# cg-saarland/hagrid

Measured on AMD Instinct MI355X. Metric: Mrays/s (primary traversal) + grid build ms, 1M-tri scene @1/2/4/8 MI355X, higher is better.
Workload: dtype f32

## Files before the change

hagrid_amd/csrc/build.hip:

```cpp
#include "ctx.h"
#include "wave_prims.h"

#include "hagrid/grid.h"
#include "hagrid/prims.h"

#include <cstring>
#include <vector>

using namespace hagrid;
using namespace hagrid_impl;

namespace {

struct BuildK {
    ivec3 dims;
    int shift;
    vec3 bmin, bmax;
    vec3 cell_size;
};

__device__ __forceinline__ Tri load_tri(const float4* __restrict__ tris, int i) {
    const float4* p = tris + 3 * size_t(i);
    const float4 a = p[0], b = p[1], c = p[2];
    return Tri(vec3(a.x, a.y, a.z), a.w, vec3(b.x, b.y, b.z), b.w, vec3(c.x, c.y, c.z), c.w);
}
__device__ __forceinline__ void store_cell(Cell* cells, int i, ivec3 lo, int begin, ivec3 hi, int end) {
    int4* p = reinterpret_cast<int4*>(cells) + 2 * size_t(i);
    p[0] = make_int4(lo.x, lo.y, lo.z, begin);
    p[1] = make_int4(hi.x, hi.y, hi.z, end);
}
__device__ __forceinline__ ivec3 load_cell_min(const Cell* cells, int i) {
    const int4 a = reinterpret_cast<const int4*>(cells)[2 * size_t(i)];
    return ivec3(a.x, a.y, a.z);
}
__device__ __forceinline__ BBox cell_world_box(const BuildK& k, ivec3 lo, ivec3 hi) {
    return BBox(k.bmin + vec3(lo) * k.cell_size, k.bmin + vec3(hi) * k.cell_size);
}

constexpr int kBoxWords = 8;
constexpr int kNoBadTri = 0x7fffffff;
__device__ __forceinline__ int wave_min_i(int v) { return -wave_max(-v); }
__global__ void __launch_bounds__(kBlock) bbox_partials(const float4* __restrict__ tris, int n, float* __restrict__ partials) {
    __shared__ float lds[kWaves][6];
    __shared__ int lds_bad[kWaves];
    float lo[3] = { FLT_MAX, FLT_MAX, FLT_MAX }, hi[3] = { -FLT_MAX, -FLT_MAX, -FLT_MAX };
    int bad = kNoBadTri;
    for (int i = blockIdx.x * kBlock + threadIdx.x; i < n; i += gridDim.x * kBlock) {
        const Tri t = load_tri(tris, i);
        const BBox b = t.bbox();
        if (!tri_admissible(t)) bad = min(bad, i);
        lo[0] = min(lo[0], b.min.x); lo[1] = min(lo[1], b.min.y); lo[2] = min(lo[2], b.min.z);
        hi[0] = max(hi[0], b.max.x); hi[1] = max(hi[1], b.max.y); hi[2] = max(hi[2], b.max.z);
    }
#pragma unroll
    for (int c = 0; c < 3; c++) { lo[c] = wave_min_f(lo[c]); hi[c] = wave_max_f(hi[c]); }
    bad = wave_min_i(bad);
    if (lane_id() == 0) { for (int c = 0; c < 3; c++) { lds[wave_id()][c] = lo[c]; lds[wave_id()][3 + c] = hi[c]; } lds_bad[wave_id()] = bad; }
    __syncthreads();
    if (threadIdx.x < 6) {
        float v = lds[0][threadIdx.x];
        for (int w = 1; w < kWaves; w++) v = threadIdx.x < 3 ? min(v, lds[w][threadIdx.x]) : max(v, lds[w][threadIdx.x]);
        partials[blockIdx.x * kBoxWords + threadIdx.x] = v;
    } else if (threadIdx.x == 6) {
        int v = lds_bad[0];
        for (int w = 1; w < kWaves; w++) v = min(v, lds_bad[w]);
        reinterpret_cast<int*>(partials)[blockIdx.x * kBoxWords + 6] = v;
    }
}
__global__ void __launch_bounds__(kBlock) bbox_final(const float* __restrict__ partials, int num, float* __restrict__ out) {
    __shared__ float lds[kWaves][6];
    __shared__ int lds_bad[kWaves];
    float v[6] = { FLT_MAX, FLT_MAX, FLT_MAX, -FLT_MAX, -FLT_MAX, -FLT_MAX };
    int bad = kNoBadTri;
    for (int i = threadIdx.x; i < num; i += kBlock) {
        for (int c = 0; c < 6; c++) v[c] = c < 3 ? min(v[c], partials[i * kBoxWords + c]) : max(v[c], partials[i * kBoxWords + c]);
        bad = min(bad, reinterpret_cast<const int*>(partials)[i * kBoxWords + 6]);
    }
#pragma unroll
    for (int c = 0; c < 6; c++) v[c] = c < 3 ? wave_min_f(v[c]) : wave_max_f(v[c]);
    bad = wave_min_i(bad);
    if (lane_id() == 0) { for (int c = 0; c < 6; c++) lds[wave_id()][c] = v[c]; lds_bad[wave_id()] = bad; }
    __syncthreads();
    if (threadIdx.x < 6) {
        float r = lds[0][threadIdx.x];
        for (int w = 1; w < kWaves; w++) r = threadIdx.x < 3 ? min(r, lds[w][threadIdx.x]) : max(r, lds[w][threadIdx.x]);
        out[threadIdx.x] = r;
    } else if (threadIdx.x == 6) {
        int r = lds_bad[0];
        for (int w = 1; w < kWaves; w++) r = min(r, lds_bad[w]);
        reinterpret_cast<int*>(out)[6] = r;
    }
}

constexpr int kCoopCells = 64;


__global__ void __launch_bounds__(kBlock) top_log_dims(const int* __restrict__ refs_per_cell, int num_top, BuildK k, float snd_density,
                                                       int* __restrict__ log_dims, int* __restrict__ max_out) {
    __shared__ int lds[kWaves];
    const int i = blockIdx.x * kBlock + threadIdx.x;
    int ld = 0;
    if (i < num_top) {
        const vec3 ext = BBox(k.bmin, k.bmax).extents() / vec3(k.dims);
        const ivec3 d = compute_grid_dims(BBox(vec3(0, 0, 0), ext), refs_per_cell[i], snd_density);
        const int max_dim = max(d.x, max(d.y, d.z));
        ld = 31 - __clz(max_dim);
        ld = (1 << ld) < max_dim ? ld + 1 : ld;
        log_dims[i] = ld;
    }
    ld = wave_max(ld);
    if (lane_id() == 0) lds[wave_id()] = ld;
    __syncthreads();
    if (threadIdx.x == 0) {
        int m = lds[0];
        for (int w = 1; w < kWaves; w++) m = max(m, lds[w]);
        if (m > 0) atomicMax(max_out, m);
    }
}


__device__ __forceinline__ BuildK with_device_shift(BuildK k, const int* __restrict__ shift_dev, vec3 extents) {
    k.shift = *shift_dev;
    k.cell_size = extents / vec3(k.dims << k.shift);
    return k;
}

__device__ __forceinline__ bool prefix_too_large(int s) { return unsigned(s) >= 0x40000000u; }
struct ChildCountIn {
    const uint32_t* entries;
    __device__ int operator()(int i) const { return (entries[i] & 3u) ? 8 : 0; }
    __device__ void load4(int i, int n, int* v) const {
        if (i + 4 <= n && lb_aligned16(entries + i)) {
            const uint4 e = *reinterpret_cast<const uint4*>(entries + i);
            v[0] = (e.x & 3u) ? 8 : 0; v[1] = (e.y & 3u) ? 8 : 0; v[2] = (e.z & 3u) ? 8 : 0; v[3] = (e.w & 3u) ? 8 : 0;
        } else {
            for (int c = 0; c < 4; c++) v[c] = i + c < n ? (*this)(i + c) : 0;
        }
    }
};
struct UpdateEntriesOut {
    uint32_t* entries; int* too_large;
    __device__ static uint32_t word(uint32_t e, int i, int start) { const uint32_t ld = e & 3u; return ld | (uint32_t(ld ? start : i) << 2); }
    __device__ void operator()(int i, int start) const { entries[i] = word(entries[i], i, start); if (prefix_too_large(start)) *too_large = 1; }
    __device__ void store4(int i, int n, const int* v) const {
        if (i + 4 <= n && lb_aligned16(entries + i)) {
            uint4* p = reinterpret_cast<uint4*>(entries + i);
            const uint4 e = *p;
            if (prefix_too_large(v[3])) *too_large = 1;
            *p = make_uint4(word(e.x, i, v[0]), word(e.y, i + 1, v[1]), word(e.z, i + 2, v[2]), word(e.w, i + 3, v[3]));
        } else {
            for (int c = 0; c < 4; c++) if (i + c < n) (*this)(i + c, v[c]);
        }
    }
};

__device__ __forceinline__ int split_mask(const BuildK& k, ivec3 lo, ivec3 hi, const Tri& tri) {
    const vec3 cmin = k.bmin + k.cell_size * vec3(lo);
    const vec3 cmax = k.bmin + k.cell_size * vec3(hi);
    const vec3 mid = (cmin + cmax) * 0.5f;
    int mask = 0xFF;
    const BBox rb = tri.bbox();
    if (rb.min.x > cmax.x || rb.max.x < cmin.x) mask = 0;
    if (rb.min.x > mid.x) mask &= 0xAA;
    if (rb.max.x < mid.x) mask &= 0x55;
    if (rb.min.y > cmax.y || rb.max.y < cmin.y) mask = 0;
    if (rb.min.y > mid.y) mask &= 0xCC;
    if (rb.max.y < mid.y) mask &= 0x33;
    if (rb.min.z > cmax.z || rb.max.z < cmin.z) mask = 0;
    if (rb.min.z > mid.z) mask &= 0xF0;
    if (rb.max.z < mid.z) mask &= 0x0F;
    int todo = mask;
    while (todo) {
        const int i = __ffs(todo) - 1;
        todo &= todo - 1;
        const BBox b(vec3(i & 1 ? mid.x : cmin.x, i & 2 ? mid.y : cmin.y, i & 4 ? mid.z : cmin.z),
                     vec3(i & 1 ? cmax.x : mid.x, i & 2 ? cmax.y : mid.y, i & 4 ? cmax.z : mid.z));
        if (!intersect_prim_cell(tri, b)) mask &= ~(1 << i);
    }
    return mask;
}


struct LeafIn {
    const uint32_t* entries; const int* cell_counts;
    __device__ static Int2 item(uint32_t e, int count) { const bool leaf = (e & 3u) == 0; return Int2{ leaf ? 1 : 0, leaf ? count : 0 }; }
    __device__ Int2 operator()(int i) const { return item(entries[i], cell_counts[i]); }
    __device__ void load4(int i, int n, Int2* v) const {
        if (i + 4 <= n && lb_aligned16(entries + i) && lb_aligned16(cell_counts + i)) {
            const uint4 e = *reinterpret_cast<const uint4*>(entries + i);
            const int4 c = *reinterpret_cast<const int4*>(cell_counts + i);
            v[0] = item(e.x, c.x); v[1] = item(e.y, c.y); v[2] = item(e.z, c.z); v[3] = item(e.w, c.w);
        } else {
            for (int k = 0; k < 4; k++) v[k] = i + k < n ? (*this)(i + k) : Int2{0, 0};
        }
    }
};
struct LeafOut {
    int* start_cell; int* ref_begin;
    __device__ void operator()(int i, Int2 v) const { start_cell[i] = v.a; ref_begin[i] = v.b; }
    __device__ void store4(int i, int n, const Int2* v) const {
        if (i + 4 <= n && lb_aligned16(start_cell + i) && lb_aligned16(ref_begin + i)) {
            *reinterpret_cast<int4*>(start_cell + i) = make_int4(v[0].a, v[1].a, v[2].a, v[3].a);
            *reinterpret_cast<int4*>(ref_begin + i) = make_int4(v[0].b, v[1].b, v[2].b, v[3].b);
        } else {
            for (int k = 0; k < 4; k++) if (i + k < n) (*this)(i + k, v[k]);
        }
    }
};


#ifndef HG_TILE_REFS
#define HG_TILE_REFS 1024
#endif
#ifndef HG_CHUNK_CELLS
#define HG_CHUNK_CELLS 256
#endif
#ifndef HG_EMIT_CHUNK
#define HG_EMIT_CHUNK 256
#endif
#ifndef HG_STAGE
#define HG_STAGE 1024
#endif
constexpr int kTileRefs = HG_TILE_REFS;
constexpr int kChunkCells = HG_CHUNK_CELLS;
constexpr int kEmitChunk = HG_EMIT_CHUNK;
constexpr int kStage = HG_STAGE;

__device__ __forceinline__ void mark_tiles(int* __restrict__ tile_first, int i, int start, int count) {
    for (int t = start / kTileRefs + 1; t <= (start + count) / kTileRefs; t++) tile_first[t] = i + 1;
}
struct SegIn {
    const int* counts;
    __device__ int operator()(int i) const { return counts[i]; }
};
struct SegOut {
    const int* counts; int* seg_begin; int* tile_first;
    Cell* cells; uint32_t* entries; int* cell_counts; const int* log_dims; const int* shift_dev; ivec3 dims;
    __device__ void operator()(int i, int start) const {
        seg_begin[i] = start; mark_tiles(tile_first, i, start, counts[i]);
        const int shift = *shift_dev;
        entries[i] = 0u; cell_counts[i] = 0;
        const int x = i % dims.x, y = (i / dims.x) % dims.y, z = i / (dims.x * dims.y);
        const ivec3 lo(x << shift, y << shift, z << shift);
// ... 425 lines not shown
struct GLevel {
    int2* refs = nullptr; int num_refs = 0;
    Cell* cells = nullptr; uint32_t* entries = nullptr; int num_cells = 0;
    int* cell_counts = nullptr;
    int* seg_begin = nullptr;
    int* tile_first = nullptr; int num_tiles = 0;
    int* start_cell = nullptr; int* ref_begin = nullptr;
};

struct Arena {
    hagrid_ctx* ctx; Temps& tmp; char* base = nullptr; size_t size = 0, used = 0, wanted = 0; int num_tris;
    Arena(hagrid_ctx* c, Temps& t, int n_tris) : ctx(c), tmp(t), num_tris(n_tris) {
        size_t want = c->build_arena_hint;
        if (want && c->build_arena_tris > 0 && 2ll * n_tris < c->build_arena_tris)
            want = size_t(double(want) * 1.25 * double(std::max(n_tris, 1)) / double(c->build_arena_tris)) + 4096;
        if (want) {
            base = pool_try_alloc<char>(c, want);
            if (base) { t.ptrs.push_back(base); size = want; }
        }
    }
    ~Arena() { ctx->build_arena_hint = wanted; ctx->build_arena_tris = num_tris; }
    template <typename T> T* get(size_t n) {
        const size_t bytes = (std::max(n, size_t(1)) * sizeof(T) + 255) & ~size_t(255);
        wanted += bytes;
        if (base && used + bytes <= size) { T* p = reinterpret_cast<T*>(base + used); used += bytes; return p; }
        return tmp.get<T>(n);
    }
    void drop(void* p) { if (!base || p < base || p >= base + size) tmp.drop(p); }
};

int build_levels(hagrid_ctx* ctx, const float4* tris, int num_tris, hagrid_grid* grid, BuildK k, const BBox& gb, float snd_density, Temps& tmp) {
    hipStream_t st = ctx->stream;
    int* dsc = ctx->dscratch;
    Arena ar(ctx, tmp, num_tris);
    const ivec3 dims = k.dims;
    const int num_top = dims.x * dims.y * dims.z;

    int* counts = ar.get<int>(size_t(num_tris));
    int* start_emit = ar.get<int>(size_t(num_tris));
    int* refs_per_cell = ar.get<int>(size_t(num_top));
    int* log_dims = ar.get<int>(size_t(num_top));
    int* const partials = nullptr;
    if (!counts || !start_emit || !refs_per_cell || !log_dims) return HAGRID_ENOMEM;
    HG_HIP(ctx, hipMemsetAsync(refs_per_cell, 0, size_t(num_top) * sizeof(int), st));
    int* big_list = ar.get<int>(size_t(num_tris));
    if (!big_list) return HAGRID_ENOMEM;
    top_range_sizes<<<grid_blocks(num_tris, kBlock), kBlock, 0, st>>>(tris, num_tris, k, counts, big_list, dsc + 2); HG_DBG(ctx);
    if (!ctx_scan<int>(ctx, PlainIn{counts}, PlainOut{start_emit, dsc + 3}, num_tris, partials, (const int*)nullptr, dsc + 0)) return HAGRID_ENOMEM;
    int R0 = 0, num_big = 0;
    {
        int h[4];
        HG_TRY(read_back(ctx, dsc, h, sizeof(h)));
        R0 = h[0]; num_big = h[2];
        if (h[3]) R0 = -1;
    }
    if (R0 < 0 || R0 > 0x3fffffff) HG_FAIL(ctx, HAGRID_ERANGE, "build_grid: too many top-level references");
    ar.drop(counts);
    int* pair_rank = ar.get<int>(size_t(R0) + 1);
    if (!pair_rank) return HAGRID_ENOMEM;
    const int prim_blocks = grid_blocks(num_tris, kBlock), big_blocks = std::min(num_big, 2048);
    count_top_refs<<<prim_blocks + big_blocks, kBlock, 0, st>>>(tris, num_tris, k, start_emit, refs_per_cell, pair_rank, big_list, dsc + 2, prim_blocks); HG_DBG(ctx);
    top_log_dims<<<grid_blocks(num_top, kBlock), kBlock, 0, st>>>(refs_per_cell, num_top, k, snd_density, log_dims, dsc + 1); HG_DBG(ctx);

    std::vector<GLevel> levels;
    GLevel L;
    L.num_refs = R0; L.num_cells = num_top;
    L.num_tiles = grid_blocks(R0, kTileRefs);
    L.refs = ar.get<int2>(size_t(R0) + 1);
    L.cells = ar.get<Cell>(size_t(num_top)); L.entries = ar.get<uint32_t>(size_t(num_top) + 1);
    L.cell_counts = ar.get<int>(size_t(num_top)); L.seg_begin = ar.get<int>(size_t(num_top) + 1);
    L.tile_first = ar.get<int>(size_t(L.num_tiles) + 2);
    L.start_cell = ar.get<int>(size_t(num_top)); L.ref_begin = ar.get<int>(size_t(num_top));
    if (!L.refs || !L.cells || !L.entries || !L.cell_counts || !L.seg_begin || !L.tile_first || !L.start_cell || !L.ref_begin) return HAGRID_ENOMEM;
    if (!ctx_scan<int>(ctx, SegIn{refs_per_cell}, SegOut{refs_per_cell, L.seg_begin, L.tile_first, L.cells, L.entries, L.cell_counts, log_dims, dsc + 1, dims}, num_top, partials,
                       (const int*)nullptr, (int*)nullptr)) return HAGRID_ENOMEM;
    hagrid_build_counts& bc = ctx->counts;
    memset(&bc, 0, sizeof(bc));
    bc.num_tris = num_tris; bc.top_cells = num_top; bc.top_refs = R0;
    emit_top_refs<<<prim_blocks + big_blocks, kBlock, 0, st>>>(tris, num_tris, k, dsc + 1, gb.extents(), start_emit, pair_rank, L.seg_begin, L.refs, log_dims, L.entries, big_list, dsc + 2, prim_blocks); HG_DBG(ctx);
    levels.push_back(L);

    {
        if (!ctx_scan<int>(ctx, ChildCountIn{L.entries}, UpdateEntriesOut{L.entries, dsc + 3}, num_top, (int*)nullptr, (const int*)nullptr, dsc + 8)) return HAGRID_ENOMEM;
    }
    int num_new_cells = 0, shift = 0;
    {
        int h[8];
        HG_TRY(read_back(ctx, dsc + 1, h, sizeof(h)));
        shift = h[0]; num_new_cells = h[7];
        if (h[2]) num_new_cells = -1;
    }
    if (shift >= 24) HG_FAIL(ctx, HAGRID_ERANGE, "build_grid: too many levels");
    k.shift = shift;
    k.cell_size = gb.extents() / vec3(dims << shift);
    ar.drop(start_emit); ar.drop(pair_rank); ar.drop(refs_per_cell);
    for (int level = 0;; level++) {
        GLevel& P = levels.back();
        int* tot = dsc + 8 + 4 * level;
        if (num_new_cells < 0 || num_new_cells > 0x3fffffff) HG_FAIL(ctx, HAGRID_ERANGE, "build_grid: level too large");
        if ((int)levels.size() >= 24) HG_FAIL(ctx, HAGRID_ERANGE, "build_grid: too many levels");
        const bool last = num_new_cells == 0;
        if (last && level > 0) {
            if (level < HAGRID_MAX_LEVELS) { bc.level_refs[level] = P.num_refs; bc.level_cells[level] = P.num_cells; bc.level_kept[level] = P.num_refs; bc.num_levels = level + 1; }
            break;
        }
        GLevel N;
        N.num_cells = num_new_cells;
        unsigned char* masks = ar.get<unsigned char>(size_t(P.num_refs) + 1);
        if (!masks) return HAGRID_ENOMEM;
        if (!last) {
            N.cells = ar.get<Cell>(size_t(num_new_cells)); N.entries = ar.get<uint32_t>(size_t(num_new_cells) + 1);
            N.cell_counts = ar.get<int>(size_t(num_new_cells)); N.seg_begin = ar.get<int>(size_t(num_new_cells) + 1);
            N.tile_first = ar.get<int>(size_t(grid_blocks(8ll * P.num_refs, kTileRefs)) + 2);
            N.start_cell = ar.get<int>(size_t(num_new_cells)); N.ref_begin = ar.get<int>(size_t(num_new_cells));
            if (!N.cells || !N.entries || !N.cell_counts || !N.seg_begin || !N.tile_first || !N.start_cell || !N.ref_begin) return HAGRID_ENOMEM;
        }
        if (P.num_refs > 0) {
            classify_refs<<<std::min(P.num_tiles, 4096), kBlock, 0, st>>>(P.refs, P.seg_begin, P.num_cells, P.num_refs, P.tile_first, P.num_tiles, level == 0 ? 1 : 0,
                                                                             tris, P.cells, P.entries, k, masks, P.cell_counts, N.cells, N.cell_counts, N.entries, tot + 1); HG_DBG(ctx);
        }
        Int2* next = reinterpret_cast<Int2*>(tot + 2);
        if (!last) {
            if (!ctx_scan<Int2>(ctx, ChildSegIn{N.cell_counts, N.entries}, ChildSegOut{N.cell_counts, N.entries, N.seg_begin, N.tile_first, tot + 1}, num_new_cells, (Int2*)nullptr,
                                (const Int2*)nullptr, next)) return HAGRID_ENOMEM;
        }
        int h3[3] = {0, 0, 0};
        HG_TRY(read_back(ctx, tot + 1, h3, sizeof(h3)));
        if (h3[0] < 0) HG_FAIL(ctx, HAGRID_ERANGE, "build_grid: level too large");
        if (level < HAGRID_MAX_LEVELS) { bc.level_refs[level] = P.num_refs; bc.level_cells[level] = P.num_cells; bc.level_kept[level] = h3[0]; bc.num_levels = level + 1; }
        if (last) { ar.drop(masks); break; }
        const int num_children = h3[1];
        if (num_children < 0 || num_children > 0x3fffffff) HG_FAIL(ctx, HAGRID_ERANGE, "build_grid: level too large");
        N.num_refs = num_children; N.num_tiles = grid_blocks(num_children, kTileRefs);
        N.refs = ar.get<int2>(size_t(num_children) + 1);
        if (!N.refs) return HAGRID_ENOMEM;
        if (P.num_refs > 0 && num_children > 0) {
            emit_child_refs<<<std::min(P.num_tiles, 4096), kBlock, 0, st>>>(P.refs, P.seg_begin, P.num_cells, P.num_refs, P.tile_first, P.num_tiles,
                                                                                   masks, P.entries, N.seg_begin, N.refs); HG_DBG(ctx);
        }
        ar.drop(masks);
        num_new_cells = h3[2];
        levels.push_back(N);
    }
    ar.drop(log_dims);

    const int num_levels = (int)levels.size();
    long long total_cells_ll = 0;
    int max_cells = 0;
    for (auto& V : levels) { total_cells_ll += V.num_cells; max_cells = std::max(max_cells, V.num_cells); }
    if (total_cells_ll > 0x3fffffff) HG_FAIL(ctx, HAGRID_ERANGE, "build_grid: too many voxel map entries");
    const int total_cells = int(total_cells_ll);
    Int2* const part2 = nullptr;
    Int2* carry = reinterpret_cast<Int2*>(dsc + 128);
    for (int l = 0; l < num_levels; l++) {
        GLevel& V = levels[l];
        if (!ctx_scan<Int2>(ctx, LeafIn{V.entries, V.cell_counts}, LeafOut{V.start_cell, V.ref_begin}, V.num_cells, part2,
                            l ? carry + (l - 1) : (const Int2*)nullptr, carry + l)) return HAGRID_ENOMEM;
    }
    int hf[2];
    HG_TRY(read_back(ctx, carry + (num_levels - 1), hf, sizeof(hf)));
    const int new_total_cells = hf[0], total_refs = hf[1];
    if (new_total_cells <= 0 || total_refs < 0) HG_FAIL(ctx, HAGRID_ERANGE, "build_grid: inconsistent totals");

    Cell* out_cells = pool_alloc<Cell>(ctx, size_t(new_total_cells));
    uint32_t* out_entries = pool_alloc<uint32_t>(ctx, size_t(total_cells));
    int* out_refs = pool_alloc<int>(ctx, size_t(total_refs));
    if (!out_cells || !out_entries || !out_refs) {
        hagrid_mem_free(ctx, out_cells); hagrid_mem_free(ctx, out_entries); hagrid_mem_free(ctx, out_refs);
        return HAGRID_ENOMEM;
    }
    for (int l = 0, off = 0; l < num_levels; off += levels[l].num_cells, l++) {
        GLevel& V = levels[l];
        concat_level<<<grid_blocks(V.num_cells, kBlock), kBlock, 0, st>>>(V.entries, V.cells, V.cell_counts, V.start_cell, V.ref_begin, V.num_cells, off,
                                                                                  V.refs, V.seg_begin, V.num_refs, l == 0 ? 1 : 0, out_cells, out_entries, out_refs); HG_DBG(ctx);
    }
    hipError_t e = hipGetLastError();
    if (e == hipSuccess) e = hipStreamSynchronize(st);
    if (e != hipSuccess) {
        hagrid_mem_free(ctx, out_cells); hagrid_mem_free(ctx, out_entries); hagrid_mem_free(ctx, out_refs);
        HG_FAIL(ctx, HAGRID_EHIP, hipGetErrorString(e));
    }
    memset(grid, 0, sizeof(*grid));
    grid->entries = out_entries; grid->ref_ids = out_refs; grid->cells = out_cells; grid->small_cells = nullptr;
    grid->bbox_min[0] = gb.min.x; grid->bbox_min[1] = gb.min.y; grid->bbox_min[2] = gb.min.z;
    grid->bbox_max[0] = gb.max.x; grid->bbox_max[1] = gb.max.y; grid->bbox_max[2] = gb.max.z;
    grid->dims[0] = dims.x; grid->dims[1] = dims.y; grid->dims[2] = dims.z;
    grid->num_cells = new_total_cells; grid->num_entries = total_cells; grid->num_refs = total_refs;
    bc.build_cells = new_total_cells; bc.build_entries = total_cells; bc.build_refs = total_refs;
    grid->shift = shift;
    grid->num_offsets = shift + 1;
    for (int i = 0, off = 0; i <= shift; i++) {
        if (i < num_levels) off += levels[i].num_cells;
        grid->offsets[i] = off;
    }
    return HAGRID_OK;
}

}

extern "C" int hagrid_build_grid(hagrid_ctx* ctx, const void* tris_v, int num_tris, hagrid_grid* grid,
                                 float top_density, float snd_density) {
    if (!ctx || !grid) return HAGRID_EINVAL;
    trav_image_drop(ctx);
    if (!tris_v || num_tris <= 0) HG_FAIL(ctx, HAGRID_EINVAL, "build_grid: no triangles");
    HG_HIP(ctx, hipSetDevice(ctx->device));
    const float4* tris = static_cast<const float4*>(tris_v);
    hipStream_t st = ctx->stream;
    Temps tmp(ctx);
    int* dsc = ctx->dscratch;
    HG_HIP(ctx, hipMemsetAsync(dsc, 0, 256 * sizeof(int), st));

    const int bb_blocks = std::min(grid_blocks(num_tris, kBlock), 1024);
    float* bb_part = tmp.get<float>(size_t(bb_blocks) * kBoxWords + 8);
    if (!bb_part) return HAGRID_ENOMEM;
    float* bb_out = bb_part + size_t(bb_blocks) * kBoxWords;
    bbox_partials<<<bb_blocks, kBlock, 0, st>>>(tris, num_tris, bb_part); HG_DBG(ctx);
    bbox_final<<<1, kBlock, 0, st>>>(bb_part, bb_blocks, bb_out); HG_DBG(ctx);
    float hb[8];
    HG_TRY(read_back(ctx, bb_out, hb, sizeof(hb)));
    int bad_tri; memcpy(&bad_tri, &hb[6], sizeof(int));
    if (bad_tri != kNoBadTri) {
        char msg[96];
        snprintf(msg, sizeof(msg), "build_grid: triangle %d is not finite", bad_tri);
        HG_FAIL(ctx, HAGRID_EINVAL, msg);
    }
    BBox gb(vec3(hb[0], hb[1], hb[2]), vec3(hb[3], hb[4], hb[5]));
    {
        const vec3 e = gb.extents();
        if (!(e.x <= FLT_MAX && e.y <= FLT_MAX && e.z <= FLT_MAX)) HG_FAIL(ctx, HAGRID_ERANGE, "build_grid: the extent of the scene box is not finite");
    }
    if (!grid_dims_defined(gb, num_tris, top_density)) gb = widen_scene_box(gb);
    ivec3 dims = compute_grid_dims(gb, num_tris, top_density);
    if (dims.x > 0x3fffffff || dims.y > 0x3fffffff || dims.z > 0x3fffffff) HG_FAIL(ctx, HAGRID_ERANGE, "build_grid: top-level grid too large");
    dims.x += dims.x & 1; dims.y += dims.y & 1; dims.z += dims.z & 1;
    const vec3 ext = gb.extents();
    gb.min -= ext * 0.001f;
    gb.max += ext * 0.001f;
    const long long num_top_ll = (long long)dims.x * dims.y * dims.z;
    if (num_top_ll > 0x3fffffff) HG_FAIL(ctx, HAGRID_ERANGE, "build_grid: top-level grid too large");
    {
        const vec3 e = gb.extents();
        if (!(e.x <= FLT_MAX && e.y <= FLT_MAX && e.z <= FLT_MAX)) HG_FAIL(ctx, HAGRID_ERANGE, "build_grid: the extent of the scene box is not finite");
    }

    BuildK k;
    k.dims = dims; k.shift = 0; k.bmin = gb.min; k.bmax = gb.max; k.cell_size = vec3(0.0f);

    return build_levels(ctx, tris, num_tris, grid, k, gb, snd_density, tmp);
}
```

hagrid_amd/csrc/compress.hip:

```cpp
#include "ctx.h"
#include "wave_prims.h"

#include "hagrid/grid.h"

using namespace hagrid;
using namespace hagrid_impl;

namespace {

struct SentinelIn {
    const Cell* cells;
    __device__ int operator()(int i) const {
        const int4* p = reinterpret_cast<const int4*>(cells) + 2 * size_t(i);
        const int n = p[1].w - p[0].w;
        return n > 0 ? n + 1 : 0;
    }
};

struct SmallCellOut {
    const Cell* cells; const int* refs; uint4* small_cells; int* out_refs;
    __device__ void operator()(int i, int first) const {
        const int4* p = reinterpret_cast<const int4*>(cells) + 2 * size_t(i);
        const int4 a = p[0], b = p[1];
        const int n = b.w - a.w;
        small_cells[i] = make_uint4((uint32_t(a.x) & 0xffffu) | (uint32_t(a.y) << 16),
                                    (uint32_t(a.z) & 0xffffu) | (uint32_t(b.x) << 16),
                                    (uint32_t(b.y) & 0xffffu) | (uint32_t(b.z) << 16),
                                    uint32_t(n > 0 ? first : -1));
        if (n > 0) {
            for (int j = 0; j < n; j++) out_refs[first + j] = refs[a.w + j];
            out_refs[first + n] = -1;
        }
    }
};
struct NullOut { __device__ void operator()(int, int) const {} };

}

extern "C" int hagrid_compress_grid(hagrid_ctx* ctx, hagrid_grid* grid) {
    if (!ctx || !grid) return HAGRID_EINVAL;
    if (!grid->cells || !grid->ref_ids) HG_FAIL(ctx, HAGRID_EINVAL, "compress_grid: incomplete (or already compressed) grid");
    trav_image_drop(ctx);
    for (int c = 0; c < 3; c++)
        if ((grid->dims[c] << grid->shift) >= (1 << 16)) return 0;
    HG_HIP(ctx, hipSetDevice(ctx->device));
    hipStream_t st = ctx->stream;
    const int n = grid->num_cells;
    const Cell* cells = static_cast<const Cell*>(grid->cells);
    int* partials = pool_alloc<int>(ctx, size_t(scan_num_tiles(n)) + 1);
    uint4* small = static_cast<uint4*>(hagrid_mem_alloc(ctx, size_t(n) * 16));
    if (!partials || !small) { hagrid_mem_free(ctx, partials); hagrid_mem_free(ctx, small); return HAGRID_ENOMEM; }
    int* total = ctx->dscratch;
    scan_partials<int, SentinelIn><<<std::max(scan_num_tiles(n), 1), kBlock, 0, st>>>(SentinelIn{cells}, n, partials); HG_DBG(ctx);
    scan_spine<int><<<1, kBlock, 0, st>>>(partials, scan_num_tiles(n), nullptr, total); HG_DBG(ctx);
    int h = 0;
    int rc = read_back(ctx, total, &h, sizeof(int));
    if (rc != HAGRID_OK || h < 0) { hagrid_mem_free(ctx, partials); hagrid_mem_free(ctx, small); return rc != HAGRID_OK ? rc : HAGRID_ERANGE; }
    int* srefs = pool_alloc<int>(ctx, size_t(h));
    if (!srefs) { hagrid_mem_free(ctx, partials); hagrid_mem_free(ctx, small); return HAGRID_ENOMEM; }
    scan_apply<int, SentinelIn, SmallCellOut><<<std::max(scan_num_tiles(n), 1), kBlock, 0, st>>>(
        SentinelIn{cells}, SmallCellOut{cells, static_cast<const int*>(grid->ref_ids), small, srefs}, n, partials); HG_DBG(ctx);
    hipError_t e = hipGetLastError();
    if (e == hipSuccess) e = hipStreamSynchronize(st);
    hagrid_mem_free(ctx, partials);
    ctx->counts.compressed = 1; ctx->counts.compress_cells = n; ctx->counts.compress_refs_out = h;
    if (e != hipSuccess) { hagrid_mem_free(ctx, small); hagrid_mem_free(ctx, srefs); HG_FAIL(ctx, HAGRID_EHIP, hipGetErrorString(e)); }
    hagrid_mem_free(ctx, grid->cells);
    hagrid_mem_free(ctx, grid->ref_ids);
    grid->cells = nullptr;
    grid->small_cells = small;
    grid->ref_ids = srefs;
    grid->num_refs = h;
    return 1;
}
```

hagrid_amd/csrc/ctx.h:

```cpp
#pragma once

#include <hip/hip_runtime.h>

#include <atomic>
#include <cstdio>
#include <memory>
#include <string>
#include <unordered_map>
#include <vector>

#include "hagrid_amd.h"

namespace hagrid_impl {

struct Slot {
    void* ptr = nullptr;
    size_t size = 0;
    bool in_use = false;
    int refs = 0;
};

}

namespace hagrid_impl {

struct TravImageCache {
    void* table = nullptr;
    size_t table_bytes = 0;
    int wide_records = 0;
    void* blocks = nullptr;
    size_t block_bytes = 0;
    bool valid = false;
    bool uniform = false;
    bool general = false;
    int slim = 0;
    int vtop_k = 0;
    uint32_t vtop_base = 0;
    bool detached = false;
    bool borrowed = false;
    std::shared_ptr<std::atomic<bool>> alive;
    const void* entries = nullptr; const void* cells = nullptr; const void* refs = nullptr;
    int num_cells = 0, num_entries = 0, num_refs = 0, shift = 0, dims[3] = {0, 0, 0}, cell_bytes = 32;
    int max_ref = -1;
    void* alt_blocks = nullptr; void* alt_table = nullptr; size_t alt_block_bytes = 0, alt_table_bytes = 0; int alt_wide_records = 0, alt_slim = 0;
};

}

namespace hagrid_impl {
enum MailboxWord : int {
    kMbxRowLen = 300,
    kMbxOrderStale = 304,
    kMbxReadBackEpoch = 310,
    kMbxHeadSuggest = 312,
    kMbxPriorStats = 316,
};
enum ScratchWord : int {
    kScrRowLenBinned = 232,
    kScrRowLen = 236,
    kScrMaxRef = 240,
    kScrBlobFlag = 250,
};
}

struct hagrid_ctx {
    int device = 0;
    hipStream_t stream = nullptr;
    bool keep = false;
    int num_cus = 0;

    std::vector<hagrid_impl::Slot> slots;
    std::unordered_map<void*, int> tracker;
    size_t usage = 0, max_usage = 0;

    hipEvent_t ev_begin = nullptr, ev_end = nullptr;

    int* mailbox = nullptr;
    int* dscratch = nullptr;
    unsigned long long* lb_state = nullptr;
    size_t lb_words = 0;
    unsigned lb_epoch = 0;
    int* row_scores = nullptr;
    int* bin_diff = nullptr;

    int ray_binning = 0;
    int opt_variant = 0;
    int opt_lookback = 1;
    int opt_merge_inplace = 1;
    int opt_merge_inplace_iters = 0;
    int opt_merge_inplace_div = 0;
    int opt_merge_inplace_room = 0;
    int opt_merge_narrow = 1;
    int opt_expand_voxel_map = 1;
    int opt_expand_subset_only = 1;
    int opt_image_width = 0;
    int opt_band_rows = 0;
    int opt_super_log2 = 3;
    int opt_xcd_chunk_log2 = -2;
    int opt_narrow = 1;
    int opt_image_max_mb = 0;
    int opt_quad_head = 20;
    int opt_image_vtop = 1;
    int opt_image_uniform = 1;
    int opt_row_cache = 1;
    struct RayHints {
        const void* key_rays = nullptr; int key_n = 0;
        const void* rowlen_rays = nullptr; int rowlen_n = 0, rowlen_age = 0, rowlen_known = -1, rowlen_seen = 0; bool rows_from_origins = false ;
        hipEvent_t rowlen_evt = nullptr; bool rowlen_pending = false;
        int* lpt_buf = nullptr; int lpt_cap = 0; const void* lpt_rays = nullptr; int lpt_n = 0, lpt_blocks = 0, lpt_age = 0, lpt_period = 32, lpt_rot = 0 ; bool rot_adopted = false ;
        hipEvent_t trial_evt[2] = {nullptr, nullptr}; bool trial_pending = false, trial_with_head = false, head_disabled = false;
        float t_base = 0.0f, t_head = 0.0f; int n_base = 0, n_head = 0, trial_opt = -1 ; unsigned head_serial = 0 ; bool lpt_valid = false;
        int lpt_epoch = 1 , relearn_streak = 0, cooldown = 0, cooldown_len = 64; unsigned long long relearn_clock = 0;
        hipEvent_t share_evt[12][2] = {}; int share_issued = 0, share_done = 0, share_choice = -1 , share_ncand = 0 , share_shape_nc = 0 , share_cands[4] = {0, 0, 0, 0} ,
            share_last = -1 , share_launches = 0; float share_t[4] = {0.0f, 0.0f, 0.0f, 0.0f}; unsigned share_serial = 0 ;
        int trial_kind = 0 , n_all = 0, all_stage = 0 ; float t_all = 0.0f; bool learned_all = false;
        bool learned_once = false;
        unsigned order_serial = 0;
        bool cmp_pending = false, cmp_done = false; int n_conf = 0; float t_conf = 0.0f;
        bool order_loses = false;
        int last_report = -1;
        unsigned long long used = 0;
    };
    static constexpr int kRayHints = 4;
    RayHints hints[kRayHints];
    unsigned long long hint_clock = 0;
    int opt_mailbox = -1;
    int opt_tail = 1;
    int opt_lds_pad = 0;
    int opt_tail_dual = -1;
    int opt_share_trial = 1;
    int opt_order_gate = 1;
    int opt_tile_order = -1;
    int opt_quad_tail = -1;
    int opt_image_slim = 1;
    int opt_image_general = 1;
    int opt_image = 2;

    int opt_id_is_steps = 0;

    hagrid_impl::TravImageCache image;
    unsigned image_serial = 0;
    int readback_epoch = 0;
    int opt_fast_readback = 1;
    int build_arena_tris = 0;
    size_t build_arena_hint = 0;
    hagrid_build_counts counts = {};

    std::string err;
};

namespace hagrid_impl {

inline int fail(hagrid_ctx* ctx, int code, const char* file, int line, const char* msg) {
    if (ctx) {
        char buf[512];
        snprintf(buf, sizeof(buf), "%s(%d): %s", file, line, msg);
        ctx->err = buf;
    }
    return code;
}

#define HG_FAIL(ctx, code, msg) return ::hagrid_impl::fail((ctx), (code), __FILE__, __LINE__, (msg))
#define HG_HIP(ctx, call)                                                                         \
    do {                                                                                          \
        hipError_t e_ = (call);                                                                   \
        if (e_ != hipSuccess) return ::hagrid_impl::fail((ctx), HAGRID_EHIP, __FILE__, __LINE__, hipGetErrorString(e_)); \
    } while (0)
#define HG_TRY(expr)                                                                              \
    do {                                                                                          \
        int rc_ = (expr);                                                                         \
        if (rc_ < 0) return rc_;                                                                  \
    } while (0)

void debug_sync(hagrid_ctx* ctx, const char* file, int line);
#ifdef HAGRID_DEBUG_SYNC
#define HG_DBG(ctx) ::hagrid_impl::debug_sync((ctx), __FILE__, __LINE__)
#else
#define HG_DBG(ctx) do { } while (0)
#endif

template <typename T>
inline T* pool_alloc(hagrid_ctx* ctx, size_t n) {
    return static_cast<T*>(hagrid_mem_alloc(ctx, (n ? n : 1) * sizeof(T)));
}

template <typename T>
inline T* pool_try_alloc(hagrid_ctx* ctx, size_t n) {
    const std::string saved = ctx->err;
    T* p = pool_alloc<T>(ctx, n);
    if (!p) { (void)hipGetLastError(); ctx->err = saved; }
    return p;
}

struct PoolTemps {
    hagrid_ctx* ctx;
    std::vector<void*> ptrs;
    explicit PoolTemps(hagrid_ctx* c) : ctx(c) {}
    PoolTemps(const PoolTemps&) = delete;
    PoolTemps& operator=(const PoolTemps&) = delete;
    template <typename T> T* get(size_t n) { T* p = pool_alloc<T>(ctx, n); if (p) ptrs.push_back(p); return p; }
    void drop(void* p) { for (auto& q : ptrs) if (q == p && p) { hagrid_mem_free(ctx, p); q = nullptr; } }
    void* keep(void* p) { for (auto& q : ptrs) if (q == p) q = nullptr; return p; }
    ~PoolTemps() { for (void* p : ptrs) if (p) hagrid_mem_free(ctx, p); }
};

int pool_split(hagrid_ctx* ctx, void* base, void* const* parts, int n);

int read_back(hagrid_ctx* ctx, const void* dptr, void* hptr, size_t bytes);

inline int grid_blocks(long long n, int block) { return (int)((n + block - 1) / block); }

inline bool aligned(const void* p, size_t n) { return (reinterpret_cast<uintptr_t>(p) & (n - 1)) == 0; }

unsigned long long* lookback_state(hagrid_ctx* ctx, int tiles, int words_per_tile, unsigned* epoch);

int trav_image_build(hagrid_ctx* ctx, const hagrid_grid* grid);
void trav_image_drop(hagrid_ctx* ctx);
bool trav_image_matches(const hagrid_ctx* ctx, const hagrid_grid* grid);
bool trav_image_stale(const hagrid_ctx* ctx);
void trav_image_source_touched(hagrid_ctx* ctx, const void* ptr, size_t bytes);

}
```

hagrid_amd/csrc/ctx.hip:

```cpp
#include "ctx.h"

#include <chrono>

#include <algorithm>
#include <cstring>
#include <iostream>

using namespace hagrid_impl;

extern "C" int hagrid_abi_version(void) { return HAGRID_ABI_VERSION; }

extern "C" int hagrid_ctx_create(hagrid_ctx** out, int device, int keep) {
    if (!out) return HAGRID_EINVAL;
    *out = nullptr;
    int count = 0;
    if (hipGetDeviceCount(&count) != hipSuccess || count <= 0 || device < 0 || device >= count) return HAGRID_ENODEV;
    hagrid_ctx* ctx = new hagrid_ctx();
    ctx->device = device;
    ctx->keep = keep != 0;
    if (hipSetDevice(device) != hipSuccess) { delete ctx; return HAGRID_ENODEV; }
    hipDeviceProp_t prop;
    if (hipGetDeviceProperties(&prop, device) != hipSuccess) { delete ctx; return HAGRID_ENODEV; }
    ctx->num_cus = prop.multiProcessorCount;
    if (hipEventCreate(&ctx->ev_begin) != hipSuccess || hipEventCreate(&ctx->ev_end) != hipSuccess ||
        hipHostMalloc((void**)&ctx->mailbox, 320 * sizeof(int), hipHostMallocDefault) != hipSuccess ||
        hipMalloc((void**)&ctx->dscratch, 256 * sizeof(int)) != hipSuccess) {
        hagrid_ctx_destroy(ctx);
        return HAGRID_EHIP;
    }
    memset(ctx->mailbox, 0, 320 * sizeof(int));
    *out = ctx;
    return HAGRID_OK;
}

extern "C" void hagrid_ctx_destroy(hagrid_ctx* ctx) {
    if (!ctx) return;
    (void)hipSetDevice(ctx->device);
    (void)hipStreamSynchronize(ctx->stream);
    for (auto& h : ctx->hints) h.rowlen_pending = false;
    if (!ctx->image.borrowed && ctx->image.alive) ctx->image.alive->store(false);
    for (auto& s : ctx->slots)
        if (s.ptr) (void)hipFree(s.ptr);
    if (ctx->ev_begin) (void)hipEventDestroy(ctx->ev_begin);
    if (ctx->ev_end) (void)hipEventDestroy(ctx->ev_end);
    for (auto& h : ctx->hints) { if (h.rowlen_evt) (void)hipEventDestroy(h.rowlen_evt); if (h.lpt_buf) (void)hipFree(h.lpt_buf); for (auto& e : h.trial_evt) if (e) (void)hipEventDestroy(e); for (auto& pr : h.share_evt) for (auto& e : pr) if (e) (void)hipEventDestroy(e); }
    if (ctx->mailbox) (void)hipHostFree(ctx->mailbox);
    if (ctx->dscratch) (void)hipFree(ctx->dscratch);
    if (ctx->bin_diff) (void)hipFree(ctx->bin_diff);
    if (ctx->row_scores) (void)hipFree(ctx->row_scores);
    if (ctx->lb_state) (void)hipFree(ctx->lb_state);
    delete ctx;
}

extern "C" int hagrid_ctx_set_stream(hagrid_ctx* ctx, void* stream) {
    if (!ctx) return HAGRID_EINVAL;
    hipStream_t next = static_cast<hipStream_t>(stream);
    if (next == ctx->stream) return HAGRID_OK;
    HG_HIP(ctx, hipSetDevice(ctx->device));
    HG_HIP(ctx, hipStreamSynchronize(ctx->stream));
    ctx->stream = next;
    return HAGRID_OK;
}

extern "C" int hagrid_ctx_synchronize(hagrid_ctx* ctx) {
    if (!ctx) return HAGRID_EINVAL;
    HG_HIP(ctx, hipSetDevice(ctx->device));
    HG_HIP(ctx, hipStreamSynchronize(ctx->stream));
    return HAGRID_OK;
}

extern "C" int hagrid_get_build_counts(const hagrid_ctx* ctx, hagrid_build_counts* out) {
    if (!ctx || !out) return HAGRID_EINVAL;
    *out = ctx->counts;
    return HAGRID_OK;
}

extern "C" const char* hagrid_last_error(const hagrid_ctx* ctx) { return ctx ? ctx->err.c_str() : "no context"; }

extern "C" int hagrid_device_info(const hagrid_ctx* ctx, char* name, int name_len, int* compute_units, int64_t* total_mem) {
    if (!ctx) return HAGRID_EINVAL;
    hipDeviceProp_t prop;
    if (hipGetDeviceProperties(&prop, ctx->device) != hipSuccess) return HAGRID_EHIP;
    if (name && name_len > 0) { strncpy(name, prop.gcnArchName, (size_t)name_len - 1); name[name_len - 1] = 0; }
    if (compute_units) *compute_units = prop.multiProcessorCount;
    if (total_mem) *total_mem = (int64_t)prop.totalGlobalMem;
    return HAGRID_OK;
}


static void release_slot_memory(hagrid_ctx* ctx, Slot& s) {
    if (s.ptr) (void)hipFree(s.ptr);
    ctx->usage -= s.size;
    s.ptr = nullptr;
    s.size = 0;
}

extern "C" void* hagrid_mem_alloc(hagrid_ctx* ctx, size_t bytes) {
    if (!ctx) return nullptr;
    if (bytes == 0) bytes = 4;
    bytes = (bytes + 255) & ~size_t(255);
    int fit = -1, biggest = -1, empty = -1;
    for (int i = 0, n = (int)ctx->slots.size(); i < n; i++) {
        const Slot& s = ctx->slots[i];
        if (s.in_use) continue;
        if (!s.ptr) { if (empty < 0) empty = i; continue; }
        if (s.size >= bytes && (fit < 0 || s.size < ctx->slots[fit].size)) fit = i;
        if (biggest < 0 || s.size > ctx->slots[biggest].size) biggest = i;
    }
    int idx = fit;
    if (idx >= 0 && ctx->slots[idx].size > 4 * bytes && ctx->slots[idx].size > (size_t(64) << 20)) idx = -1;
    if (idx < 0) {
        idx = fit < 0 ? (biggest >= 0 && ctx->keep ? biggest : empty) : empty;
        if (idx < 0) { idx = (int)ctx->slots.size(); ctx->slots.emplace_back(); }
        Slot& s = ctx->slots[idx];
        if (s.ptr) release_slot_memory(ctx, s);
        void* p = nullptr;
        (void)hipSetDevice(ctx->device);
        if (hipMalloc(&p, bytes) != hipSuccess) {
            for (auto& t : ctx->slots) if (!t.in_use && t.ptr) release_slot_memory(ctx, t);
            if (hipMalloc(&p, bytes) != hipSuccess) { fail(ctx, HAGRID_ENOMEM, __FILE__, __LINE__, "hipMalloc failed"); return nullptr; }
        }
        s.ptr = p; s.size = bytes;
        ctx->usage += bytes;
        ctx->max_usage = std::max(ctx->max_usage, ctx->usage);
    }
    Slot& s = ctx->slots[idx];
    s.in_use = true;
    s.refs = 1;
    ctx->tracker[s.ptr] = idx;
    return s.ptr;
}

int hagrid_impl::pool_split(hagrid_ctx* ctx, void* base, void* const* parts, int n) {
    auto it = ctx->tracker.find(base);
    if (it == ctx->tracker.end() || n <= 0) HG_FAIL(ctx, HAGRID_EINVAL, "pool_split: not a pool buffer");
    const int idx = it->second;
    Slot& s = ctx->slots[idx];
    if (s.refs != 1 || s.ptr != base) HG_FAIL(ctx, HAGRID_EINVAL, "pool_split: buffer is already split");
    for (int i = 0; i < n; i++) {
        const char* p = static_cast<const char*>(parts[i]);
        if (p < static_cast<const char*>(base) || p >= static_cast<const char*>(base) + s.size) HG_FAIL(ctx, HAGRID_EINVAL, "pool_split: part outside the buffer");
        for (int j = 0; j < i; j++) if (parts[j] == parts[i]) HG_FAIL(ctx, HAGRID_EINVAL, "pool_split: parts coincide");
    }
    ctx->tracker.erase(it);
    for (int i = 0; i < n; i++) ctx->tracker[parts[i]] = idx;
    s.refs = n;
    return HAGRID_OK;
}

extern "C" int hagrid_mem_free(hagrid_ctx* ctx, void* ptr) {
    if (!ctx) return HAGRID_EINVAL;
    if (!ptr) return HAGRID_OK;
    auto it = ctx->tracker.find(ptr);
    if (it == ctx->tracker.end()) HG_FAIL(ctx, HAGRID_EINVAL, "free of a pointer that does not come from this MemManager");
    trav_image_source_touched(ctx, ptr, 1);
    it = ctx->tracker.find(ptr);
    Slot& s = ctx->slots[it->second];
    ctx->tracker.erase(it);
    if (--s.refs > 0) return HAGRID_OK;
    s.in_use = false;
    if (!ctx->keep) {
        HG_HIP(ctx, hipStreamSynchronize(ctx->stream));
        release_slot_memory(ctx, s);
    }
    return HAGRID_OK;
}

extern "C" int hagrid_mem_copy_h2d(hagrid_ctx* ctx, void* dst, const void* src, size_t bytes) {
    if (!ctx) return HAGRID_EINVAL;
    if (!bytes) return HAGRID_OK;
    trav_image_source_touched(ctx, dst, bytes);
    HG_HIP(ctx, hipSetDevice(ctx->device));
    HG_HIP(ctx, hipMemcpyAsync(dst, src, bytes, hipMemcpyHostToDevice, ctx->stream));
    HG_HIP(ctx, hipStreamSynchronize(ctx->stream));
    return HAGRID_OK;
}
extern "C" int hagrid_mem_copy_d2h(hagrid_ctx* ctx, void* dst, const void* src, size_t bytes) {
    if (!ctx) return HAGRID_EINVAL;
    if (!bytes) return HAGRID_OK;
    HG_HIP(ctx, hipSetDevice(ctx->device));
    HG_HIP(ctx, hipMemcpyAsync(dst, src, bytes, hipMemcpyDeviceToHost, ctx->stream));
    HG_HIP(ctx, hipStreamSynchronize(ctx->stream));
    return HAGRID_OK;
}
extern "C" int hagrid_mem_copy_d2d(hagrid_ctx* ctx, void* dst, const void* src, size_t bytes) {
    if (!ctx) return HAGRID_EINVAL;
    if (!bytes) return HAGRID_OK;
    trav_image_source_touched(ctx, dst, bytes);
    HG_HIP(ctx, hipSetDevice(ctx->device));
    HG_HIP(ctx, hipMemcpyAsync(dst, src, bytes, hipMemcpyDeviceToDevice, ctx->stream));
    return HAGRID_OK;
}
extern "C" int hagrid_mem_zero(hagrid_ctx* ctx, void* ptr, size_t bytes) {
    if (!ctx) return HAGRID_EINVAL;
    if (!bytes) return HAGRID_OK;
    trav_image_source_touched(ctx, ptr, bytes);
    HG_HIP(ctx, hipSetDevice(ctx->device));
    HG_HIP(ctx, hipMemsetAsync(ptr, 0, bytes, ctx->stream));
    return HAGRID_OK;
}
extern "C" int hagrid_mem_one(hagrid_ctx* ctx, void* ptr, size_t bytes) {
    if (!ctx) return HAGRID_EINVAL;
    if (!bytes) return HAGRID_OK;
    trav_image_source_touched(ctx, ptr, bytes);
    HG_HIP(ctx, hipSetDevice(ctx->device));
    HG_HIP(ctx, hipMemsetAsync(ptr, 0xFF, bytes, ctx->stream));
    return HAGRID_OK;
}
extern "C" size_t hagrid_mem_usage(const hagrid_ctx* ctx) { return ctx ? ctx->usage : 0; }
extern "C" size_t hagrid_mem_max_usage(const hagrid_ctx* ctx) { return ctx ? ctx->max_usage : 0; }

extern "C" void hagrid_mem_debug_slots(const hagrid_ctx* ctx) {
    if (!ctx) return;
    size_t total = 0;
    std::cout << "SLOTS: " << std::endl;
    for (const auto& s : ctx->slots) {
        std::cout << "[" << (s.in_use ? 'X' : ' ') << "] " << (double)s.size / (1024.0 * 1024.0) << "MB" << std::endl;
        total += s.size;
    }
    std::cout << (double)total / (1024.0 * 1024.0) << "MB total" << std::endl;
}


extern "C" int hagrid_profile_begin(hagrid_ctx* ctx) {
    if (!ctx) return HAGRID_EINVAL;
    HG_HIP(ctx, hipSetDevice(ctx->device));
    HG_HIP(ctx, hipEventRecord(ctx->ev_begin, ctx->stream));
    return HAGRID_OK;
}
extern "C" float hagrid_profile_end(hagrid_ctx* ctx) {
    if (!ctx) return -1.0f;
    float ms = -1.0f;
    if (hipEventRecord(ctx->ev_end, ctx->stream) != hipSuccess) return -1.0f;
    if (hipEventSynchronize(ctx->ev_end) != hipSuccess) return -1.0f;
    if (hipEventElapsedTime(&ms, ctx->ev_begin, ctx->ev_end) != hipSuccess) return -1.0f;
    return ms;
}

namespace {
typedef float f32x4_t __attribute__((ext_vector_type(4)));
__global__ void __launch_bounds__(256) bw_stream_kernel(const f32x4_t* __restrict__ a, const f32x4_t* __restrict__ b, f32x4_t* __restrict__ c, size_t n) {
    const size_t base = size_t(blockIdx.x) * 1024 + threadIdx.x;
    if (!b) {
        f32x4_t v[4];
#pragma unroll
        for (int j = 0; j < 4; j++) if (base + j * 256 < n) v[j] = __builtin_nontemporal_load(a + base + j * 256);
#pragma unroll
        for (int j = 0; j < 4; j++) if (base + j * 256 < n) __builtin_nontemporal_store(v[j], c + base + j * 256);
    } else {
        f32x4_t v[4], w[4];
#pragma unroll
        for (int j = 0; j < 4; j++) if (base + j * 256 < n) { v[j] = __builtin_nontemporal_load(a + base + j * 256); w[j] = __builtin_nontemporal_load(b + base + j * 256); }
#pragma unroll
        for (int j = 0; j < 4; j++) if (base + j * 256 < n) __builtin_nontemporal_store(v[j] + 3.0f * w[j], c + base + j * 256);
    }
}
}

extern "C" int hagrid_bandwidth_probe(hagrid_ctx* ctx, size_t bytes, int iters, float* copy_gbps, float* triad_gbps) {
    if (!ctx || iters <= 0 || bytes < (size_t(1) << 20)) return HAGRID_EINVAL;
    HG_HIP(ctx, hipSetDevice(ctx->device));
    const size_t n = bytes / 16;
    f32x4_t* a = pool_alloc<f32x4_t>(ctx, n);
    f32x4_t* b = pool_alloc<f32x4_t>(ctx, n);
    f32x4_t* c = pool_alloc<f32x4_t>(ctx, n);
    int rc = HAGRID_OK;
    if (!a || !b || !c) rc = HAGRID_ENOMEM;
    if (rc == HAGRID_OK) {
        (void)hipMemsetAsync(a, 0, n * 16, ctx->stream); (void)hipMemsetAsync(b, 0, n * 16, ctx->stream);
        const int blocks = int((n + 1023) / 1024);
        float best_copy = 0.0f, best_triad = 0.0f;
        for (int it = 0; it < iters + 1 && rc == HAGRID_OK; it++) {
            float ms = -1.0f;
            if (hagrid_profile_begin(ctx) != HAGRID_OK) { rc = HAGRID_EHIP; break; }
            bw_stream_kernel<<<blocks, 256, 0, ctx->stream>>>(a, nullptr, c, n); HG_DBG(ctx);
            ms = hagrid_profile_end(ctx);
            if (ms > 0.0f && it) best_copy = std::max(best_copy, float(2.0 * double(n) * 16.0 / (double(ms) * 1e6)));
            if (hagrid_profile_begin(ctx) != HAGRID_OK) { rc = HAGRID_EHIP; break; }
            bw_stream_kernel<<<blocks, 256, 0, ctx->stream>>>(a, b, c, n); HG_DBG(ctx);
            ms = hagrid_profile_end(ctx);
            if (ms > 0.0f && it) best_triad = std::max(best_triad, float(3.0 * double(n) * 16.0 / (double(ms) * 1e6)));
        }
        if (copy_gbps) *copy_gbps = best_copy;
        if (triad_gbps) *triad_gbps = best_triad;
        if (hipGetLastError() != hipSuccess) rc = HAGRID_EHIP;
    }
    hagrid_mem_free(ctx, a); hagrid_mem_free(ctx, b); hagrid_mem_free(ctx, c);
    return rc;
}

unsigned long long* hagrid_impl::lookback_state(hagrid_ctx* ctx, int tiles, int words_per_tile, unsigned* epoch) {
    const size_t need = size_t(tiles > 0 ? tiles : 1) * size_t(words_per_tile);
    if (need > ctx->lb_words || ctx->lb_epoch >= (1u << 30) - 2u) {
        (void)hipStreamSynchronize(ctx->stream);
        if (need > ctx->lb_words) {
            if (ctx->lb_state) (void)hipFree(ctx->lb_state);
            ctx->lb_state = nullptr; ctx->lb_words = 0;
            const size_t words = need + need / 2 + 1024;
            if (hipMalloc((void**)&ctx->lb_state, words * sizeof(unsigned long long)) != hipSuccess) { (void)hipGetLastError(); return nullptr; }
            ctx->lb_words = words;
        }
        (void)hipMemsetAsync(ctx->lb_state, 0, ctx->lb_words * sizeof(unsigned long long), ctx->stream);
        ctx->lb_epoch = 0;
    }
    *epoch = ++ctx->lb_epoch;
    return ctx->lb_state;
}

void hagrid_impl::debug_sync(hagrid_ctx* ctx, const char* file, int line) {
    hipError_t e = hipStreamSynchronize(ctx->stream);
    if (e == hipSuccess) e = hipGetLastError();
    if (e != hipSuccess) {
        fprintf(stderr, "%s(%d): %s\n", file, line, hipGetErrorString(e));
        abort();
    }
}

extern "C" int hagrid_debug_sync_enabled(void) {
#ifdef HAGRID_DEBUG_SYNC
    return 1;
#else
    return 0;
#endif
}

namespace {
__global__ void __launch_bounds__(256) publish_words(const int* __restrict__ src, int n, int* dst, int* flag, int epoch) {
    if (int(threadIdx.x) < n) dst[threadIdx.x] = src[threadIdx.x];
    __threadfence_system();
    __syncthreads();
    if (threadIdx.x == 0) __hip_atomic_store(flag, epoch, __ATOMIC_RELEASE, __HIP_MEMORY_SCOPE_SYSTEM);
}
}

int hagrid_impl::read_back(hagrid_ctx* ctx, const void* dptr, void* hptr, size_t bytes) {
    if (ctx->opt_fast_readback && bytes > 0 && bytes <= 256 * sizeof(int) && (bytes & 3u) == 0 && (reinterpret_cast<uintptr_t>(dptr) & 3u) == 0) {
        int* flag = ctx->mailbox + kMbxReadBackEpoch;
        const int epoch = ++ctx->readback_epoch;
        publish_words<<<1, 256, 0, ctx->stream>>>(static_cast<const int*>(dptr), int(bytes / 4), ctx->mailbox, flag, epoch);
        HG_HIP(ctx, hipGetLastError());
        const auto t0 = std::chrono::steady_clock::now();
        for (unsigned spins = 0;; spins++) {
            if (__atomic_load_n(flag, __ATOMIC_ACQUIRE) == epoch) break;
            if ((spins & 1023u) == 1023u && std::chrono::steady_clock::now() - t0 > std::chrono::milliseconds(20)) {
                HG_HIP(ctx, hipStreamSynchronize(ctx->stream));
                if (__atomic_load_n(flag, __ATOMIC_ACQUIRE) != epoch) HG_FAIL(ctx, HAGRID_EHIP, "read_back: the words never arrived");
                break;
            }
        }
        memcpy(hptr, ctx->mailbox, bytes);
        return HAGRID_OK;
    }
    if (bytes <= 256 * sizeof(int)) {
        HG_HIP(ctx, hipMemcpyAsync(ctx->mailbox, dptr, bytes, hipMemcpyDeviceToHost, ctx->stream));
        HG_HIP(ctx, hipStreamSynchronize(ctx->stream));
        memcpy(hptr, ctx->mailbox, bytes);
    } else {
        HG_HIP(ctx, hipMemcpyAsync(hptr, dptr, bytes, hipMemcpyDeviceToHost, ctx->stream));
        HG_HIP(ctx, hipStreamSynchronize(ctx->stream));
    }
    return HAGRID_OK;
}
```

hagrid_amd/csrc/expand.hip:

```cpp
#include "ctx.h"
#include "wave_prims.h"

#include "hagrid/grid.h"
#include "hagrid/prims.h"

using namespace hagrid;
using namespace hagrid_impl;

namespace {

struct ExpandK { ivec3 dims; ivec3 top; int shift; vec3 gmin, cell_size, grid_inv; const int* voxel_cells; };
constexpr int kChanged = 1 << 3;
struct CellRec { ivec3 lo; int begin; ivec3 hi; int end; };

__device__ __forceinline__ CellRec load_cell(const Cell* cells, int i) {
    const int4* p = reinterpret_cast<const int4*>(cells) + 2 * size_t(i);
    const int4 a = p[0], b = p[1];
    CellRec c; c.lo = ivec3(a.x, a.y, a.z); c.begin = a.w; c.hi = ivec3(b.x, b.y, b.z); c.end = b.w;
    return c;
}
__device__ __forceinline__ int comp(const ivec3& v, int axis) { return axis == 0 ? v.x : (axis == 1 ? v.y : v.z); }


__device__ __forceinline__ int lower_bound_in(const int* __restrict__ a, int n, int x) {
// ... 113 lines not shown
        ov1 = face_growth<axis, SUBSET_ONLY>(k, entries, refs, tris, cells, cell, false, flag);
        ov2 = face_growth<axis, SUBSET_ONLY>(k, entries, refs, tris, cells, cell, true, flag);
    }
    if (axis == 0) { cell.lo.x += ov1; cell.hi.x += ov2; }
    if (axis == 1) { cell.lo.y += ov1; cell.hi.y += ov2; }
    if (axis == 2) { cell.lo.z += ov1; cell.hi.z += ov2; }
    cell_flags[id] = (unsigned char)((flag ? 1 << axis : 0) | (flags & ~((1 << axis) | kChanged)) | ((ov1 | ov2) ? kChanged : 0));
    int4* out = reinterpret_cast<int4*>(new_cells) + 2 * size_t(id);
    out[0] = make_int4(cell.lo.x, cell.lo.y, cell.lo.z, cell.begin);
    out[1] = make_int4(cell.hi.x, cell.hi.y, cell.hi.z, cell.end);
}

template <int axis, bool SUBSET_ONLY>
__global__ void __launch_bounds__(kBlock) overlap_step(ExpandK k, const Entry* __restrict__ entries, const int* __restrict__ refs,
                                                       const float4* __restrict__ tris, const Cell* __restrict__ cells, Cell* __restrict__ new_cells,
                                                       unsigned char* __restrict__ cell_flags, int num_cells) {
    const int id = xcd_block(blockIdx.x, gridDim.x) * kBlock + threadIdx.x;
    if (id >= num_cells) return;
    const int flags = cell_flags[id];
    if ((flags & (1 << axis)) == 0) {
        const int4* p = reinterpret_cast<const int4*>(cells) + 2 * size_t(id);
        int4* out = reinterpret_cast<int4*>(new_cells) + 2 * size_t(id);
        const int4 a = p[0], b = p[1];
        out[0] = a; out[1] = b;
        if (flags & kChanged) cell_flags[id] = (unsigned char)(flags & ~kChanged);
        return;
    }
    grow_cell<axis, SUBSET_ONLY, false>(k, entries, refs, tris, cells, new_cells, cell_flags, id, flags, false);
}

constexpr int kSelectItems = 16;
constexpr int kSelectTile = kBlock * kSelectItems;

template <int axis>
__global__ void __launch_bounds__(kBlock) expand_select(const Cell* __restrict__ cells, Cell* __restrict__ new_cells, unsigned char* __restrict__ cell_flags,
                                                        int num_cells, int* __restrict__ list, int* __restrict__ count) {
    __shared__ int tile_list[kSelectTile];
    __shared__ int tile_count, tile_base;
    if (threadIdx.x == 0) tile_count = 0;
    __syncthreads();
    const int base = blockIdx.x * kSelectTile;
    int fl[kSelectItems];
    #pragma unroll
    for (int j = 0; j < kSelectItems; j++) {
        const int id = base + j * kBlock + threadIdx.x;
        fl[j] = id < num_cells ? cell_flags[id] : 0;
    }
    #pragma unroll
    for (int j = 0; j < kSelectItems; j++) {
        const int id = base + j * kBlock + threadIdx.x;
        const int flags = fl[j];
        const bool listed = (flags & (1 << axis)) != 0;
        const unsigned long long m = __ballot(listed);
        int wbase = 0;
        if (lane_id() == 0 && m) wbase = atomicAdd(&tile_count, __popcll(m));
        wbase = __shfl(wbase, 0, 64);
        if (listed) {
            tile_list[wbase + __popcll(m & ((1ull << lane_id()) - 1ull))] = id;
        } else if (flags & kChanged) {
            const int4* p = reinterpret_cast<const int4*>(cells) + 2 * size_t(id);
            int4* out = reinterpret_cast<int4*>(new_cells) + 2 * size_t(id);
            const int4 a = p[0], b = p[1];
            out[0] = a; out[1] = b;
            cell_flags[id] = (unsigned char)(flags & ~kChanged);
        }
    }
    __syncthreads();
    if (threadIdx.x == 0) tile_base = tile_count ? atomicAdd(count, tile_count) : 0;
    __syncthreads();
    for (int i = threadIdx.x; i < tile_count; i += kBlock) list[tile_base + i] = tile_list[i];
}

template <int axis, bool SUBSET_ONLY>
__global__ void __launch_bounds__(kBlock) expand_listed(ExpandK k, const Entry* __restrict__ entries, const int* __restrict__ refs,
                                                        const float4* __restrict__ tris, const Cell* __restrict__ cells, Cell* __restrict__ new_cells,
                                                        unsigned char* __restrict__ cell_flags, const int* __restrict__ list, const int* __restrict__ count) {
    const int n = *count, active = (2 * n + kBlock - 1) / kBlock;
    if (int(blockIdx.x) >= active) return;
    const int t = xcd_block(blockIdx.x, active) * kBlock + threadIdx.x;
    const int i = t >> 1;
    if (i >= n) return;
    const int id = list[i];
    grow_cell<axis, SUBSET_ONLY, true>(k, entries, refs, tris, cells, new_cells, cell_flags, id, cell_flags[id], (t & 1) != 0);
}

template <int axis, bool SUBSET_ONLY>
void listed_step(hipStream_t st, const ExpandK& k, const Entry* entries, const int* refs, const float4* tris, const Cell* cells, Cell* other,
                 unsigned char* flags, int n, int* list, int* count) {
    expand_select<axis><<<grid_blocks(n, kSelectTile), kBlock, 0, st>>>(cells, other, flags, n, list, count);
    expand_listed<axis, SUBSET_ONLY><<<grid_blocks(2ll * n, kBlock), kBlock, 0, st>>>(k, entries, refs, tris, cells, other, flags, list, count);
}

}

extern "C" int hagrid_expand_grid(hagrid_ctx* ctx, hagrid_grid* grid, const void* tris_v, int iters) {
    if (!ctx || !grid) return HAGRID_EINVAL;
    const bool subset_only = ctx->opt_expand_subset_only != 0;
    if (!subset_only && !tris_v && iters > 0) HG_FAIL(ctx, HAGRID_EINVAL, "expand_grid: the precise mode needs the triangles");
    const float4* tris = static_cast<const float4*>(tris_v);
    if (iters <= 0) return HAGRID_OK;
    if (!grid->cells || !grid->entries || !grid->ref_ids) HG_FAIL(ctx, HAGRID_EINVAL, "expand_grid: incomplete (or compressed) grid");
    trav_image_drop(ctx);
    HG_HIP(ctx, hipSetDevice(ctx->device));
    hipStream_t st = ctx->stream;
    ExpandK k;
    k.top = ivec3(grid->dims[0], grid->dims[1], grid->dims[2]);
    k.dims = k.top << grid->shift;
    k.shift = grid->shift;
    {
        const vec3 lo(grid->bbox_min[0], grid->bbox_min[1], grid->bbox_min[2]), ext = vec3(grid->bbox_max[0], grid->bbox_max[1], grid->bbox_max[2]) - lo;
        k.gmin = lo; k.cell_size = ext / vec3(k.dims); k.grid_inv = vec3(k.dims) / ext;
    }
    const int n = grid->num_cells;
    Cell* cells = static_cast<Cell*>(grid->cells);
    Cell* other = pool_alloc<Cell>(ctx, size_t(n));
    unsigned char* flags = pool_alloc<unsigned char>(ctx, size_t(n));
    if (!other || !flags) { hagrid_mem_free(ctx, other); hagrid_mem_free(ctx, flags); return HAGRID_ENOMEM; }
    (void)hipMemsetAsync(flags, 0xFF, size_t(n), st);
    const Entry* entries = static_cast<const Entry*>(grid->entries);
    const int* refs = static_cast<const int*>(grid->ref_ids);
    const int blocks = grid_blocks(n, kBlock);
    int* list = iters > 1 ? pool_try_alloc<int>(ctx, size_t(n)) : nullptr;
    const long long voxels = (long long)k.dims.x * k.dims.y * k.dims.z;
    int* voxel_cells = (ctx->opt_expand_voxel_map && voxels <= (1ll << 28)) ? pool_try_alloc<int>(ctx, size_t(voxels)) : nullptr;
    k.voxel_cells = voxel_cells;
    if (voxel_cells) { ExpandK kf = k; kf.voxel_cells = nullptr; fill_voxel_cells<<<grid_blocks(voxels, kBlock), kBlock, 0, st>>>(kf, entries, voxel_cells, int(voxels)); HG_DBG(ctx); }
    int* counts = ctx->dscratch + 160;
    const int max_listed = 48;
    if (list) (void)hipMemsetAsync(counts, 0, max_listed * sizeof(int), st);
    int listed = 0;
    for (int it = 0; it < iters; it++) {
        if (it > 0 && list && listed + 3 <= max_listed) {
            if (subset_only) {
                listed_step<0, true>(st, k, entries, refs, tris, cells, other, flags, n, list, counts + listed++); std::swap(cells, other);
                listed_step<1, true>(st, k, entries, refs, tris, cells, other, flags, n, list, counts + listed++); std::swap(cells, other);
                listed_step<2, true>(st, k, entries, refs, tris, cells, other, flags, n, list, counts + listed++); std::swap(cells, other);
            } else {
                listed_step<0, false>(st, k, entries, refs, tris, cells, other, flags, n, list, counts + listed++); std::swap(cells, other);
                listed_step<1, false>(st, k, entries, refs, tris, cells, other, flags, n, list, counts + listed++); std::swap(cells, other);
                listed_step<2, false>(st, k, entries, refs, tris, cells, other, flags, n, list, counts + listed++); std::swap(cells, other);
            }
            continue;
        }
        if (subset_only) {
            overlap_step<0, true><<<blocks, kBlock, 0, st>>>(k, entries, refs, tris, cells, other, flags, n); HG_DBG(ctx); std::swap(cells, other);
            overlap_step<1, true><<<blocks, kBlock, 0, st>>>(k, entries, refs, tris, cells, other, flags, n); HG_DBG(ctx); std::swap(cells, other);
            overlap_step<2, true><<<blocks, kBlock, 0, st>>>(k, entries, refs, tris, cells, other, flags, n); HG_DBG(ctx); std::swap(cells, other);
        } else {
            overlap_step<0, false><<<blocks, kBlock, 0, st>>>(k, entries, refs, tris, cells, other, flags, n); HG_DBG(ctx); std::swap(cells, other);
            overlap_step<1, false><<<blocks, kBlock, 0, st>>>(k, entries, refs, tris, cells, other, flags, n); HG_DBG(ctx); std::swap(cells, other);
            overlap_step<2, false><<<blocks, kBlock, 0, st>>>(k, entries, refs, tris, cells, other, flags, n); HG_DBG(ctx); std::swap(cells, other);
        }
    }
    hipError_t e = hipGetLastError();
    if (e == hipSuccess) e = hipStreamSynchronize(st);
    ctx->counts.expand_passes = 3 * iters; ctx->counts.expand_cells = n;
    hagrid_mem_free(ctx, flags);
    hagrid_mem_free(ctx, other);
    hagrid_mem_free(ctx, list);
    hagrid_mem_free(ctx, voxel_cells);
    grid->cells = cells;
    if (e != hipSuccess) HG_FAIL(ctx, HAGRID_EHIP, hipGetErrorString(e));
    return HAGRID_OK;
}
```

hagrid_amd/csrc/flatten.hip:

```cpp
#include "ctx.h"
#include "wave_prims.h"

#include "hagrid/grid.h"

using namespace hagrid;
using namespace hagrid_impl;

namespace {

constexpr int kFlatLevels = 3;

__global__ void __launch_bounds__(kBlock) collapse_and_depth(uint32_t* __restrict__ entries, int* __restrict__ depths, int first, int num) {
    const int id = blockIdx.x * kBlock + threadIdx.x;
    if (id >= num) return;
    uint32_t e = entries[first + id];
    int d = 0;
    if (e & 3u) {
        const uint4* p = reinterpret_cast<const uint4*>(entries + (e >> 2));
        const uint4 a = p[0], b = p[1];
        if (a.x == a.y && a.x == a.z && a.x == a.w && a.x == b.x && b.x == b.y && b.x == b.z && b.x == b.w) {
            e = a.x;
            entries[first + id] = e;
        }
    }
    if (e & 3u) {
        const int4* q = reinterpret_cast<const int4*>(depths + (e >> 2));
        const int4 a = q[0], b = q[1];
        d = 1 + max(max(max(a.x, b.x), max(a.y, b.y)), max(max(a.z, b.z), max(a.w, b.w)));
    }
    depths[first + id] = d;
}

struct BlockSizeIn {
    const int* depths;
    __device__ int operator()(int i) const { const int d = depths[i]; return d > 0 ? 1 << (min(d, kFlatLevels) * 3) : 0; }
};
struct StartOut {
    int* start;
    __device__ void operator()(int i, int s) const { start[i] = s; }
};

__global__ void __launch_bounds__(kBlock) copy_top(const uint32_t* __restrict__ entries, const int* __restrict__ start, const int* __restrict__ depths,
                                                   uint32_t* __restrict__ out, int num) {
    const int id = blockIdx.x * kBlock + threadIdx.x;
    if (id >= num) return;
    uint32_t e = entries[id];
    if (e & 3u) e = uint32_t(min(depths[id], kFlatLevels)) | (uint32_t(start[id]) << 2);
    out[id] = e;
}

__global__ void __launch_bounds__(kBlock) flatten_level(const uint32_t* __restrict__ entries, const int* __restrict__ start, const int* __restrict__ depths,
                                                        uint32_t* __restrict__ out, int first, int num) {
    const int id = blockIdx.x * kWaves + wave_id();
    if (id >= num) return;
    const int d = min(depths[first + id], kFlatLevels);
    if (d == 0) return;
    const int nsub = 1 << (3 * d);
    const int base = start[first + id];
    const uint32_t root = entries[first + id];
    for (int m = lane_id(); m < nsub; m += 64) {
        int x = 0, y = 0, z = 0, next_id = first + id;
        uint32_t e = root;
        for (int cur = d - 1; cur >= 0; cur--) {
            const int pos = m >> (cur * 3);
            x += (pos & 1) << cur;
            y += ((pos >> 1) & 1) << cur;
            z += ((pos >> 2) & 1) << cur;
            if (e & 3u) { next_id = int(e >> 2) + (pos & 7); e = entries[next_id]; }
        }
        if (e & 3u) e = uint32_t(min(depths[next_id], kFlatLevels)) | (uint32_t(start[next_id]) << 2);
        out[base + x + ((y + (z << d)) << d)] = e;
    }
}

}

extern "C" int hagrid_flatten_grid(hagrid_ctx* ctx, hagrid_grid* grid) {
    if (!ctx || !grid) return HAGRID_EINVAL;
    if (!grid->entries || grid->num_offsets != grid->shift + 1) HG_FAIL(ctx, HAGRID_EINVAL, "flatten_grid: needs the un-flattened voxel map of build_grid/merge_grid");
    trav_image_drop(ctx);
    HG_HIP(ctx, hipSetDevice(ctx->device));
    hipStream_t st = ctx->stream;
    const int shift = grid->shift, num_entries = grid->num_entries;
    uint32_t* entries = static_cast<uint32_t*>(grid->entries);
    auto first_of = [&](int i) { return i > 0 ? grid->offsets[i - 1] : 0; };

    int* depths = pool_alloc<int>(ctx, size_t(num_entries) + 8);
    int* start = pool_alloc<int>(ctx, size_t(num_entries) + 8);
    int max_level = 0;
    for (int i = 0; i <= shift; i++) max_level = std::max(max_level, grid->offsets[i] - first_of(i));
    int* partials = pool_alloc<int>(ctx, size_t(scan_num_tiles(max_level)) + 1);
    auto release = [&]() { hagrid_mem_free(ctx, depths); hagrid_mem_free(ctx, start); hagrid_mem_free(ctx, partials); };
    if (!depths || !start || !partials) { release(); return HAGRID_ENOMEM; }

    for (int i = shift; i >= 0; i--) {
        const int first = first_of(i), num = grid->offsets[i] - first;
        if (num > 0) collapse_and_depth<<<grid_blocks(num, kBlock), kBlock, 0, st>>>(entries, depths, first, num);
    }
    int* carry = ctx->dscratch;
    const int top_entries = grid->offsets[0];
    HG_HIP(ctx, hipMemcpyAsync(carry, &top_entries, sizeof(int), hipMemcpyHostToDevice, st));
    int groups = 0;
    for (int i = 0; i < shift; i += kFlatLevels, groups++) {
        const int first = first_of(i), num = grid->offsets[i] - first;
        if (!ctx_scan<int>(ctx, BlockSizeIn{depths + first}, StartOut{start + first}, num, partials, carry + groups, carry + groups + 1)) { release(); return HAGRID_ENOMEM; }
    }
    int h[HAGRID_MAX_LEVELS + 2];
    int rc = read_back(ctx, carry, h, sizeof(int) * size_t(groups + 1));
    if (rc != HAGRID_OK) { release(); return rc; }
    const int total_entries = h[groups];
    if (total_entries < top_entries || total_entries > 0x3fffffff) { release(); HG_FAIL(ctx, HAGRID_ERANGE, "flatten_grid: voxel map too large"); }

    uint32_t* out = pool_alloc<uint32_t>(ctx, size_t(total_entries));
    if (!out) { release(); return HAGRID_ENOMEM; }
    copy_top<<<grid_blocks(top_entries, kBlock), kBlock, 0, st>>>(entries, start, depths, out, top_entries); HG_DBG(ctx);
    int new_offsets[HAGRID_MAX_LEVELS], num_new = 0;
    for (int i = 0, g = 0; i < shift; i += kFlatLevels, g++) {
        const int first = first_of(i), num = grid->offsets[i] - first;
        if (num > 0) flatten_level<<<grid_blocks(num, kWaves), kBlock, 0, st>>>(entries, start, depths, out, first, num);
        new_offsets[num_new++] = h[g];
    }
    new_offsets[num_new++] = total_entries;
    hipError_t e = hipGetLastError();
    if (e == hipSuccess) e = hipStreamSynchronize(st);
    if (e != hipSuccess) { release(); hagrid_mem_free(ctx, out); HG_FAIL(ctx, HAGRID_EHIP, hipGetErrorString(e)); }
    release();
    hagrid_mem_free(ctx, entries);
    ctx->counts.flatten_entries_in = num_entries; ctx->counts.flatten_entries_out = total_entries;
    grid->entries = out;
    grid->num_entries = total_entries;
    grid->num_offsets = num_new;
    for (int i = 0; i < num_new; i++) grid->offsets[i] = new_offsets[i];
    return HAGRID_OK;
}
```

hagrid_amd/csrc/kat/hagrid_amd_kat.h:

```cpp
#ifndef HAGRID_AMD_KAT_H
#define HAGRID_AMD_KAT_H

#include "hagrid_amd.h"

#ifdef __cplusplus
extern "C" {
#endif

int hagrid_kat_intersect_prim_ray(hagrid_ctx* ctx, const void* tris, const void* rays, const int32_t* tri_index,
                                  int n, int32_t* ret, int32_t* hit_id, float* hit_t);
int hagrid_kat_intersect_prim_ray_uvs(hagrid_ctx* ctx, const void* tris, const void* rays, const int32_t* tri_index,
                                      int n, int32_t* ret, int32_t* hit_id, float* hit_t, float* hit_u, float* hit_v);
int hagrid_kat_intersect_prim_cell(hagrid_ctx* ctx, const void* tris, const void* boxes, const int32_t* tri_index,
                                   int n, int32_t* ret);
int hagrid_kat_compute_range(hagrid_ctx* ctx, const int32_t* dims3, const void* grid_bb, const void* obj_bb, int n, int32_t* out6);
int hagrid_kat_compute_grid_dims(hagrid_ctx* ctx, const void* bb, const int32_t* num_prims, const float* density, int n, int32_t* out3);
int hagrid_kat_lookup_entry(hagrid_ctx* ctx, const uint32_t* entries, int num_entries, int shift, const int32_t* top_dims3,
                            const int32_t* voxels3, int n, uint32_t* out);
int hagrid_kat_scan(hagrid_ctx* ctx, const int32_t* values, int n, int words, const int32_t* carry_in, int lookback,
                    int32_t* out, int32_t* total);
int hagrid_kat_detect_ray_rows(hagrid_ctx* ctx, const void* rays_dev, int num_rays, float bbox_diag, int32_t* row_len);
int hagrid_kat_tile_slots(hagrid_ctx* ctx, int num_rays, int row_len, int super_log2, int xcd_chunk_log2, int32_t* slots);
int hagrid_kat_bin_rays(hagrid_ctx* ctx, const float* bbox_min3, const float* bbox_max3, const void* rays_dev, int num_rays, int mode,
                        int32_t* perm_out, uint16_t* keys_out, int32_t* decision_out);
int hagrid_kat_tile_order(hagrid_ctx* ctx, const int32_t* cost_in, int n, int rot, int head_tenths, const void* rays_dev, int num_rays,
                          int32_t* order_out, int32_t* cost_after_out, int32_t* suggest_out, float* sample_out8);
int hagrid_kat_traverse_timed(hagrid_ctx* ctx, const hagrid_grid* grid, const void* tris, const void* rays, void* hits, int num_rays,
                              int row_len, int tail, unsigned long long* times_dev, const int* tile_order_dev);
int hagrid_kat_image_records(hagrid_ctx* ctx, const hagrid_grid* grid, const int32_t* voxels3, int n, uint32_t* records8, int64_t* image_bytes);

int hagrid_kat_set_option(hagrid_ctx* ctx, const char* key, int value);

int hagrid_kat_forget_hints(hagrid_ctx* ctx);
int hagrid_kat_order_state(hagrid_ctx* ctx, const void* rays, int32_t* out12, float* ms4);

#ifdef __cplusplus
}
#endif
#endif
```

hagrid_amd/csrc/kat/kat.hip:

```cpp
#include "../trav_kernels.h"
#include "hagrid_amd_kat.h"

#include <cstring>

using namespace hagrid;
using namespace hagrid_impl;
using namespace hagrid_trav;


namespace {

__global__ void kat_prim_ray(const Tri* tris, const Ray* rays, const int* idx, int n, int* ret, int* hid, float* ht) {
    const int i = blockIdx.x * blockDim.x + threadIdx.x;
    if (i >= n) return;
    Hit h(-1, rays[i].tmax, 0, 0);
    ret[i] = intersect_prim_ray(tris[idx[i]], rays[i], idx[i], h) ? 1 : 0;
    hid[i] = h.id; ht[i] = h.t;
}
__global__ void kat_prim_ray_uvs(const Tri* tris, const Ray* rays, const int* idx, int n, int* ret, int* hid, float* ht, float* hu, float* hv) {
    const int i = blockIdx.x * blockDim.x + threadIdx.x;
    if (i >= n) return;
    Hit h(-1, rays[i].tmax, 0, 0);
    ret[i] = intersect_prim_ray_uvs(tris[idx[i]], rays[i], idx[i], h) ? 1 : 0;
    hid[i] = h.id; ht[i] = h.t; hu[i] = h.u; hv[i] = h.v;
// ... 144 lines not shown
    int max_idx = 0;
    for (int i = 0; i < n; i++) max_idx = std::max(max_idx, tri_index[i]);
    Staged t(ctx, tris, size_t(max_idx + 1) * 48), b(ctx, boxes, size_t(n) * 32), ix(ctx, tri_index, size_t(n) * 4), o(ctx, nullptr, size_t(n) * 4);
    kat_prim_cell<<<grid_blocks(n, 64), 64, 0, ctx->stream>>>((const Tri*)t.d, (const BBox*)b.d, (const int*)ix.d, n, (int*)o.d); HG_DBG(ctx);
    HG_HIP(ctx, hipGetLastError());
    return o.fetch(ret);
}

extern "C" int hagrid_kat_compute_range(hagrid_ctx* ctx, const int32_t* dims3, const void* grid_bb, const void* obj_bb, int n, int32_t* out6) {
    if (!ctx || n <= 0) return HAGRID_EINVAL;
    Staged d(ctx, dims3, size_t(n) * 12), g(ctx, grid_bb, size_t(n) * 32), ob(ctx, obj_bb, size_t(n) * 32), o(ctx, nullptr, size_t(n) * 24);
    kat_range<<<grid_blocks(n, 64), 64, 0, ctx->stream>>>((const int*)d.d, (const BBox*)g.d, (const BBox*)ob.d, n, (int*)o.d); HG_DBG(ctx);
    HG_HIP(ctx, hipGetLastError());
    return o.fetch(out6);
}

extern "C" int hagrid_kat_compute_grid_dims(hagrid_ctx* ctx, const void* bb, const int32_t* num_prims, const float* density, int n, int32_t* out3) {
    if (!ctx || n <= 0) return HAGRID_EINVAL;
    Staged b(ctx, bb, size_t(n) * 32), np(ctx, num_prims, size_t(n) * 4), de(ctx, density, size_t(n) * 4), o(ctx, nullptr, size_t(n) * 12);
    kat_grid_dims<<<grid_blocks(n, 64), 64, 0, ctx->stream>>>((const BBox*)b.d, (const int*)np.d, (const float*)de.d, n, (int*)o.d); HG_DBG(ctx);
    HG_HIP(ctx, hipGetLastError());
    return o.fetch(out3);
}

extern "C" int hagrid_kat_lookup_entry(hagrid_ctx* ctx, const uint32_t* entries, int num_entries, int shift, const int32_t* top_dims3,
                                       const int32_t* voxels3, int n, uint32_t* out) {
    if (!ctx || n <= 0 || num_entries <= 0) return HAGRID_EINVAL;
    Staged e(ctx, entries, size_t(num_entries) * 4), v(ctx, voxels3, size_t(n) * 12), o(ctx, nullptr, size_t(n) * 4);
    kat_lookup<<<grid_blocks(n, 64), 64, 0, ctx->stream>>>((const Entry*)e.d, shift, ivec3(top_dims3[0], top_dims3[1], top_dims3[2]), (const int*)v.d, n, (uint32_t*)o.d); HG_DBG(ctx);
    HG_HIP(ctx, hipGetLastError());
    return o.fetch(out);
}

extern "C" int hagrid_kat_detect_ray_rows(hagrid_ctx* ctx, const void* rays_dev, int num_rays, float bbox_diag, int32_t* row_len) {
    if (!ctx || !rays_dev || num_rays < 0 || !row_len) return HAGRID_EINVAL;
    int* d = ctx->dscratch + 232;
    TraverseArgs a;
    memset(&a, 0, sizeof(a));
    a.rays = static_cast<const float4*>(rays_dev);
    a.max_x = bbox_diag; a.min_x = 0.0f;
    launch_detect(ctx, a, num_rays, d, 65536);
    HG_HIP(ctx, hipGetLastError());
    HG_TRY(read_back(ctx, d, row_len, sizeof(int)));
    *row_len &= kRowLenMask;
    return HAGRID_OK;
}

extern "C" int hagrid_kat_bin_rays(hagrid_ctx* ctx, const float* bbox_min3, const float* bbox_max3, const void* rays_dev, int num_rays, int mode,
                                   int32_t* perm_out, uint16_t* keys_out, int32_t* decision_out) {
    if (!ctx || !bbox_min3 || !bbox_max3 || !rays_dev || num_rays <= 0 || (mode != 1 && mode != 2) || !perm_out || !keys_out) return HAGRID_EINVAL;
    TraverseArgs a;
    memset(&a, 0, sizeof(a));
    a.rays = static_cast<const float4*>(rays_dev); a.num_rays = num_rays;
    a.min_x = bbox_min3[0]; a.min_y = bbox_min3[1]; a.min_z = bbox_min3[2];
    a.max_x = bbox_max3[0]; a.max_y = bbox_max3[1]; a.max_z = bbox_max3[2];
    if (decision_out) *decision_out = -1;
    if (num_rays > 4096) {
        PoolTemps pre(ctx);
        int* p0 = pre.get<int>(size_t(num_rays)); unsigned short* p1 = pre.get<unsigned short>(size_t(num_rays));
        if (p0) HG_TRY(hagrid_mem_one(ctx, p0, size_t(num_rays) * sizeof(int)));
        if (p1) HG_TRY(hagrid_mem_one(ctx, p1, size_t(num_rays) * sizeof(unsigned short)));
    }
    PoolTemps tmp(ctx);
    const int saved = ctx->ray_binning;
    ctx->ray_binning = mode;
    const int rc = bin_rays(ctx, a, num_rays, tmp);
    ctx->ray_binning = saved;
    HG_TRY(rc);
    HG_HIP(ctx, hipGetLastError());
    if (!a.perm) return 0;
    if (tmp.ptrs.size() < 2 || tmp.ptrs[0] != a.perm || !tmp.ptrs[1]) HG_FAIL(ctx, HAGRID_EINVAL, "kat_bin_rays: bin_rays no longer takes perm and keys first from its pool temporaries");
    HG_TRY(hagrid_mem_copy_d2h(ctx, perm_out, a.perm, size_t(num_rays) * sizeof(int)));
    HG_TRY(hagrid_mem_copy_d2h(ctx, keys_out, tmp.ptrs[1], size_t(num_rays) * sizeof(uint16_t)));
    if (decision_out && a.perm_flag) HG_TRY(hagrid_mem_copy_d2h(ctx, decision_out, a.perm_flag, sizeof(int)));
    return 1;
}

extern "C" int hagrid_kat_tile_order(hagrid_ctx* ctx, const int32_t* cost_in, int n, int rot, int head_tenths, const void* rays_dev, int num_rays,
                                     int32_t* order_out, int32_t* cost_after_out, int32_t* suggest_out, float* sample_out8) {
    if (!ctx || !cost_in || n <= 0 || n > kMaxOrderTiles || head_tenths < 0 || head_tenths > 1000 || !rays_dev || num_rays <= 0 ||
        !order_out || !cost_after_out || !suggest_out || !sample_out8) return HAGRID_EINVAL;
    hagrid_ctx::RayHints h;
    if (!tile_order_buffers(ctx, h, n)) return HAGRID_ENOMEM;
    struct Release { hagrid_ctx* ctx; hagrid_ctx::RayHints& h; ~Release() { (void)hipStreamSynchronize(ctx->stream); (void)hipFree(h.lpt_buf); } } release{ctx, h};
    if (h.lpt_cap < n) HG_FAIL(ctx, HAGRID_EINVAL, "kat_tile_order: buffers smaller than the launch");
    const int32_t unset = -1;
    Staged sg(ctx, &unset, sizeof(int));
    if (!sg.d) return HAGRID_ENOMEM;
    HG_TRY(hagrid_mem_copy_h2d(ctx, h.lpt_buf, cost_in, size_t(n) * sizeof(int)));
    HG_HIP(ctx, hipMemsetAsync(h.lpt_buf + h.lpt_cap, 0xFF, size_t(h.lpt_cap) * sizeof(int) + 8 * sizeof(float4), ctx->stream));
    TraverseArgs a;
    memset(&a, 0, sizeof(a));
    a.rays = static_cast<const float4*>(rays_dev); a.num_rays = num_rays;
    const int saved = ctx->opt_quad_head;
    ctx->opt_quad_head = head_tenths;
    launch_tile_order(ctx, h, n, a, rot, static_cast<int*>(sg.d));
    ctx->opt_quad_head = saved;
    HG_HIP(ctx, hipGetLastError());
    HG_TRY(hagrid_mem_copy_d2h(ctx, order_out, h.lpt_buf + h.lpt_cap, size_t(n) * sizeof(int)));
    HG_TRY(hagrid_mem_copy_d2h(ctx, cost_after_out, h.lpt_buf, size_t(n) * sizeof(int)));
    HG_TRY(hagrid_mem_copy_d2h(ctx, sample_out8, tile_order_samples(h), 2 * sizeof(float4)));
    return sg.fetch(suggest_out);
}

extern "C" int hagrid_kat_tile_slots(hagrid_ctx* ctx, int num_rays, int row_len, int super_log2, int xcd_chunk_log2, int32_t* slots) {
    if (!ctx || num_rays <= 0 || !slots || super_log2 < 0 || (super_log2 & 0xff) > 8) return HAGRID_EINVAL;
    const int blocks = grid_blocks(num_rays, 64);
    TraverseArgs a;
    memset(&a, 0, sizeof(a));
    a.num_rays = num_rays; a.row_len_hint = row_len; a.super_log2 = super_log2 & 0xff; a.band_rows = super_log2 >> 8; a.xcd_chunk_log2 = xcd_chunk_log2;
    Staged o(ctx, nullptr, size_t(blocks) * 64 * 4);
    if (!o.d) return HAGRID_ENOMEM;
    kat_tile_slots<<<blocks, 64, 0, ctx->stream>>>(a, (int*)o.d); HG_DBG(ctx);
    HG_HIP(ctx, hipGetLastError());
    return o.fetch(slots);
}

extern "C" int hagrid_kat_image_records(hagrid_ctx* ctx, const hagrid_grid* grid, const int32_t* voxels3, int n, uint32_t* records8, int64_t* image_bytes) {
    if (!ctx || !grid || n < 0) return HAGRID_EINVAL;
    if (!trav_image_matches(ctx, grid)) HG_FAIL(ctx, HAGRID_EINVAL, "no traversal image for this grid");
    if (image_bytes) *image_bytes = (int64_t)ctx->image.block_bytes + (int64_t)ctx->image.table_bytes;
    if (n == 0) return HAGRID_OK;
    TraverseArgs a;
    HG_TRY(make_args(ctx, grid, nullptr, nullptr, nullptr, 0, a));
    image_args(ctx, a);
    Staged v(ctx, voxels3, size_t(n) * 12), o(ctx, nullptr, size_t(n) * 32);
    if (!v.d || !o.d) return HAGRID_ENOMEM;
    kat_image_records<<<grid_blocks(n, 64), 64, 0, ctx->stream>>>(a, (const int*)v.d, n, (uint32_t*)o.d, 1, ctx->image.slim, ctx->image.uniform ? 1 : 0, ctx->image.general ? 1 : 0); HG_DBG(ctx);
    HG_HIP(ctx, hipGetLastError());
    return o.fetch(records8);
}

extern "C" int hagrid_kat_traverse_timed(hagrid_ctx* ctx, const hagrid_grid* grid, const void* tris, const void* rays, void* hits, int num_rays,
                                         int row_len, int tail, unsigned long long* times_dev, const int* tile_order_dev) {
    if (!ctx || !grid || !times_dev || num_rays <= 0) return HAGRID_EINVAL;
    if (!trav_image_matches(ctx, grid) || !(ctx->image.uniform && ctx->image.slim == 20))
        HG_FAIL(ctx, HAGRID_EINVAL, "kat_traverse_timed: needs the table-free image with 20-bit slim records of this grid");
    TraverseArgs a;
    HG_TRY(make_args(ctx, grid, tris, rays, hits, num_rays, a));
    image_args(ctx, a);
    a.row_len_hint = row_len; a.wave_times = times_dev; a.tile_order = tile_order_dev;
    const int blocks = grid_blocks(num_rays, 64);
    if (tail) traverse_kernel_tail<20, true><<<blocks, 64, 0, ctx->stream>>>(a);
    else      traverse_kernel_img<0, 20, 0, true><<<blocks, 64, 0, ctx->stream>>>(a);
    HG_DBG(ctx);
    HG_HIP(ctx, hipGetLastError());
    return HAGRID_OK;
}

extern "C" int hagrid_kat_set_option(hagrid_ctx* ctx, const char* key, int value) {
    if (!ctx || !key) return HAGRID_EINVAL;
    struct { const char* name; int* dst; int lo, hi; } table[] = {
        {"traverse.variant", &ctx->opt_variant, 0, 4},              {"traverse.narrow", &ctx->opt_narrow, 0, 1},
        {"traverse.image_uniform", &ctx->opt_image_uniform, 0, 2},  {"traverse.image_slim", &ctx->opt_image_slim, 1, 2}, {"traverse.image_general", &ctx->opt_image_general, 0, 2}, {"traverse.image_vtop", &ctx->opt_image_vtop, 0, 1}, {"traverse.quad_head", &ctx->opt_quad_head, 0, 1000}, {"ctx.fast_readback", &ctx->opt_fast_readback, 0, 1},
        {"traverse.tail", &ctx->opt_tail, 0, 1},                    {"traverse.quad_tail", &ctx->opt_quad_tail, -1, 100},
        {"traverse.tail_dual", &ctx->opt_tail_dual, -1, 1},        
        {"traverse.super_tile", &ctx->opt_super_log2, 0, 8},        {"traverse.xcd_chunk", &ctx->opt_xcd_chunk_log2, -2, 16},
        {"traverse.row_cache", &ctx->opt_row_cache, 0, 1},          {"traverse.lds_pad", &ctx->opt_lds_pad, 0, 65536},
        {"merge.narrow_cells", &ctx->opt_merge_narrow, 0, 1},       {"scan.lookback", &ctx->opt_lookback, 1, 2},
        {"traverse.order_gate", &ctx->opt_order_gate, 0, 1}, {"traverse.share_trial", &ctx->opt_share_trial, 0, 1}, {"traverse.band_rows", &ctx->opt_band_rows, 0, 1 << 16}, {"traverse.mailbox", &ctx->opt_mailbox, -1, 1},
        {"merge.inplace", &ctx->opt_merge_inplace, 0, 1},           {"merge.inplace_iters", &ctx->opt_merge_inplace_iters, 0, 1 << 20}, {"merge.inplace_room", &ctx->opt_merge_inplace_room, 0, 0x7fffffff}, {"merge.inplace_div", &ctx->opt_merge_inplace_div, 0, 1 << 20},
        {"expand.voxel_map", &ctx->opt_expand_voxel_map, 0, 1},
    };
    for (auto& t : table)
        if (!strcmp(key, t.name)) {
            if (value < t.lo || value > t.hi || (t.dst == &ctx->opt_variant && value == 3)) HG_FAIL(ctx, HAGRID_EINVAL, "kat_set_option: value out of range");
            *t.dst = value;
            return HAGRID_OK;
        }
    return hagrid_set_option(ctx, key, value);
}

extern "C" int hagrid_kat_order_state(hagrid_ctx* ctx, const void* rays, int32_t* out12, float* ms2 ) {
    if (!ctx || !out12) return HAGRID_EINVAL;
    for (int i = 0; i < 12; i++) out12[i] = 0;
    out12[0] = -1;
    for (int i = 0; i < hagrid_ctx::kRayHints; i++) {
        const hagrid_ctx::RayHints& h = ctx->hints[i];
        if (h.key_rays != rays) continue;
        const int v[12] = {i, h.lpt_valid, h.cooldown > 0, h.lpt_rot, h.head_disabled, h.n_base, h.n_head, h.share_choice >= 0 ? h.share_cands[h.share_choice] : -1, h.share_done + 100 * h.share_issued + 10000 * int(h.order_loses), h.n_all + 10 * int(h.learned_all) + 100 * h.cooldown, __atomic_load_n(ctx->mailbox + kMbxHeadSuggest + i, __ATOMIC_RELAXED), h.share_launches};
        for (int k = 0; k < 12; k++) out12[k] = v[k];
        if (ms2) { ms2[0] = h.t_base; ms2[1] = h.t_head; ms2[2] = h.t_all; ms2[3] = h.share_choice >= 0 ? h.share_t[h.share_choice] : 0.0f; }
        return HAGRID_OK;
    }
    return HAGRID_OK;
}

extern "C" int hagrid_kat_forget_hints(hagrid_ctx* ctx) {
    if (!ctx) return HAGRID_EINVAL;
    for (auto& h : ctx->hints) { h.key_rays = nullptr; h.key_n = 0; h.used = 0; h.lpt_rays = nullptr; h.lpt_valid = false; h.rowlen_rays = nullptr; h.rowlen_seen = 0; h.share_ncand = 0; h.share_shape_nc = 0; h.share_choice = -1; }
    return HAGRID_OK;
}
```

hagrid_amd/csrc/merge.hip:

```cpp
#include "ctx.h"
#include "wave_prims.h"

#include "hagrid/grid.h"

using namespace hagrid;
using namespace hagrid_impl;

namespace {

struct MergeK {
    ivec3 dims;
    ivec3 top;
    vec3 cell_size;
    int shift;
};

struct CellRec { ivec3 lo; int begin; ivec3 hi; int end; };

template <bool NARROW> struct CellFmt;
template <> struct CellFmt<false> {
    static __device__ __forceinline__ CellRec load(const void* cells, int i) {
        const int4* p = reinterpret_cast<const int4*>(cells) + 2 * size_t(i);
        const int4 a = p[0], b = p[1];
        CellRec c; c.lo = ivec3(a.x, a.y, a.z); c.begin = a.w; c.hi = ivec3(b.x, b.y, b.z); c.end = b.w;
// ... 256 lines not shown
    return m;
}

__device__ __forceinline__ int ip_compact_tile(uint32_t mask4 , int id4, int* __restrict__ list, int* __restrict__ count) {
    if (threadIdx.x == 0) *count = 0;
    __syncthreads();
    const int n = int((mask4 & 1u) + ((mask4 >> 8) & 1u) + ((mask4 >> 16) & 1u) + ((mask4 >> 24) & 1u));
    const int incl = wave_inclusive_scan(n);
    const int total = __shfl(incl, 63, 64);
    int base = 0;
    if (lane_id() == 63 && total) base = atomicAdd(count, total);
    base = __shfl(base, 63, 64) + incl - n;
    for (int c = 0; c < 4; c++) if (mask4 & (1u << (8 * c))) list[base++] = id4 + c;
    __syncthreads();
    return *count;
}

__global__ void __launch_bounds__(kBlock) ip_begin(const void* __restrict__ cells, int slots, int* __restrict__ list_end, unsigned char* __restrict__ dirty,
                                                   const unsigned char* __restrict__ stamps, int since_x, int since_y, int since_z,
                                                   unsigned char* __restrict__ evaluated, unsigned char* __restrict__ absorbs, int* __restrict__ books, int num_refs, size_t dstride) {
    const int id = blockIdx.x * kBlock + threadIdx.x;
    if (id == 0) { books[0] = num_refs; books[1] = slots; books[2] = num_refs; books[3] = 0; }
    if (id >= slots) return;
    evaluated[id] = 0; absorbs[id] = 0;
    list_end[id] = int(reinterpret_cast<const uint4*>(cells)[size_t(id) + 1].w);
    const int st = stamps ? stamps[id] : 255;
    dirty[id] = st >= since_x; dirty[dstride + id] = st >= since_y; dirty[2 * dstride + id] = st >= since_z;
}
__global__ void __launch_bounds__(kBlock) ip_mark_entry(MergeK k, const Entry* __restrict__ entries, const void* __restrict__ cells, int slots,
                                                        unsigned char* __restrict__ dirty, const unsigned char* __restrict__ stamps, int since_x, int since_y, int since_z, size_t dstride) {
    __shared__ int list[kIpTile];
    __shared__ int count;
    const int id4 = (blockIdx.x * kBlock + threadIdx.x) * kIpPer;
    const int since_min = min(since_x, min(since_y, since_z));
    uint32_t recent = 0;
    if (id4 < slots) {
        const uint32_t f = ip_flags4(stamps, id4, slots);
        for (int c = 0; c < 4; c++) if (id4 + c < slots && int((f >> (8 * c)) & 0xffu) >= since_min) recent |= 1u << (8 * c);
    }
    const int n = ip_compact_tile(recent, id4, list, &count);
    for (int i = threadIdx.x; i < n; i += kBlock) {
        const int id = list[i], st = stamps[id];
        const CellRec cell = CellFmt<true>::load(cells, id);
        for (int axis = 0; axis < 3; axis++) {
            if (st < (axis == 0 ? since_x : (axis == 1 ? since_y : since_z))) continue;
            ivec3 p = cell.lo;
            if (axis == 0) p.x--; else if (axis == 1) p.y--; else p.z--;
            if (comp(p, axis) < 0) continue;
            dirty[size_t(axis) * dstride + int(lookup_entry(entries, k.shift, k.top, p))] = 1;
        }
    }
}

__device__ __forceinline__ void ip_count_one(int id, int axis, const MergeK& k, const Entry* __restrict__ entries, const void* __restrict__ cells, const int* __restrict__ list_end,
                                             const int* __restrict__ refs, Int2* __restrict__ minfo, int* __restrict__ nexts, unsigned char* __restrict__ evaluated,
                                             unsigned char* __restrict__ has_prev, int pass_tag, int empty_mask) {
    if (ip_is_tomb(reinterpret_cast<const uint4*>(cells)[id])) return;
    const CellRec c1 = ip_load(cells, list_end, id);
    const ivec3 np = next_cell_pos(axis, c1.lo, c1.hi);
    if (!merge_allowed(k, empty_mask, comp(c1.lo, axis)) || comp(np, axis) >= comp(k.dims, axis)) return;
    const int next_id = ip_live(cells, int(lookup_entry(entries, k.shift, k.top, np)));
    const CellRec c2 = ip_load(cells, list_end, next_id);
    if (!aligned(axis, c1, c2)) return;
    const int n = merged_size_if_cheaper(k, axis, c1, c2, refs);
    if (n < 0) return;
    minfo[id] = Int2{ n, (c1.end - c1.begin) + (c2.end - c2.begin) - n };
    nexts[id] = next_id;
    evaluated[id] = (unsigned char)pass_tag;
    has_prev[next_id] = (unsigned char)pass_tag;
}
__global__ void __launch_bounds__(kBlock) ip_counts(int axis, MergeK k, const Entry* __restrict__ entries, const void* __restrict__ cells, const int* __restrict__ list_end,
                                                    const int* __restrict__ refs, int slots, unsigned char* __restrict__ dirty_axis,
                                                    Int2* __restrict__ minfo, int* __restrict__ nexts, unsigned char* __restrict__ evaluated,
                                                    unsigned char* __restrict__ has_prev, int pass_tag, int empty_mask) {
    __shared__ int list[kIpTile];
    __shared__ int count;
    const int id4 = (xcd_block(blockIdx.x, gridDim.x) * kBlock + threadIdx.x) * kIpPer;
    uint32_t mask = 0;
    if (id4 < slots) {
        const uint32_t f = ip_flags4(dirty_axis, id4, slots);
        for (int c = 0; c < 4; c++) if ((f >> (8 * c)) & 0xffu) { mask |= 1u << (8 * c); dirty_axis[id4 + c] = 0; }
    }
    const int n = ip_compact_tile(mask, id4, list, &count);
    for (int i = threadIdx.x; i < n; i += kBlock)
        ip_count_one(list[i], axis, k, entries, cells, list_end, refs, minfo, nexts, evaluated, has_prev, pass_tag, empty_mask);
}

__global__ void __launch_bounds__(kBlock) ip_chains(int slots, const int* __restrict__ nexts, const unsigned char* __restrict__ evaluated,
                                                    const unsigned char* __restrict__ has_prev, unsigned char* __restrict__ absorbs, int pass_tag) {
    const int id4 = (blockIdx.x * kBlock + threadIdx.x) * kIpPer;
    if (id4 >= slots) return;
    const uint32_t heads = ip_match4(ip_flags4(evaluated, id4, slots), pass_tag) & ~ip_match4(ip_flags4(has_prev, id4, slots), pass_tag);
    if (!heads) return;
    for (int c = 0; c < 4; c++) {
        if (!(heads & (1u << (8 * c)))) continue;
        int cur = id4 + c, pos = 0;
        for (;;) {
            const int nxt = evaluated[cur] == pass_tag ? nexts[cur] : -1;
            if (nxt < 0) break;
            if (!(pos & 1)) absorbs[cur] = (unsigned char)pass_tag;
            cur = nxt; pos++;
        }
    }
}

__global__ void __launch_bounds__(kBlock) ip_tile_sums(const unsigned char* __restrict__ absorbs, int pass_tag, const Int2* __restrict__ minfo, int slots,
                                                       Int2* __restrict__ sums, int* __restrict__ removed) {
    __shared__ int lds[kWaves];
    const int id4 = (blockIdx.x * kBlock + threadIdx.x) * kIpPer;
    int need = 0, merges = 0, gone = 0;
    if (id4 < slots) {
        const uint32_t m = ip_match4(ip_flags4(absorbs, id4, slots), pass_tag);
        for (int c = 0; c < 4; c++) if (m & (1u << (8 * c))) { const Int2 v = minfo[id4 + c]; need += v.a; merges++; gone += v.b; }
    }
    need = block_sum(need, lds); merges = block_sum(merges, lds); gone = block_sum(gone, lds);
    if (threadIdx.x == 0) { sums[blockIdx.x] = Int2{need, merges}; removed[blockIdx.x] = gone; }
}

__global__ void __launch_bounds__(kBlock) ip_apply(void* cells, int* list_end, int* refs, const unsigned char* __restrict__ absorbs, int pass_tag,
                                                   const Int2* __restrict__ minfo, const int* __restrict__ nexts, const Int2* __restrict__ tile_prefix,
                                                   int slots, int* __restrict__ books, const Int2* __restrict__ pass_total, int capacity, int axis) {
    __shared__ int lds[kWaves];
    const int id4 = (blockIdx.x * kBlock + threadIdx.x) * kIpPer;
    const int* cursor = books;
    const int overflow = __hip_atomic_load(books + 3, __ATOMIC_RELAXED, __HIP_MEMORY_SCOPE_AGENT);
    if (overflow > 0 || (long long)*cursor + pass_total->a > (long long)capacity) {
        if (id4 == 0 && overflow <= 0) __hip_atomic_store(books + 3, -(1 + axis), __ATOMIC_RELAXED, __HIP_MEMORY_SCOPE_AGENT);
        return;
    }
    const uint32_t mine = id4 < slots ? ip_match4(ip_flags4(absorbs, id4, slots), pass_tag) : 0u;
    int m[4], total = 0;
    for (int c = 0; c < 4; c++) { m[c] = (mine & (1u << (8 * c))) ? minfo[id4 + c].a : 0; total += m[c]; }
    const int incl = wave_inclusive_scan(total);
    if (lane_id() == 63) lds[wave_id()] = incl;
    __syncthreads();
    if (!mine) return;
    int at = *cursor + tile_prefix[blockIdx.x].a + incl - total;
    for (int w = 0; w < wave_id(); w++) at += lds[w];
    for (int c = 0; c < 4; c++) {
        if (!(mine & (1u << (8 * c)))) continue;
        const int id = id4 + c, other = nexts[id];
        const CellRec a = ip_load(cells, list_end, id), n = ip_load(cells, list_end, other);
        write_union(refs + a.begin, a.end - a.begin, refs + n.begin, n.end - n.begin, refs + at, m[c]);
        CellFmt<true>::store(cells, id, min(n.lo, a.lo), at, max(n.hi, a.hi), 0);
        list_end[id] = at + m[c];
        reinterpret_cast<uint4*>(cells)[other] = make_uint4(kTombLo, 0u, 0u, uint32_t(id));
        at += m[c];
    }
}

__global__ void __launch_bounds__(kBlock) ip_mark(MergeK k, const Entry* __restrict__ entries, const void* __restrict__ cells, const unsigned char* __restrict__ absorbs,
                                                  int pass_tag, int slots, unsigned char* __restrict__ dirty, const Int2* __restrict__ pass_total,
                                                  const int* __restrict__ removed, int num_tiles, int* __restrict__ books ,
                                                  int* __restrict__ snap, size_t dstride) {
    __shared__ int lds[kWaves];
    const int id4 = (blockIdx.x * kBlock + threadIdx.x) * kIpPer;
    const int overflow = books[3];
    if (blockIdx.x == 0) {
        int gone = 0;
        for (int i = threadIdx.x; i < num_tiles; i += kBlock) gone += removed[i];
        gone = block_sum(gone, lds);
        if (threadIdx.x == 0) {
            if (overflow == 0) { books[0] += pass_total->a; books[1] -= pass_total->b; books[2] -= gone; }
            else if (overflow < 0) books[3] = -overflow;
            snap[0] = books[1]; snap[1] = books[2];
        }
    }
    __shared__ int list[kIpTile];
    __shared__ int count;
    const uint32_t mine = (overflow == 0 && id4 < slots) ? ip_match4(ip_flags4(absorbs, id4, slots), pass_tag) : 0u;
    const int n = ip_compact_tile(mine, id4, list, &count);
    for (int i = threadIdx.x; i < n; i += kBlock) {
        const int id = list[i];
        const CellRec cell = CellFmt<true>::load(cells, id);
        for (int axis = 0; axis < 3; axis++) {
            dirty[size_t(axis) * dstride + id] = 1;
            ivec3 p = cell.lo;
            if (axis == 0) p.x--; else if (axis == 1) p.y--; else p.z--;
            if (comp(p, axis) < 0) continue;
            dirty[size_t(axis) * dstride + ip_live(cells, int(lookup_entry(entries, k.shift, k.top, p)))] = 1;
        }
    }
}

__global__ void __launch_bounds__(kBlock) ip_live_sums(const void* __restrict__ cells, const int* __restrict__ list_end, int slots, Int2* __restrict__ sums, int num_tiles) {
    const int tile = blockIdx.x * kWaves + wave_id();
    if (tile >= num_tiles) return;
    Int2 s{0, 0};
    for (int c = 0; c < 4; c++) {
        const int i = tile * kMergeTile + c * 64 + lane_id();
        if (i < slots) {
            const uint4 v = reinterpret_cast<const uint4*>(cells)[i];
            if (!ip_is_tomb(v)) s = s + Int2{1, list_end[i] - int(v.w)};
        }
    }
    s = Int2{wave_sum(s.a), wave_sum(s.b)};
    if (lane_id() == 0) sums[tile] = s;
}
__global__ void __launch_bounds__(kBlock) ip_compact(const void* __restrict__ cells, const int* __restrict__ list_end, const int* __restrict__ refs, int slots,
                                                     const Int2* __restrict__ tile_prefix, Cell* __restrict__ out_cells, int* __restrict__ out_refs, int* __restrict__ new_ids) {
    __shared__ Int2 lds[kWaves];
    const int id = blockIdx.x * kBlock + threadIdx.x;
    uint4 v = make_uint4(kTombLo, 0u, 0u, 0u);
    if (id < slots) v = reinterpret_cast<const uint4*>(cells)[id];
    const bool live = id < slots && !ip_is_tomb(v);
    const int end = live ? list_end[id] : 0;
    const Int2 item = live ? Int2{1, end - int(v.w)} : Int2{0, 0};
    const Int2 incl = wave_inclusive_scan(item);
    if (lane_id() == 63) lds[wave_id()] = incl;
    __syncthreads();
    if (id >= slots) return;
    if (!live) { new_ids[id] = -1 - int(v.w); return; }
    Int2 at = tile_prefix[blockIdx.x];
    for (int w = 0; w < wave_id(); w++) at = at + lds[w];
    const int new_id = at.a + incl.a - 1, nb = at.b + incl.b - item.b;
    const CellRec c = CellFmt<true>::load(cells, id);
    CellFmt<false>::store(out_cells, new_id, c.lo, nb, c.hi, nb + item.b);
    for (int i = 0; i < item.b; i++) out_refs[nb + i] = refs[c.begin + i];
    new_ids[id] = new_id;
}
__global__ void __launch_bounds__(kBlock) ip_resolve_tombs(int* __restrict__ new_ids, int slots) {
    const int id = blockIdx.x * kBlock + threadIdx.x;
    if (id >= slots) return;
    int v = new_ids[id];
    if (v >= 0) return;
    int cur = -1 - v;
    for (;;) {
        const int w = __hip_atomic_load(new_ids + cur, __ATOMIC_RELAXED, __HIP_MEMORY_SCOPE_AGENT);
        if (w >= 0) { v = w; break; }
        cur = -1 - w;
    }
    new_ids[id] = v;
}

__global__ void __launch_bounds__(kBlock) widen_cells_kernel(const void* __restrict__ narrow, Cell* __restrict__ cells, const Int2* __restrict__ totals) {
    const int id = blockIdx.x * kBlock + threadIdx.x;
    if (id >= totals->a) return;
    CellRec c = CellFmt<true>::load(narrow, id);
    CellFmt<true>::finish(narrow, id, c);
    CellFmt<false>::store(cells, id, c.lo, c.begin, c.hi, c.end);
}

__global__ void __launch_bounds__(kBlock) remap_entries_kernel(uint32_t* __restrict__ entries, const int* __restrict__ new_cell_ids, int num_entries) {
    const int id = (blockIdx.x * kBlock + threadIdx.x) * 4;
    if (id >= num_entries) return;
    auto remap = [&](uint32_t e) { return (e & 3u) == 0 ? uint32_t(new_cell_ids[e >> 2]) << 2 : e; };
    if (id + 4 <= num_entries && lb_aligned16(entries + id)) {
        uint4* p = reinterpret_cast<uint4*>(entries + id);
        const uint4 e = *p;
        *p = make_uint4(remap(e.x), remap(e.y), remap(e.z), remap(e.w));
    } else {
        for (int i = id; i < min(id + 4, num_entries); i++) entries[i] = remap(entries[i]);
    }
}

}

extern "C" int hagrid_merge_grid(hagrid_ctx* ctx, hagrid_grid* grid, float alpha) {
    if (!ctx || !grid) return HAGRID_EINVAL;
    if (!grid->cells || !grid->entries || !grid->ref_ids) HG_FAIL(ctx, HAGRID_EINVAL, "merge_grid: incomplete (or compressed) grid");
    trav_image_drop(ctx);
    ctx->counts.merge_passes = 0;
    ctx->counts.merged_cells = grid->num_cells; ctx->counts.merged_refs = grid->num_refs;
    if (!(alpha > 0)) return HAGRID_OK;
    HG_HIP(ctx, hipSetDevice(ctx->device));
    hipStream_t st = ctx->stream;

    MergeK k;
    k.top = ivec3(grid->dims[0], grid->dims[1], grid->dims[2]);
    k.dims = k.top << grid->shift;
    k.shift = grid->shift;
    k.cell_size = (vec3(grid->bbox_max[0], grid->bbox_max[1], grid->bbox_max[2]) - vec3(grid->bbox_min[0], grid->bbox_min[1], grid->bbox_min[2])) / vec3(k.dims);

    const size_t nc0 = size_t(grid->num_cells), nr0 = size_t(grid->num_refs);
    Cell* cells_b = pool_alloc<Cell>(ctx, nc0);
    int* refs_b = pool_alloc<int>(ctx, nr0);
    int* merge_counts = pool_alloc<int>(ctx, nc0 + 1);
    int* nexts = pool_alloc<int>(ctx, nc0 + 1);
    unsigned char* prevs = pool_alloc<unsigned char>(ctx, nc0 + 4);
    unsigned char* cell_flags = pool_alloc<unsigned char>(ctx, nc0 + 4);
    const size_t stamp_stride = (nc0 + 4 + 255) & ~size_t(255);
    unsigned char* stamps = pool_alloc<unsigned char>(ctx, 2 * stamp_stride);
    unsigned char* stamps_other = stamps ? stamps + stamp_stride : nullptr;
    unsigned char* const stamps_base = stamps;
    const int max_tiles = grid_blocks(grid->num_cells, kMergeTile);
    Int2* tile_sums = pool_alloc<Int2>(ctx, size_t(max_tiles) + 1);
    Int2* partials = pool_alloc<Int2>(ctx, size_t(scan_num_tiles(max_tiles)) + 1);
    Int2* total = reinterpret_cast<Int2*>(ctx->dscratch);
    auto release = [&]() {
        hagrid_mem_free(ctx, merge_counts); hagrid_mem_free(ctx, nexts); hagrid_mem_free(ctx, prevs); hagrid_mem_free(ctx, cell_flags);
        hagrid_mem_free(ctx, tile_sums); hagrid_mem_free(ctx, partials); hagrid_mem_free(ctx, stamps_base);
    };
    if (!cells_b || !refs_b || !merge_counts || !nexts || !prevs || !cell_flags || !tile_sums || !partials || !stamps) {
        release(); hagrid_mem_free(ctx, cells_b); hagrid_mem_free(ctx, refs_b);
        return HAGRID_ENOMEM;
    }

    void* cells = grid->cells;
    void* cells_other = cells_b;
    int* refs = static_cast<int*>(grid->ref_ids);
    uint32_t* entries = static_cast<uint32_t*>(grid->entries);
    int num_cells = grid->num_cells, num_refs = grid->num_refs;
    const int num_entries = grid->num_entries;
    const bool narrow = ctx->opt_merge_narrow && std::max(k.dims.x, std::max(k.dims.y, k.dims.z)) < 65536;

    int rc = HAGRID_OK;
    int prev_num_cells = 0, iter = 0, pass_tag = 0;
    bool in_narrow = false;
    (void)hipMemsetAsync(prevs, 0, nc0, st);
    hagrid_build_counts& bc = ctx->counts;
    auto record = [&](int c, int r) {
        if (bc.merge_passes < HAGRID_MAX_MERGE_PASSES) { bc.merge_cells[bc.merge_passes] = c; bc.merge_refs[bc.merge_passes] = r; bc.merge_passes++; }
    };

    int global_pass = 0;
    bool have_stamps = false;
    int since[3] = {0, 0, 0};
    bool in_place = false;
    int ip_slots = 0, ip_iters = 0, prev_mask = 0;
    int* list_end = merge_counts;
    Int2* minfo = nullptr; unsigned char* dirty = nullptr; unsigned char* evaluated = nullptr;
    int* books = ctx->dscratch + 16;
    int* snap = ctx->dscratch + 20;
    Int2* ip_total = reinterpret_cast<Int2*>(ctx->dscratch + 26);
    int* tile_removed = nullptr;
    const int ip_capacity = int(std::min<size_t>(nr0, 0x7fffffff));
    size_t ip_dstride = 0;
    auto ip_enter = [&]() -> bool {
        const auto r256 = [](size_t n) { return (n + 255) & ~size_t(255); };
        const size_t slots = size_t(num_cells), dstride = r256(slots);
        const size_t off_dirty = r256(slots * 8), off_eval = off_dirty + 3 * dstride, off_removed = off_eval + r256(slots);
        if (off_removed + r256(size_t(grid_blocks(num_cells, kIpTile)) * sizeof(int)) > nc0 * sizeof(Cell)) return false;
        ip_slots = num_cells; ip_dstride = dstride;
        char* scratch = static_cast<char*>(cells_other);
        minfo = reinterpret_cast<Int2*>(scratch);
        dirty = reinterpret_cast<unsigned char*>(scratch + off_dirty);
        evaluated = reinterpret_cast<unsigned char*>(scratch + off_eval);
        tile_removed = reinterpret_cast<int*>(scratch + off_removed);
        const unsigned char* stp = have_stamps ? stamps : nullptr;
        ip_begin<<<grid_blocks(ip_slots, kBlock), kBlock, 0, st>>>(cells, ip_slots, list_end, dirty, stp, since[0], since[1], since[2],
                                                                   evaluated, cell_flags , books, num_refs, ip_dstride); HG_DBG(ctx);
        if (stp) ip_mark_entry<<<grid_blocks(ip_slots, kIpTile), kBlock, 0, st>>>(k, reinterpret_cast<const Entry*>(entries), cells, ip_slots, dirty, stp, since[0], since[1], since[2], ip_dstride); HG_DBG(ctx);
        in_place = true;
        return true;
    };
    auto ip_leave = [&]() -> int {
        const int tiles = grid_blocks(ip_slots, kMergeTile);
        ip_live_sums<<<grid_blocks(tiles, kWaves), kBlock, 0, st>>>(cells, list_end, ip_slots, tile_sums, tiles); HG_DBG(ctx);
        if (!ctx_scan<Int2>(ctx, SumsIn{tile_sums}, SumsOut{tile_sums}, tiles, partials, (const Int2*)nullptr, ip_total)) return HAGRID_ENOMEM;
        ip_compact<<<tiles, kBlock, 0, st>>>(cells, list_end, refs, ip_slots, tile_sums, static_cast<Cell*>(cells_other), refs_b, nexts); HG_DBG(ctx);
        ip_resolve_tombs<<<grid_blocks(ip_slots, kBlock), kBlock, 0, st>>>(nexts, ip_slots); HG_DBG(ctx);
        remap_entries_kernel<<<grid_blocks((num_entries + 3) / 4, kBlock), kBlock, 0, st>>>(entries, nexts, num_entries); HG_DBG(ctx);
        std::swap(cells, cells_other);
        std::swap(refs, refs_b);
        int h[2];
        HG_TRY(read_back(ctx, ip_total, h, sizeof(h)));
        if (h[0] != num_cells) return fail(ctx, HAGRID_EHIP, __FILE__, __LINE__, "merge_grid: the books of the in-place iterations do not add up");
        num_refs = h[1];
        in_place = false; in_narrow = false; ip_iters = 0;
        have_stamps = false;
        return HAGRID_OK;
    };
    int last_pass_in = 0, last_pass_out = 0;
    auto compacting_passes = [&](int first_axis, int mask) -> int {
        for (int axis = first_axis; axis < 3; axis++) {
            const int blocks = grid_blocks(num_cells, kBlock);
            Int2* tot = total + axis;
            const int* n_dev = axis > first_axis ? &total[axis - 1].a : nullptr;
            const Entry* ent = reinterpret_cast<const Entry*>(entries);
            if (++pass_tag == 256) { pass_tag = 1; (void)hipMemsetAsync(prevs, 0, nc0, st); }
            if (in_narrow) merge_counts_kernel<true><<<blocks, kBlock, 0, st>>>(axis, k, ent, cells, refs, merge_counts, nexts, prevs, pass_tag, mask, num_cells, n_dev);
            else           merge_counts_kernel<false><<<blocks, kBlock, 0, st>>>(axis, k, ent, cells, refs, merge_counts, nexts, prevs, pass_tag, mask, num_cells, n_dev);
            HG_DBG(ctx);
            cell_flags_kernel<<<grid_blocks((num_cells + 3) / 4, kBlock), kBlock, 0, st>>>(nexts, prevs, pass_tag, cell_flags, num_cells, n_dev); HG_DBG(ctx);
            const int tiles = grid_blocks(num_cells, kMergeTile);
            merge_tile_sums<<<grid_blocks(tiles, kWaves), kBlock, 0, st>>>(cell_flags, merge_counts, num_cells, n_dev, tile_sums, tiles); HG_DBG(ctx);
            if (!ctx_scan<Int2>(ctx, SumsIn{tile_sums}, SumsOut{tile_sums}, tiles, partials, (const Int2*)nullptr, tot)) return HAGRID_ENOMEM;
            global_pass++;
            const bool stamping = global_pass < 250 && (have_stamps || global_pass == 1);
            const unsigned char* st_in = stamping && have_stamps ? stamps : nullptr;
            unsigned char* st_out = stamping ? stamps_other : nullptr;
            if (in_narrow)   merge_kernel<true, true><<<tiles, kBlock, 0, st>>>(axis, k, ent, cells, refs, cell_flags, tile_sums, merge_counts, nexts, cells_other, refs_b, num_cells, n_dev, tot, st_in, st_out, global_pass);
            else if (narrow) merge_kernel<false, true><<<tiles, kBlock, 0, st>>>(axis, k, ent, cells, refs, cell_flags, tile_sums, merge_counts, nexts, cells_other, refs_b, num_cells, n_dev, tot, st_in, st_out, global_pass);
            else             merge_kernel<false, false><<<tiles, kBlock, 0, st>>>(axis, k, ent, cells, refs, cell_flags, tile_sums, merge_counts, nexts, cells_other, refs_b, num_cells, n_dev, tot, st_in, st_out, global_pass);
            HG_DBG(ctx);
            have_stamps = stamping; since[axis] = global_pass;
            std::swap(stamps, stamps_other);
            in_narrow = narrow;
            remap_entries_kernel<<<grid_blocks((num_entries + 3) / 4, kBlock), kBlock, 0, st>>>(entries, nexts, num_entries); HG_DBG(ctx);
            std::swap(cells, cells_other);
            std::swap(refs, refs_b);
        }
        int h[6];
        HG_TRY(read_back(ctx, total, h, sizeof(int) * 6));
        for (int axis = first_axis; axis < 3; axis++) {
            record(num_cells, num_refs);
            if (axis == 2) { last_pass_in = num_cells; last_pass_out = h[4]; }
            num_cells = h[2 * axis]; num_refs = h[2 * axis + 1];
        }
        return HAGRID_OK;
    };

    do {
        prev_num_cells = num_cells;
        const int mask = iter > 3 ? 0 : (1 << (iter + 1)) - 1;
        if (in_place && ctx->opt_merge_inplace_iters > 0 && ip_iters >= ctx->opt_merge_inplace_iters) {
            rc = ip_leave();
            if (rc != HAGRID_OK) break;
        }
        int first_compacting_axis = 0;
        if (in_place) {
            if (prev_mask & ~mask) (void)hipMemsetAsync(dirty, 1, 3 * ip_dstride, st);
            const int blocks = grid_blocks(ip_slots, kIpTile), tiles = blocks;
            const Entry* ent = reinterpret_cast<const Entry*>(entries);
            for (int axis = 0; axis < 3 && rc == HAGRID_OK; axis++) {
                global_pass++;
                if (++pass_tag == 256) {
                    pass_tag = 1;
                    (void)hipMemsetAsync(prevs, 0, nc0, st); (void)hipMemsetAsync(evaluated, 0, size_t(ip_slots), st); (void)hipMemsetAsync(cell_flags, 0, size_t(ip_slots), st);
                }
                ip_counts<<<blocks, kBlock, 0, st>>>(axis, k, ent, cells, list_end, refs, ip_slots, dirty + size_t(axis) * ip_dstride, minfo, nexts, evaluated, prevs, pass_tag, mask); HG_DBG(ctx);
                ip_chains<<<blocks, kBlock, 0, st>>>(ip_slots, nexts, evaluated, prevs, cell_flags, pass_tag); HG_DBG(ctx);
                ip_tile_sums<<<tiles, kBlock, 0, st>>>(cell_flags, pass_tag, minfo, ip_slots, tile_sums, tile_removed); HG_DBG(ctx);
                if (!ctx_scan<Int2>(ctx, SumsIn{tile_sums}, SumsOut{tile_sums}, tiles, partials, (const Int2*)nullptr, ip_total)) { rc = HAGRID_ENOMEM; break; }
                ip_apply<<<tiles, kBlock, 0, st>>>(cells, list_end, refs, cell_flags, pass_tag, minfo, nexts, tile_sums, ip_slots, books, ip_total,
                                                    ctx->opt_merge_inplace_room > 0 ? std::min(ip_capacity, ctx->opt_merge_inplace_room) : ip_capacity, axis); HG_DBG(ctx);
                ip_mark<<<blocks, kBlock, 0, st>>>(k, ent, cells, cell_flags, pass_tag, ip_slots, dirty, ip_total, tile_removed, tiles, books, snap + 2 * axis, ip_dstride); HG_DBG(ctx);
            }
            if (rc != HAGRID_OK) break;
            int h[10];
            rc = read_back(ctx, books, h, sizeof(h));
            if (rc != HAGRID_OK) break;
            const int applied = h[3] > 0 ? h[3] - 1 : 3;
            for (int axis = 0; axis < applied; axis++) { record(num_cells, num_refs); num_cells = h[4 + 2 * axis]; num_refs = h[5 + 2 * axis]; }
            ip_iters++;
            if (applied < 3) {
                rc = ip_leave();
                if (rc != HAGRID_OK) break;
                first_compacting_axis = applied;
            }
        }
        if (!in_place) {
            if (first_compacting_axis < 3) rc = compacting_passes(first_compacting_axis, mask);
            if (rc != HAGRID_OK) break;
            const int div = ctx->opt_merge_inplace_div > 0 ? ctx->opt_merge_inplace_div : 2;
            if (in_narrow && ctx->opt_merge_inplace && (long long)div * (prev_num_cells - num_cells) < prev_num_cells && num_cells < alpha * prev_num_cells) (void)ip_enter();
        }
        prev_mask = mask;
        iter++;
    } while (rc == HAGRID_OK && num_cells < alpha * prev_num_cells);
    if (rc == HAGRID_OK && in_place) rc = ip_leave();
    else if (rc == HAGRID_OK && in_narrow) {
        widen_cells_kernel<<<grid_blocks(num_cells, kBlock), kBlock, 0, st>>>(cells, static_cast<Cell*>(cells_other), total + 2); HG_DBG(ctx);
        std::swap(cells, cells_other);
    }

    if (rc == HAGRID_OK) {
        hipError_t e = hipGetLastError();
        if (e != hipSuccess) rc = fail(ctx, HAGRID_EHIP, __FILE__, __LINE__, hipGetErrorString(e));
    }
    release();
    hagrid_mem_free(ctx, cells_other);
    hagrid_mem_free(ctx, refs_b);
    if (rc != HAGRID_OK) {
        (void)hipStreamSynchronize(st);
        hagrid_mem_free(ctx, cells); hagrid_mem_free(ctx, refs);
        grid->cells = nullptr; grid->ref_ids = nullptr; grid->num_cells = 0; grid->num_refs = 0;
        return rc;
    }
    grid->cells = cells; grid->ref_ids = refs;
    grid->num_cells = num_cells; grid->num_refs = num_refs;
    ctx->counts.merged_cells = num_cells; ctx->counts.merged_refs = num_refs;
    return rc;
}
```

hagrid_amd/csrc/wave_prims.h:

```cpp
#pragma once
#include "ctx.h"

#include <hip/hip_runtime.h>
#include <stdint.h>

#include <algorithm>

namespace hagrid_impl {

constexpr int kBlock = 256;
constexpr int kWaves = kBlock / 64;
constexpr int kScanItems = 8;
constexpr int kScanTile = kBlock * kScanItems;

__device__ __forceinline__ int lane_id() { return threadIdx.x & 63; }
__device__ __forceinline__ int wave_id() { return threadIdx.x >> 6; }

#ifndef HG_XCD_CHUNK_LOG2
#define HG_XCD_CHUNK_LOG2 6
#endif
constexpr int kXcdChunkLog2 = HG_XCD_CHUNK_LOG2;
__device__ __forceinline__ int xcd_block(int b, int nb) {
    if (kXcdChunkLog2 < 0) return b;
    const int full = (nb >> (kXcdChunkLog2 + 3)) << (kXcdChunkLog2 + 3);
// ... 56 lines not shown
}
__device__ __forceinline__ float wave_max_f(float v) {
#pragma unroll
    for (int d = 32; d > 0; d >>= 1) { float o = __shfl_xor(v, d, 64); v = o > v ? o : v; }
    return v;
}

__device__ __forceinline__ int block_sum(int v, int* lds) {
    v = wave_sum(v);
    __syncthreads();
    if (lane_id() == 0) lds[wave_id()] = v;
    __syncthreads();
    int r = 0;
#pragma unroll
    for (int w = 0; w < kWaves; w++) r += lds[w];
    return r;
}

__device__ __forceinline__ int wave_append(int n, int* counter) {
    const int incl = wave_inclusive_scan(n);
    const int total = __shfl(incl, 63, 64);
    int base = 0;
    if (lane_id() == 63 && total > 0) base = atomicAdd(counter, total);
    base = __shfl(base, 63, 64);
    return base + incl - n;
}


template <typename V, typename In>
__global__ void __launch_bounds__(kBlock) scan_partials(In in, int n, V* partials) {
    __shared__ V lds[kWaves];
    const int base = blockIdx.x * kScanTile;
    V s = zero_of(V());
#pragma unroll
    for (int j = 0; j < kScanItems; j++) {
        const int i = base + j * kBlock + threadIdx.x;
        if (i < n) s = s + in(i);
    }
    s = wave_inclusive_scan(s);
    if (lane_id() == 63) lds[wave_id()] = s;
    __syncthreads();
    if (threadIdx.x == 0) {
        V t = lds[0];
        for (int w = 1; w < kWaves; w++) t = t + lds[w];
        partials[blockIdx.x] = t;
    }
}

template <typename V>
__global__ void __launch_bounds__(kBlock) scan_spine(V* partials, int num_partials, const V* carry_in, V* total_out) {
    __shared__ V lds[kWaves];
    __shared__ V running;
    if (threadIdx.x == 0) running = carry_in ? *carry_in : zero_of(V());
    __syncthreads();
    for (int base = 0; base < num_partials; base += kBlock) {
        const int i = base + threadIdx.x;
        const V v = i < num_partials ? partials[i] : zero_of(V());
        const V incl = wave_inclusive_scan(v);
        if (lane_id() == 63) lds[wave_id()] = incl;
        __syncthreads();
        V excl = running;
        for (int w = 0; w < wave_id(); w++) excl = excl + lds[w];
        const V prev = shfl_up_v(incl, 1);
        if (lane_id() > 0) excl = excl + prev;
        if (i < num_partials) partials[i] = excl;
        __syncthreads();
        if (threadIdx.x == 0) {
            V t = running;
            for (int w = 0; w < kWaves; w++) t = t + lds[w];
            running = t;
        }
        __syncthreads();
    }
    if (threadIdx.x == 0 && total_out) *total_out = running;
}

template <typename V, typename In, typename Out>
__global__ void __launch_bounds__(kBlock) scan_apply(In in, Out out, int n, const V* partials) {
    __shared__ V lds[kWaves];
    __shared__ V running;
    if (threadIdx.x == 0) running = partials[blockIdx.x];
    __syncthreads();
    const int base = blockIdx.x * kScanTile;
#pragma unroll 1
    for (int j = 0; j < kScanItems; j++) {
        const int i = base + j * kBlock + threadIdx.x;
        if (base + j * kBlock >= n) break;
        const V v = i < n ? in(i) : zero_of(V());
        const V incl = wave_inclusive_scan(v);
        if (lane_id() == 63) lds[wave_id()] = incl;
        __syncthreads();
        V excl = running;
        for (int w = 0; w < wave_id(); w++) excl = excl + lds[w];
        const V prev = shfl_up_v(incl, 1);
        if (lane_id() > 0) excl = excl + prev;
        if (i < n) out(i, excl);
        __syncthreads();
        if (threadIdx.x == 0) {
            V t = running;
            for (int w = 0; w < kWaves; w++) t = t + lds[w];
            running = t;
        }
        __syncthreads();
    }
}

constexpr int kLbVec = 4;
constexpr int kLbItems = 8;
constexpr int kLbWindows = 4;
constexpr int kLbTile = kBlock * kLbItems;
constexpr unsigned kLbAggregate = 1u, kLbPrefix = 2u;

__device__ __forceinline__ unsigned long long lb_pack(unsigned epoch, unsigned flag, int value) {
    return ((unsigned long long)epoch << 34) | ((unsigned long long)flag << 32) | (unsigned)value;
}
__device__ __forceinline__ void lb_store(unsigned long long* p, unsigned long long w) {
    __hip_atomic_store(p, w, __ATOMIC_RELAXED, __HIP_MEMORY_SCOPE_AGENT);
}
__device__ __forceinline__ unsigned long long lb_load(const unsigned long long* p) {
    return __hip_atomic_load(p, __ATOMIC_RELAXED, __HIP_MEMORY_SCOPE_AGENT);
}
__device__ __forceinline__ void lb_publish(unsigned long long* state, int tile, unsigned epoch, unsigned flag, int v) { lb_store(state + tile, lb_pack(epoch, flag, v)); }
__device__ __forceinline__ void lb_publish(unsigned long long* state, int tile, unsigned epoch, unsigned flag, Int2 v) {
    lb_store(state + 2 * size_t(tile), lb_pack(epoch, flag, v.a));
    lb_store(state + 2 * size_t(tile) + 1, lb_pack(epoch, flag, v.b));
}
__device__ __forceinline__ unsigned lb_wait(const unsigned long long* state, int t, unsigned epoch, int& v) {
    unsigned long long w;
    do { w = lb_load(state + t); } while ((unsigned)(w >> 34) != epoch || ((w >> 32) & 3u) == 0u);
    v = int(unsigned(w));
    return unsigned(w >> 32) & 3u;
}
__device__ __forceinline__ unsigned lb_wait(const unsigned long long* state, int t, unsigned epoch, Int2& v) {
    int a, b;
    unsigned fa, fb;
    do {
        fa = lb_wait(state, 2 * t, epoch, a);
        fb = lb_wait(state, 2 * t + 1, epoch, b);
    } while (fa != fb);
    v = Int2{a, b};
    return fa;
}
__device__ __forceinline__ bool lb_try(const unsigned long long* state, int t, unsigned epoch, int& v, unsigned& flag) {
    const unsigned long long w = lb_load(state + t);
    v = int(unsigned(w)); flag = unsigned(w >> 32) & 3u;
    return (unsigned)(w >> 34) == epoch && flag != 0u;
}
__device__ __forceinline__ bool lb_try(const unsigned long long* state, int t, unsigned epoch, Int2& v, unsigned& flag) {
    const unsigned long long a = lb_load(state + 2 * size_t(t)), b = lb_load(state + 2 * size_t(t) + 1);
    v = Int2{int(unsigned(a)), int(unsigned(b))}; flag = unsigned(a >> 32) & 3u;
    return (unsigned)(a >> 34) == epoch && (unsigned)(b >> 34) == epoch && flag != 0u && flag == (unsigned(b >> 32) & 3u);
}
template <typename V> constexpr int lb_words() { return int(sizeof(V) / sizeof(int)); }

__device__ __forceinline__ bool lb_aligned16(const void* p) { return (reinterpret_cast<uintptr_t>(p) & 15u) == 0; }
template <typename V, typename In> __device__ __forceinline__ auto lb_load_row(const In& in, int i, int n, V* v, int) -> decltype(in.load4(i, n, v), void()) { in.load4(i, n, v); }
template <typename V, typename In> __device__ __forceinline__ void lb_load_row(const In& in, int i, int n, V* v, long) {
#pragma unroll
    for (int c = 0; c < kLbVec; c++) v[c] = i + c < n ? in(i + c) : zero_of(V());
}
template <typename V, typename Out> __device__ __forceinline__ auto lb_store_row(const Out& out, int i, int n, const V* v, int) -> decltype(out.store4(i, n, v), void()) { out.store4(i, n, v); }
template <typename V, typename Out> __device__ __forceinline__ void lb_store_row(const Out& out, int i, int n, const V* v, long) {
#pragma unroll
    for (int c = 0; c < kLbVec; c++) if (i + c < n) out(i + c, v[c]);
}

template <typename V, typename In, typename Out>
__global__ void __launch_bounds__(kBlock) scan_lookback(In in, Out out, int n, int tiles, unsigned long long* state, unsigned epoch, unsigned help_after, const V* carry_in, V* total_out) {
    __shared__ V lds[kWaves];
    __shared__ V tile_prefix;
    constexpr int kWaveItems = kLbItems * 64, kRows = kLbItems / kLbVec;
    for (int tile = blockIdx.x; tile < tiles; tile += gridDim.x) {
        const int base = tile * kLbTile + wave_id() * kWaveItems + lane_id() * kLbVec;
        V v[kLbItems];
#pragma unroll
        for (int r = 0; r < kRows; r++) lb_load_row<V>(in, base + r * 64 * kLbVec, n, v + r * kLbVec, 0);
        V run = zero_of(V());
#pragma unroll
        for (int r = 0; r < kRows; r++) {
            V mine = zero_of(V());
#pragma unroll
            for (int c = 0; c < kLbVec; c++) { const V x = v[r * kLbVec + c]; v[r * kLbVec + c] = mine; mine = mine + x; }
            const V incl = wave_inclusive_scan(mine);
            const V before = shfl_up_v(incl, 1);
            const V lane_off = lane_id() > 0 ? run + before : run;
#pragma unroll
            for (int c = 0; c < kLbVec; c++) v[r * kLbVec + c] = v[r * kLbVec + c] + lane_off;
            run = run + V(shfl_v(incl, 63));
        }
        __syncthreads();
        if (lane_id() == 0) lds[wave_id()] = run;
        __syncthreads();
        if (wave_id() == 0) {
            V agg = lds[0];
            for (int w = 1; w < kWaves; w++) agg = agg + lds[w];
            V excl = zero_of(V());
            if (tile == 0) {
                if (carry_in) excl = *carry_in;
            } else {
                if (lane_id() == 0) lb_publish(state, tile, epoch, kLbAggregate, agg);
                int p = tile - 1;
                for (;;) {
                    V pv[kLbWindows];
                    unsigned flag[kLbWindows];
                    bool ok[kLbWindows];
#pragma unroll
                    for (int w = 0; w < kLbWindows; w++) {
                        pv[w] = zero_of(V()); flag[w] = kLbPrefix;
                        ok[w] = p - w * 64 - lane_id() < 0;
                    }
                    for (unsigned polls = 0;; polls++) {
                        bool all = true;
#pragma unroll
                        for (int w = 0; w < kLbWindows; w++) {
                            if (!ok[w]) {
                                ok[w] = lb_try(state, p - w * 64 - lane_id(), epoch, pv[w], flag[w]);
                                if (!ok[w] && polls >= help_after) {
                                    const int t = p - w * 64 - lane_id();
                                    const int first = t * kLbTile, last = min(n, first + kLbTile);
                                    V sum = zero_of(V());
                                    for (int i = first; i < last; i++) sum = sum + in(i);
                                    if (t == 0 && carry_in) sum = sum + *carry_in;
                                    pv[w] = sum; flag[w] = t == 0 ? kLbPrefix : kLbAggregate; ok[w] = true;
                                    __builtin_amdgcn_fence(__ATOMIC_ACQUIRE, "agent");
                                    V pub = zero_of(V()); unsigned pflag = 0u;
                                    if (lb_try(state, t, epoch, pub, pflag)) { pv[w] = pub; flag[w] = pflag; }
                                }
                            }
                            all = all && ok[w];
                        }
                        if (all) break;
                    }
                    unsigned long long is_prefix[kLbWindows];
#pragma unroll
                    for (int w = 0; w < kLbWindows; w++) is_prefix[w] = __ballot(flag[w] == kLbPrefix);
                    bool found = false;
#pragma unroll
                    for (int w = 0; w < kLbWindows; w++) {
                        if (found) break;
                        const int first = __ffsll((long long)is_prefix[w]) - 1;
                        if (first < 0 || lane_id() <= first) excl = excl + pv[w];
                        found = first >= 0;
                    }
                    if (found) break;
                    p -= 64 * kLbWindows;
                }
#pragma unroll
                for (int d = 32; d > 0; d >>= 1) excl = excl + V(shfl_xor_v(excl, d));
            }
            if (lane_id() == 0) {
                lb_publish(state, tile, epoch, kLbPrefix, excl + agg);
#if !defined(__gfx950__) && !defined(__gfx942__) && !defined(__gfx90a__) && defined(__HIP_DEVICE_COMPILE__)
#error "scan_lookback: the in-place ordering relies on gfx9's vmcnt counting stores; use a release fence on this target"
#endif
                asm volatile("s_waitcnt vmcnt(0)" ::: "memory");
                tile_prefix = excl;
                if (total_out && tile == tiles - 1) *total_out = excl + agg;
            }
        }
        __syncthreads();
        V offset = tile_prefix;
        for (int w = 0; w < wave_id(); w++) offset = offset + lds[w];
#pragma unroll
        for (int r = 0; r < kRows; r++) {
#pragma unroll
            for (int c = 0; c < kLbVec; c++) v[r * kLbVec + c] = offset + v[r * kLbVec + c];
            lb_store_row<V>(out, base + r * 64 * kLbVec, n, v + r * kLbVec, 0);
        }
    }
    if (tiles == 0 && blockIdx.x == 0 && threadIdx.x == 0 && total_out) *total_out = carry_in ? *carry_in : zero_of(V());
}

inline int scan_num_tiles(int n) { return (n + kScanTile - 1) / kScanTile; }

template <typename V, typename In, typename Out>
inline void device_scan_lookback(hipStream_t stream, int num_cus, In in, Out out, int n, unsigned long long* state, unsigned epoch, unsigned help_after, const V* carry_in, V* total_out) {
    static const int per_cu = [] {
        int n = 0;
        if (hipOccupancyMaxActiveBlocksPerMultiprocessor(&n, scan_lookback<V, In, Out>, kBlock, 0) != hipSuccess) { (void)hipGetLastError(); n = 2; }
        return std::max(1, std::min(n - 1, 8));
    }();
    const int tiles = (n + kLbTile - 1) / kLbTile;
    const int blocks = std::max(1, std::min(tiles, std::max(num_cus, 1) * per_cu));
    scan_lookback<V, In, Out><<<blocks, kBlock, 0, stream>>>(in, out, n, tiles, state, epoch, help_after, carry_in, total_out);
}

template <typename V, typename In, typename Out>
inline void device_scan(hipStream_t stream, In in, Out out, int n, V* partials, const V* carry_in, V* total_out) {
    const int tiles = scan_num_tiles(n);
    if (tiles > 0) scan_partials<V, In><<<tiles, kBlock, 0, stream>>>(in, n, partials);
    scan_spine<V><<<1, kBlock, 0, stream>>>(partials, tiles, carry_in, total_out);
    if (tiles > 0) scan_apply<V, In, Out><<<tiles, kBlock, 0, stream>>>(in, out, n, partials);
}

template <typename V, typename In, typename Out>
inline bool ctx_scan(hagrid_ctx* ctx, In in, Out out, int n, V* partials, const V* carry_in, V* total_out) {
#ifdef HG_SCAN_THREE_KERNELS
    if (!ctx->opt_lookback) { device_scan<V>(ctx->stream, in, out, n, partials, carry_in, total_out); HG_DBG(ctx); return true; }
#endif
    unsigned epoch = 0;
    unsigned long long* state = lookback_state(ctx, scan_num_tiles(n), lb_words<V>(), &epoch);
    if (!state) return false;
    device_scan_lookback<V>(ctx->stream, ctx->num_cus, in, out, n, state, epoch, ctx->opt_lookback == 2 ? 0u : 4096u, carry_in, total_out);
    HG_DBG(ctx);
    return true;
}

}
```

hagrid_amd/lib.py:

```python
from __future__ import annotations

import ctypes as C
import os

HERE = os.path.dirname(os.path.abspath(__file__))
LIB_PATH = os.environ.get("HAGRID_AMD_LIB") or os.path.join(HERE, "libhagrid_amd.so")
MAX_LEVELS = 32
ABI_VERSION = 3

OK, EINVAL, EHIP, ENOMEM, ERANGE, ENODEV = 0, -1, -2, -3, -4, -5


class HagridError(RuntimeError):
    pass


class GridPOD(C.Structure):
    _fields_ = [("entries", C.c_void_p), ("ref_ids", C.c_void_p), ("cells", C.c_void_p), ("small_cells", C.c_void_p),
                ("bbox_min", C.c_float * 3), ("bbox_max", C.c_float * 3), ("dims", C.c_int32 * 3),
                ("num_cells", C.c_int32), ("num_entries", C.c_int32), ("num_refs", C.c_int32), ("shift", C.c_int32),
                ("num_offsets", C.c_int32), ("offsets", C.c_int32 * MAX_LEVELS)]


class TraversalStats(C.Structure):
    _fields_ = [(n, C.c_int64) for n in ("rays", "rays_hit_grid", "cells", "entry_words", "refs", "sentinels", "hits", "long_list_refs")]

    def as_dict(self):
        return {n: int(getattr(self, n)) for n, _ in self._fields_}


class Camera(C.Structure):
    _fields_ = [("eye", C.c_float * 3), ("dir", C.c_float * 3), ("right", C.c_float * 3), ("up", C.c_float * 3)]

    @classmethod
    def from_scene(cls, cam) -> "Camera":
        c = cls()
        for name, v in zip(("eye", "dir", "right", "up"), cam[:4]):
            for i in range(3):
                getattr(c, name)[i] = float(v[i])
        return c


class Mesh(C.Structure):
    _fields_ = [("vertices", C.c_void_p), ("indices", C.c_void_p), ("num_vertices", C.c_int32), ("num_tris", C.c_int32),
                ("vertex_stride", C.c_int32), ("reserved", C.c_int32)]


MAX_MERGE_PASSES = 96


class BlobHeader(C.Structure):
    _fields_ = [("magic", C.c_uint32), ("version", C.c_uint32), ("dims", C.c_int32 * 3), ("shift", C.c_int32),
                ("num_cells", C.c_int32), ("num_entries", C.c_int32), ("num_refs", C.c_int32), ("num_tris", C.c_int32),
                ("compressed", C.c_int32), ("num_offsets", C.c_int32), ("offsets", C.c_int32 * MAX_LEVELS),
                ("bbox_min", C.c_float * 3), ("bbox_max", C.c_float * 3),
                ("off_entries", C.c_uint64), ("off_cells", C.c_uint64), ("off_refs", C.c_uint64), ("off_tris", C.c_uint64), ("total_bytes", C.c_uint64),
                ("reserved", C.c_uint8 * 16)]


class BuildCounts(C.Structure):
    _fields_ = [("num_tris", C.c_int64), ("top_cells", C.c_int64), ("top_refs", C.c_int64),
                ("num_levels", C.c_int32), ("merge_passes", C.c_int32), ("expand_passes", C.c_int32), ("compressed", C.c_int32),
                ("level_refs", C.c_int64 * MAX_LEVELS), ("level_cells", C.c_int64 * MAX_LEVELS), ("level_kept", C.c_int64 * MAX_LEVELS),
                ("build_cells", C.c_int64), ("build_refs", C.c_int64), ("build_entries", C.c_int64),
                ("merge_cells", C.c_int64 * MAX_MERGE_PASSES), ("merge_refs", C.c_int64 * MAX_MERGE_PASSES),
                ("merged_cells", C.c_int64), ("merged_refs", C.c_int64),
                ("flatten_entries_in", C.c_int64), ("flatten_entries_out", C.c_int64),
                ("expand_cells", C.c_int64), ("compress_cells", C.c_int64), ("compress_refs_out", C.c_int64)]

    def as_dict(self) -> dict:
        d = {}
        for n, t in self._fields_:
            v = getattr(self, n)
            d[n] = int(v) if not hasattr(v, "__len__") else [int(x) for x in v]
        d["level_refs"] = d["level_refs"][:d["num_levels"]]; d["level_cells"] = d["level_cells"][:d["num_levels"]]
        d["level_kept"] = d["level_kept"][:d["num_levels"]]
        d["merge_cells"] = d["merge_cells"][:d["merge_passes"]]; d["merge_refs"] = d["merge_refs"][:d["merge_passes"]]
        return d


_vp, _i32, _i64, _f32, _sz = C.c_void_p, C.c_int, C.c_int64, C.c_float, C.c_size_t
SIGNATURES = {
    "hagrid_abi_version": (_i32, []),
    "hagrid_debug_sync_enabled": (_i32, []),
    "hagrid_ctx_create": (_i32, [C.POINTER(_vp), _i32, _i32]),
    "hagrid_ctx_destroy": (None, [_vp]),
    "hagrid_ctx_set_stream": (_i32, [_vp, _vp]),
    "hagrid_last_error": (C.c_char_p, [_vp]),
    "hagrid_device_info": (_i32, [_vp, C.c_char_p, _i32, C.POINTER(_i32), C.POINTER(_i64)]),
    "hagrid_mem_alloc": (_vp, [_vp, _sz]),
    "hagrid_mem_free": (_i32, [_vp, _vp]),
    "hagrid_mem_copy_h2d": (_i32, [_vp, _vp, _vp, _sz]),
    "hagrid_mem_copy_d2h": (_i32, [_vp, _vp, _vp, _sz]),
    "hagrid_mem_copy_d2d": (_i32, [_vp, _vp, _vp, _sz]),
    "hagrid_mem_zero": (_i32, [_vp, _vp, _sz]),
    "hagrid_mem_one": (_i32, [_vp, _vp, _sz]),
    "hagrid_mem_usage": (_sz, [_vp]),
    "hagrid_mem_max_usage": (_sz, [_vp]),
    "hagrid_mem_debug_slots": (None, [_vp]),
    "hagrid_bandwidth_probe": (_i32, [_vp, _sz, _i32, C.POINTER(_f32), C.POINTER(_f32)]),
    "hagrid_get_build_counts": (_i32, [_vp, C.POINTER(BuildCounts)]),
    "hagrid_profile_begin": (_i32, [_vp]),
    "hagrid_profile_end": (_f32, [_vp]),
    "hagrid_build_grid": (_i32, [_vp, _vp, _i32, C.POINTER(GridPOD), _f32, _f32]),
    "hagrid_merge_grid": (_i32, [_vp, C.POINTER(GridPOD), _f32]),
    "hagrid_flatten_grid": (_i32, [_vp, C.POINTER(GridPOD)]),
    "hagrid_expand_grid": (_i32, [_vp, C.POINTER(GridPOD), _vp, _i32]),
    "hagrid_compress_grid": (_i32, [_vp, C.POINTER(GridPOD)]),
    "hagrid_grid_blob_bytes": (_sz, [C.POINTER(GridPOD), _i32]),
    "hagrid_grid_pack": (_i32, [_vp, C.POINTER(GridPOD), _vp, _i32, C.POINTER(_vp), C.POINTER(_sz)]),
    "hagrid_grid_unpack": (_i32, [_vp, _vp, _sz, C.POINTER(GridPOD), C.POINTER(_vp), C.POINTER(_i32)]),
    "hagrid_grid_save": (_i32, [_vp, C.POINTER(GridPOD), _vp, _i32, C.c_char_p]),
    "hagrid_grid_load": (_i32, [_vp, C.c_char_p, C.POINTER(GridPOD), C.POINTER(_vp), C.POINTER(_i32)]),
    "hagrid_grid_broadcast": (_i32, [_vp, _vp, _i32, _i32, C.POINTER(GridPOD), C.POINTER(_vp), C.POINTER(_i32)]),
    "hagrid_setup_traversal": (_i32, [_vp, C.POINTER(GridPOD)]),
    "hagrid_grid_release_for_traversal": (_i32, [_vp, C.POINTER(GridPOD)]),
    "hagrid_share_traversal": (_i32, [_vp, _vp]),
    "hagrid_ctx_synchronize": (_i32, [_vp]),
    "hagrid_traverse_grid": (_i32, [_vp, C.POINTER(GridPOD), _vp, _vp, _vp, _i32]),
    "hagrid_traverse_grid_ex": (_i32, [_vp, C.POINTER(GridPOD), _vp, _vp, _vp, _i32, C.c_uint32]),
    "hagrid_traverse_grid_stats": (_i32, [_vp, C.POINTER(GridPOD), _vp, _vp, _vp, _i32, _vp, C.POINTER(TraversalStats)]),
    "hagrid_traverse_grid_multi": (_i32, [_vp, C.POINTER(GridPOD), _vp, _vp, _vp, _i32, _i32, C.c_uint32]),
    "hagrid_closest_points": (_i32, [_vp, C.POINTER(GridPOD), _vp, _vp, _vp, _i32, _vp, C.c_uint32]),
    "hagrid_overlap_boxes": (_i32, [_vp, C.POINTER(GridPOD), _vp, _vp, _i32, _i32, _vp, _vp, _vp, C.c_uint32]),
    "hagrid_overlap_lattice": (_i32, [_vp, C.POINTER(GridPOD), _vp, C.POINTER(C.c_float), C.POINTER(C.c_float), C.POINTER(C.c_int), _i32, _vp, _vp, _vp, C.c_uint32]),
    "hagrid_count_crossings": (_i32, [_vp, C.POINTER(GridPOD), _vp, _vp, _vp, _i32, _vp, C.c_uint32]),
    "hagrid_list_crossings": (_i32, [_vp, C.POINTER(GridPOD), _vp, _vp, _i32, _vp, _i32, _vp, _i64, _vp, _vp, C.c_uint32]),
    "hagrid_points_inside": (_i32, [_vp, C.POINTER(GridPOD), _vp, _vp, _i32, C.POINTER(C.c_float), _i32, _vp, _vp, _vp, C.c_uint32]),
    "hagrid_inside_lattice": (_i32, [_vp, C.POINTER(GridPOD), _vp, C.POINTER(C.c_float), C.POINTER(C.c_float), C.POINTER(C.c_int), C.POINTER(C.c_float), _i32, _vp, _vp, _vp, C.c_uint32]),
    "hagrid_set_ray_binning": (_i32, [_vp, _i32]),
    "hagrid_set_option": (_i32, [_vp, C.c_char_p, _i32]),
    "hagrid_traversal_image_info": (_i32, [_vp, C.POINTER(GridPOD), _vp, C.POINTER(_i64)]),
    "hagrid_gen_primary_rays": (_i32, [_vp, C.POINTER(Camera), _f32, _i32, _i32, _i64, _i32, _vp]),
    "hagrid_gen_bounce_rays": (_i32, [_vp, _vp, _vp, _vp, _i32, C.c_uint64, C.c_uint64, C.POINTER(_f32), C.POINTER(_f32), _f32, C.c_uint32, _vp]),
    "hagrid_shade_hits": (_i32, [_vp, _vp, _i32, _i32, _f32, _vp]),
    "hagrid_shade_layers": (_i32, [_vp, _vp, _i32, _i32, _f32, _f32, _vp]),
    "hagrid_accumulate_occlusion": (_i32, [_vp, _vp, _i32, _vp]),
    "hagrid_shade_occlusion": (_i32, [_vp, _vp, _vp, _i32, _i32, _vp]),
    "hagrid_frame_workspace_bytes": (_sz, [_i32, _i32, _i32]),
    "hagrid_render_frame": (_i32, [_vp, C.POINTER(GridPOD), _vp, C.POINTER(Camera), _f32, _i32, _i32, _i32, _i32, _f32, C.c_uint64, _vp, _vp]),
    "hagrid_scene_create": (_i32, [_vp, C.POINTER(Mesh), _i32, C.POINTER(C.c_int32), _i32, C.POINTER(_vp)]),
    "hagrid_scene_destroy": (None, [_vp, _vp]),
    "hagrid_scene_first_tri": (_i32, [_vp, _i32]),
    "hagrid_scene_assemble": (_i32, [_vp, _vp, _vp, _vp, _vp]),
    "hagrid_scene_bad_indices": (_i32, [_vp, _vp, C.POINTER(_i64)]),
}

KAT_LIB_PATH = os.path.join(HERE, "libhagrid_amd_kat.so")
KAT_SIGNATURES = {
    "hagrid_kat_intersect_prim_ray": (_i32, [_vp, _vp, _vp, _vp, _i32, _vp, _vp, _vp]),
    "hagrid_kat_intersect_prim_ray_uvs": (_i32, [_vp, _vp, _vp, _vp, _i32, _vp, _vp, _vp, _vp, _vp]),
    "hagrid_kat_intersect_prim_cell": (_i32, [_vp, _vp, _vp, _vp, _i32, _vp]),
    "hagrid_kat_compute_range": (_i32, [_vp, _vp, _vp, _vp, _i32, _vp]),
    "hagrid_kat_compute_grid_dims": (_i32, [_vp, _vp, _vp, _vp, _i32, _vp]),
    "hagrid_kat_lookup_entry": (_i32, [_vp, _vp, _i32, _i32, _vp, _vp, _i32, _vp]),
    "hagrid_kat_scan": (_i32, [_vp, _vp, _i32, _i32, _vp, _i32, _vp, _vp]),
    "hagrid_kat_set_option": (_i32, [_vp, C.c_char_p, _i32]),
    "hagrid_kat_order_state": (_i32, [_vp, _vp, _vp, _vp]),
    "hagrid_kat_forget_hints": (_i32, [_vp]),
    "hagrid_kat_detect_ray_rows": (_i32, [_vp, _vp, _i32, C.c_float, _vp]),
    "hagrid_kat_image_records": (_i32, [_vp, _vp, _vp, _i32, _vp, _vp]),
    "hagrid_kat_tile_slots": (_i32, [_vp, _i32, _i32, _i32, _i32, _vp]),
    "hagrid_kat_bin_rays": (_i32, [_vp, _vp, _vp, _vp, _i32, _i32, _vp, _vp, _vp]),
    "hagrid_kat_tile_order": (_i32, [_vp, _vp, _i32, _i32, _i32, _vp, _i32, _vp, _vp, _vp, _vp]),
    "hagrid_kat_traverse_timed": (_i32, [_vp, C.POINTER(GridPOD), _vp, _vp, _vp, _i32, _i32, _i32, _vp, _vp]),
}

_lib = None
_kat = None


def _preload_hip_runtime() -> None:
    candidates = []
    try:
        import torch
        candidates.append(os.path.join(os.path.dirname(torch.__file__), "lib", "libamdhip64.so"))
    except Exception:
        pass
    candidates += ["/opt/rocm/lib/libamdhip64.so", "libamdhip64.so"]
    last = None
    for c in candidates:
        try:
            C.CDLL(c, mode=C.RTLD_GLOBAL)
            return
        except OSError as e:
            last = e
    raise HagridError(f"no HIP runtime (libamdhip64.so) could be loaded: {last}")


def load() -> C.CDLL:
    global _lib
    if _lib is not None:
        return _lib
    if not os.path.exists(LIB_PATH):
        raise HagridError(f"{LIB_PATH} is missing: run `python -c 'import __graft_entry__ as g; g.build()'` "
                          "(or python hagrid_amd/build.py).  There is no CPU fallback.")
    _preload_hip_runtime()
    try:
        lib = C.CDLL(LIB_PATH)
    except OSError as e:
        raise HagridError(f"cannot load {LIB_PATH}: {e}") from e
    for name, (res, args) in SIGNATURES.items():
        fn = getattr(lib, name)
        fn.restype = res
        fn.argtypes = args
    if lib.hagrid_abi_version() != ABI_VERSION:
        raise HagridError("ABI version mismatch")
    _lib = lib
    return lib


def load_kat() -> C.CDLL:
    global _kat
    if _kat is not None:
        return _kat
    load()
    if os.path.realpath(LIB_PATH) != os.path.realpath(os.path.join(HERE, "libhagrid_amd.so")):
        raise HagridError(f"HAGRID_AMD_LIB={LIB_PATH} overrides the product library, but {KAT_LIB_PATH} is built against its sibling "
                          f"{os.path.join(HERE, 'libhagrid_amd.so')}: the test hooks (known-answer tests, code-path selectors) cannot be used in an A/B run")
    if not os.path.exists(KAT_LIB_PATH):
        raise HagridError(f"{KAT_LIB_PATH} is missing: run `python -c 'import __graft_entry__ as g; g.build()'`")
    try:
        lib = C.CDLL(KAT_LIB_PATH)
    except OSError as e:
        raise HagridError(f"cannot load {KAT_LIB_PATH}: {e}") from e
    for name, (res, args) in KAT_SIGNATURES.items():
        fn = getattr(lib, name)
        fn.restype = res
        fn.argtypes = args
    _kat = lib
    return lib
```

Baseline: 7684.

## Fuse host readbacks into producing kernels and drop end-of-pass stream syncs

Small device-to-host readbacks (bbox, scan totals, merge books) are now published straight to a host-mapped mailbox by the kernel that produces them, instead of launching a separate publish kernel afterwards. The end-of-pass hipStreamSynchronize calls in build, expand, flatten and compress are replaced by a check that only reports launch errors, and later syncs pick up any deferred async errors. This targets host launch and sync latency in grid build. The cost is extra complexity in the error reporting, and more work is left queued asynchronously when a pass returns.

```diff
diff --git a/hagrid_amd/csrc/build.hip b/hagrid_amd/csrc/build.hip
--- a/hagrid_amd/csrc/build.hip
+++ b/hagrid_amd/csrc/build.hip
@@ -67,7 +67,7 @@
         reinterpret_cast<int*>(partials)[blockIdx.x * kBoxWords + 6] = v;
     }
 }
-__global__ void __launch_bounds__(kBlock) bbox_final(const float* __restrict__ partials, int num, float* __restrict__ out) {
+__global__ void __launch_bounds__(kBlock) bbox_final(const float* __restrict__ partials, int num, float* __restrict__ out, Publish pub) {
     __shared__ float lds[kWaves][6];
     __shared__ int lds_bad[kWaves];
     float v[6] = { FLT_MAX, FLT_MAX, FLT_MAX, -FLT_MAX, -FLT_MAX, -FLT_MAX };
@@ -85,10 +85,17 @@
         float r = lds[0][threadIdx.x];
         for (int w = 1; w < kWaves; w++) r = threadIdx.x < 3 ? min(r, lds[w][threadIdx.x]) : max(r, lds[w][threadIdx.x]);
         out[threadIdx.x] = r;
+        if (pub.n > 0) pub.dst[threadIdx.x] = __float_as_int(r);
     } else if (threadIdx.x == 6) {
         int r = lds_bad[0];
         for (int w = 1; w < kWaves; w++) r = min(r, lds_bad[w]);
         reinterpret_cast<int*>(out)[6] = r;
+        if (pub.n > 0) pub.dst[6] = r;
+    }
+    if (pub.n > 0 && wave_id() == 0) {
+        __threadfence_system();
+        __builtin_amdgcn_wave_barrier();
+        if (threadIdx.x == 0) __hip_atomic_store(pub.flag, pub.epoch, __ATOMIC_RELEASE, __HIP_MEMORY_SCOPE_SYSTEM);
     }
 }
 
@@ -820,13 +827,14 @@
     const int total_cells = int(total_cells_ll);
     Int2* const part2 = nullptr;
     Int2* carry = reinterpret_cast<Int2*>(dsc + 128);
+    int hf[2];
+    const Publish leaf_pub = read_back_begin(ctx, carry + (num_levels - 1), sizeof(hf));
     for (int l = 0; l < num_levels; l++) {
         GLevel& V = levels[l];
         if (!ctx_scan<Int2>(ctx, LeafIn{V.entries, V.cell_counts}, LeafOut{V.start_cell, V.ref_begin}, V.num_cells, part2,
-                            l ? carry + (l - 1) : (const Int2*)nullptr, carry + l)) return HAGRID_ENOMEM;
-    }
-    int hf[2];
-    HG_TRY(read_back(ctx, carry + (num_levels - 1), hf, sizeof(hf)));
+                            l ? carry + (l - 1) : (const Int2*)nullptr, carry + l, l == num_levels - 1 ? leaf_pub : Publish())) return HAGRID_ENOMEM;
+    }
+    HG_TRY(read_back_wait(ctx, leaf_pub, carry + (num_levels - 1), hf, sizeof(hf)));
     const int new_total_cells = hf[0], total_refs = hf[1];
     if (new_total_cells <= 0 || total_refs < 0) HG_FAIL(ctx, HAGRID_ERANGE, "build_grid: inconsistent totals");
 
@@ -842,8 +850,7 @@
         concat_level<<<grid_blocks(V.num_cells, kBlock), kBlock, 0, st>>>(V.entries, V.cells, V.cell_counts, V.start_cell, V.ref_begin, V.num_cells, off,
                                                                                   V.refs, V.seg_begin, V.num_refs, l == 0 ? 1 : 0, out_cells, out_entries, out_refs); HG_DBG(ctx);
     }
-    hipError_t e = hipGetLastError();
-    if (e == hipSuccess) e = hipStreamSynchronize(st);
+    const hipError_t e = pass_end(ctx);
     if (e != hipSuccess) {
         hagrid_mem_free(ctx, out_cells); hagrid_mem_free(ctx, out_entries); hagrid_mem_free(ctx, out_refs);
         HG_FAIL(ctx, HAGRID_EHIP, hipGetErrorString(e));
@@ -883,9 +890,10 @@
     if (!bb_part) return HAGRID_ENOMEM;
     float* bb_out = bb_part + size_t(bb_blocks) * kBoxWords;
     bbox_partials<<<bb_blocks, kBlock, 0, st>>>(tris, num_tris, bb_part); HG_DBG(ctx);
-    bbox_final<<<1, kBlock, 0, st>>>(bb_part, bb_blocks, bb_out); HG_DBG(ctx);
-    float hb[8];
-    HG_TRY(read_back(ctx, bb_out, hb, sizeof(hb)));
+    float hb[8] = {};
+    const Publish box_pub = read_back_begin(ctx, bb_out, 7 * sizeof(float));
+    bbox_final<<<1, kBlock, 0, st>>>(bb_part, bb_blocks, bb_out, box_pub); HG_DBG(ctx);
+    HG_TRY(read_back_wait(ctx, box_pub, bb_out, hb, 7 * sizeof(float)));
     int bad_tri; memcpy(&bad_tri, &hb[6], sizeof(int));
     if (bad_tri != kNoBadTri) {
         char msg[96];
diff --git a/hagrid_amd/csrc/compress.hip b/hagrid_amd/csrc/compress.hip
--- a/hagrid_amd/csrc/compress.hip
+++ b/hagrid_amd/csrc/compress.hip
@@ -60,8 +60,7 @@
     if (!srefs) { hagrid_mem_free(ctx, partials); hagrid_mem_free(ctx, small); return HAGRID_ENOMEM; }
     scan_apply<int, SentinelIn, SmallCellOut><<<std::max(scan_num_tiles(n), 1), kBlock, 0, st>>>(
         SentinelIn{cells}, SmallCellOut{cells, static_cast<const int*>(grid->ref_ids), small, srefs}, n, partials); HG_DBG(ctx);
-    hipError_t e = hipGetLastError();
-    if (e == hipSuccess) e = hipStreamSynchronize(st);
+    const hipError_t e = pass_end(ctx);
     hagrid_mem_free(ctx, partials);
     ctx->counts.compressed = 1; ctx->counts.compress_cells = n; ctx->counts.compress_refs_out = h;
     if (e != hipSuccess) { hagrid_mem_free(ctx, small); hagrid_mem_free(ctx, srefs); HG_FAIL(ctx, HAGRID_EHIP, hipGetErrorString(e)); }
diff --git a/hagrid_amd/csrc/ctx.h b/hagrid_amd/csrc/ctx.h
--- a/hagrid_amd/csrc/ctx.h
+++ b/hagrid_amd/csrc/ctx.h
@@ -141,7 +141,8 @@
     hagrid_impl::TravImageCache image;
     unsigned image_serial = 0;
     int readback_epoch = 0;
-    int opt_fast_readback = 1;
+    int opt_fast_readback = 2;
+    int async_err = 0;
     int build_arena_tris = 0;
     size_t build_arena_hint = 0;
     hagrid_build_counts counts = {};
@@ -206,7 +207,32 @@
 
 int pool_split(hagrid_ctx* ctx, void* base, void* const* parts, int n);
 
+
+int stream_sync(hagrid_ctx* ctx, const char* file, int line);
+#define HG_SYNC(ctx) HG_TRY(::hagrid_impl::stream_sync((ctx), __FILE__, __LINE__))
+void stream_sync_quiet(hagrid_ctx* ctx);
+hipError_t pass_end(hagrid_ctx* ctx);
+
+struct Publish { const int* src = nullptr; int n = 0; int* dst = nullptr; int* flag = nullptr; int epoch = 0; };
 int read_back(hagrid_ctx* ctx, const void* dptr, void* hptr, size_t bytes);
+Publish read_back_begin(hagrid_ctx* ctx, const void* dptr, size_t bytes);
+int read_back_wait(hagrid_ctx* ctx, const Publish& pub, const void* dptr, void* hptr, size_t bytes);
+
+#if defined(__HIPCC__)
+__device__ __forceinline__ void publish_from_wave(const Publish& pub, const int* own_at, int own0, int own1, int n_own) {
+    if (pub.n <= 0) return;
+    const int lane = int(__lane_id());
+    if (lane < pub.n) {
+        int v = pub.src[lane];
+        const long d = (pub.src + lane) - own_at;
+        if (own_at && d >= 0 && d < n_own) v = d == 0 ? own0 : own1;
+        pub.dst[lane] = v;
+    }
+    __threadfence_system();
+    __builtin_amdgcn_wave_barrier();
+    if (lane == 0) __hip_atomic_store(pub.flag, pub.epoch, __ATOMIC_RELEASE, __HIP_MEMORY_SCOPE_SYSTEM);
+}
+#endif
 
 inline int grid_blocks(long long n, int block) { return (int)((n + block - 1) / block); }
 
diff --git a/hagrid_amd/csrc/ctx.hip b/hagrid_amd/csrc/ctx.hip
--- a/hagrid_amd/csrc/ctx.hip
+++ b/hagrid_amd/csrc/ctx.hip
@@ -57,15 +57,15 @@
     hipStream_t next = static_cast<hipStream_t>(stream);
     if (next == ctx->stream) return HAGRID_OK;
     HG_HIP(ctx, hipSetDevice(ctx->device));
-    HG_HIP(ctx, hipStreamSynchronize(ctx->stream));
+    const int rc = stream_sync(ctx, __FILE__, __LINE__);
     ctx->stream = next;
-    return HAGRID_OK;
+    return rc;
 }
 
 extern "C" int hagrid_ctx_synchronize(hagrid_ctx* ctx) {
     if (!ctx) return HAGRID_EINVAL;
     HG_HIP(ctx, hipSetDevice(ctx->device));
-    HG_HIP(ctx, hipStreamSynchronize(ctx->stream));
+    HG_SYNC(ctx);
     return HAGRID_OK;
 }
 
@@ -89,7 +89,7 @@
 
 
 static void release_slot_memory(hagrid_ctx* ctx, Slot& s) {
-    if (s.ptr) (void)hipFree(s.ptr);
+    if (s.ptr) { stream_sync_quiet(ctx); (void)hipFree(s.ptr); }
     ctx->usage -= s.size;
     s.ptr = nullptr;
     s.size = 0;
@@ -159,10 +159,7 @@
     ctx->tracker.erase(it);
     if (--s.refs > 0) return HAGRID_OK;
     s.in_use = false;
-    if (!ctx->keep) {
-        HG_HIP(ctx, hipStreamSynchronize(ctx->stream));
-        release_slot_memory(ctx, s);
-    }
+    if (!ctx->keep) release_slot_memory(ctx, s);
     return HAGRID_OK;
 }
 
@@ -172,7 +169,7 @@
     trav_image_source_touched(ctx, dst, bytes);
     HG_HIP(ctx, hipSetDevice(ctx->device));
     HG_HIP(ctx, hipMemcpyAsync(dst, src, bytes, hipMemcpyHostToDevice, ctx->stream));
-    HG_HIP(ctx, hipStreamSynchronize(ctx->stream));
+    HG_SYNC(ctx);
     return HAGRID_OK;
 }
 extern "C" int hagrid_mem_copy_d2h(hagrid_ctx* ctx, void* dst, const void* src, size_t bytes) {
@@ -180,7 +177,7 @@
     if (!bytes) return HAGRID_OK;
     HG_HIP(ctx, hipSetDevice(ctx->device));
     HG_HIP(ctx, hipMemcpyAsync(dst, src, bytes, hipMemcpyDeviceToHost, ctx->stream));
-    HG_HIP(ctx, hipStreamSynchronize(ctx->stream));
+    HG_SYNC(ctx);
     return HAGRID_OK;
 }
 extern "C" int hagrid_mem_copy_d2d(hagrid_ctx* ctx, void* dst, const void* src, size_t bytes) {
@@ -292,7 +289,7 @@
 unsigned long long* hagrid_impl::lookback_state(hagrid_ctx* ctx, int tiles, int words_per_tile, unsigned* epoch) {
     const size_t need = size_t(tiles > 0 ? tiles : 1) * size_t(words_per_tile);
     if (need > ctx->lb_words || ctx->lb_epoch >= (1u << 30) - 2u) {
-        (void)hipStreamSynchronize(ctx->stream);
+        stream_sync_quiet(ctx);
         if (need > ctx->lb_words) {
             if (ctx->lb_state) (void)hipFree(ctx->lb_state);
             ctx->lb_state = nullptr; ctx->lb_words = 0;
@@ -307,6 +304,29 @@
     return ctx->lb_state;
 }
 
+int hagrid_impl::stream_sync(hagrid_ctx* ctx, const char* file, int line) {
+    hipError_t e = hipStreamSynchronize(ctx->stream);
+    if (e == hipSuccess && ctx->async_err) e = hipError_t(ctx->async_err);
+    ctx->async_err = 0;
+    if (e != hipSuccess) return fail(ctx, HAGRID_EHIP, file, line, hipGetErrorString(e));
+    return HAGRID_OK;
+}
+
+void hagrid_impl::stream_sync_quiet(hagrid_ctx* ctx) {
+    const hipError_t e = hipStreamSynchronize(ctx->stream);
+    if (e != hipSuccess && !ctx->async_err) ctx->async_err = int(e);
+}
+
+hipError_t hagrid_impl::pass_end(hagrid_ctx* ctx) {
+    hipError_t e = hipGetLastError();
+#ifdef HAGRID_DEBUG_SYNC
+    if (e == hipSuccess) e = hipStreamSynchronize(ctx->stream);
+#else
+    (void)ctx;
+#endif
+    return e;
+}
+
 void hagrid_impl::debug_sync(hagrid_ctx* ctx, const char* file, int line) {
     hipError_t e = hipStreamSynchronize(ctx->stream);
     if (e == hipSuccess) e = hipGetLastError();
@@ -333,31 +353,49 @@
 }
 }
 
+static int await_words(hagrid_ctx* ctx, int epoch, void* hptr, size_t bytes) {
+    int* flag = ctx->mailbox + kMbxReadBackEpoch;
+    const auto t0 = std::chrono::steady_clock::now();
+    for (unsigned spins = 0;; spins++) {
+        if (__atomic_load_n(flag, __ATOMIC_ACQUIRE) == epoch) break;
+        if ((spins & 1023u) == 1023u && std::chrono::steady_clock::now() - t0 > std::chrono::milliseconds(20)) {
+            HG_SYNC(ctx);
+            if (__atomic_load_n(flag, __ATOMIC_ACQUIRE) != epoch) HG_FAIL(ctx, HAGRID_EHIP, "read_back: the words never arrived");
+            break;
+        }
+    }
+    memcpy(hptr, ctx->mailbox, bytes);
+    return HAGRID_OK;
+}
+
 int hagrid_impl::read_back(hagrid_ctx* ctx, const void* dptr, void* hptr, size_t bytes) {
     if (ctx->opt_fast_readback && bytes > 0 && bytes <= 256 * sizeof(int) && (bytes & 3u) == 0 && (reinterpret_cast<uintptr_t>(dptr) & 3u) == 0) {
-        int* flag = ctx->mailbox + kMbxReadBackEpoch;
         const int epoch = ++ctx->readback_epoch;
-        publish_words<<<1, 256, 0, ctx->stream>>>(static_cast<const int*>(dptr), int(bytes / 4), ctx->mailbox, flag, epoch);
+        publish_words<<<1, 256, 0, ctx->stream>>>(static_cast<const int*>(dptr), int(bytes / 4), ctx->mailbox, ctx->mailbox + kMbxReadBackEpoch, epoch);
         HG_HIP(ctx, hipGetLastError());
-        const auto t0 = std::chrono::steady_clock::now();
-        for (unsigned spins = 0;; spins++) {
-            if (__atomic_load_n(flag, __ATOMIC_ACQUIRE) == epoch) break;
-            if ((spins & 1023u) == 1023u && std::chrono::steady_clock::now() - t0 > std::chrono::milliseconds(20)) {
-                HG_HIP(ctx, hipStreamSynchronize(ctx->stream));
-                if (__atomic_load_n(flag, __ATOMIC_ACQUIRE) != epoch) HG_FAIL(ctx, HAGRID_EHIP, "read_back: the words never arrived");
-                break;
-            }
-        }
-        memcpy(hptr, ctx->mailbox, bytes);
-        return HAGRID_OK;
+        return await_words(ctx, epoch, hptr, bytes);
     }
     if (bytes <= 256 * sizeof(int)) {
         HG_HIP(ctx, hipMemcpyAsync(ctx->mailbox, dptr, bytes, hipMemcpyDeviceToHost, ctx->stream));
-        HG_HIP(ctx, hipStreamSynchronize(ctx->stream));
+        HG_SYNC(ctx);
         memcpy(hptr, ctx->mailbox, bytes);
     } else {
         HG_HIP(ctx, hipMemcpyAsync(hptr, dptr, bytes, hipMemcpyDeviceToHost, ctx->stream));
-        HG_HIP(ctx, hipStreamSynchronize(ctx->stream));
-    }
-    return HAGRID_OK;
-}
+        HG_SYNC(ctx);
+    }
+    return HAGRID_OK;
+}
+
+hagrid_impl::Publish hagrid_impl::read_back_begin(hagrid_ctx* ctx, const void* dptr, size_t bytes) {
+    Publish pub;
+    if (ctx->opt_fast_readback < 2 || bytes == 0 || bytes > 64 * sizeof(int) || (bytes & 3u) != 0 || (reinterpret_cast<uintptr_t>(dptr) & 3u) != 0) return pub;
+    pub.src = static_cast<const int*>(dptr); pub.n = int(bytes / 4);
+    pub.dst = ctx->mailbox; pub.flag = ctx->mailbox + kMbxReadBackEpoch; pub.epoch = ++ctx->readback_epoch;
+    return pub;
+}
+
+int hagrid_impl::read_back_wait(hagrid_ctx* ctx, const Publish& pub, const void* dptr, void* hptr, size_t bytes) {
+    if (pub.n <= 0) return read_back(ctx, dptr, hptr, bytes);
+    HG_HIP(ctx, hipGetLastError());
+    return await_words(ctx, pub.epoch, hptr, bytes);
+}
diff --git a/hagrid_amd/csrc/expand.hip b/hagrid_amd/csrc/expand.hip
--- a/hagrid_amd/csrc/expand.hip
+++ b/hagrid_amd/csrc/expand.hip
@@ -289,8 +289,7 @@
             overlap_step<2, false><<<blocks, kBlock, 0, st>>>(k, entries, refs, tris, cells, other, flags, n); HG_DBG(ctx); std::swap(cells, other);
         }
     }
-    hipError_t e = hipGetLastError();
-    if (e == hipSuccess) e = hipStreamSynchronize(st);
+    const hipError_t e = pass_end(ctx);
     ctx->counts.expand_passes = 3 * iters; ctx->counts.expand_cells = n;
     hagrid_mem_free(ctx, flags);
     hagrid_mem_free(ctx, other);
diff --git a/hagrid_amd/csrc/flatten.hip b/hagrid_amd/csrc/flatten.hip
--- a/hagrid_amd/csrc/flatten.hip
+++ b/hagrid_amd/csrc/flatten.hip
@@ -100,13 +100,16 @@
     int* carry = ctx->dscratch;
     const int top_entries = grid->offsets[0];
     HG_HIP(ctx, hipMemcpyAsync(carry, &top_entries, sizeof(int), hipMemcpyHostToDevice, st));
+    const int num_groups = (shift + kFlatLevels - 1) / kFlatLevels;
+    const Publish pub = num_groups > 0 ? read_back_begin(ctx, carry, sizeof(int) * size_t(num_groups + 1)) : Publish();
     int groups = 0;
     for (int i = 0; i < shift; i += kFlatLevels, groups++) {
         const int first = first_of(i), num = grid->offsets[i] - first;
-        if (!ctx_scan<int>(ctx, BlockSizeIn{depths + first}, StartOut{start + first}, num, partials, carry + groups, carry + groups + 1)) { release(); return HAGRID_ENOMEM; }
+        if (!ctx_scan<int>(ctx, BlockSizeIn{depths + first}, StartOut{start + first}, num, partials, carry + groups, carry + groups + 1,
+                           groups == num_groups - 1 ? pub : Publish())) { release(); return HAGRID_ENOMEM; }
     }
     int h[HAGRID_MAX_LEVELS + 2];
-    int rc = read_back(ctx, carry, h, sizeof(int) * size_t(groups + 1));
+    int rc = read_back_wait(ctx, pub, carry, h, sizeof(int) * size_t(groups + 1));
     if (rc != HAGRID_OK) { release(); return rc; }
     const int total_entries = h[groups];
     if (total_entries < top_entries || total_entries > 0x3fffffff) { release(); HG_FAIL(ctx, HAGRID_ERANGE, "flatten_grid: voxel map too large"); }
@@ -121,8 +124,7 @@
         new_offsets[num_new++] = h[g];
     }
     new_offsets[num_new++] = total_entries;
-    hipError_t e = hipGetLastError();
-    if (e == hipSuccess) e = hipStreamSynchronize(st);
+    const hipError_t e = pass_end(ctx);
     if (e != hipSuccess) { release(); hagrid_mem_free(ctx, out); HG_FAIL(ctx, HAGRID_EHIP, hipGetErrorString(e)); }
     release();
     hagrid_mem_free(ctx, entries);
diff --git a/hagrid_amd/csrc/kat/hagrid_amd_kat.h b/hagrid_amd/csrc/kat/hagrid_amd_kat.h
--- a/hagrid_amd/csrc/kat/hagrid_amd_kat.h
+++ b/hagrid_amd/csrc/kat/hagrid_amd_kat.h
@@ -32,6 +32,7 @@
 int hagrid_kat_set_option(hagrid_ctx* ctx, const char* key, int value);
 
 int hagrid_kat_forget_hints(hagrid_ctx* ctx);
+int hagrid_kat_set_async_error(hagrid_ctx* ctx, int hip_error);
 int hagrid_kat_order_state(hagrid_ctx* ctx, const void* rays, int32_t* out12, float* ms4);
 
 #ifdef __cplusplus
diff --git a/hagrid_amd/csrc/kat/kat.hip b/hagrid_amd/csrc/kat/kat.hip
--- a/hagrid_amd/csrc/kat/kat.hip
+++ b/hagrid_amd/csrc/kat/kat.hip
@@ -320,7 +320,7 @@
     if (!ctx || !key) return HAGRID_EINVAL;
     struct { const char* name; int* dst; int lo, hi; } table[] = {
         {"traverse.variant", &ctx->opt_variant, 0, 4},              {"traverse.narrow", &ctx->opt_narrow, 0, 1},
-        {"traverse.image_uniform", &ctx->opt_image_uniform, 0, 2},  {"traverse.image_slim", &ctx->opt_image_slim, 1, 2}, {"traverse.image_general", &ctx->opt_image_general, 0, 2}, {"traverse.image_vtop", &ctx->opt_image_vtop, 0, 1}, {"traverse.quad_head", &ctx->opt_quad_head, 0, 1000}, {"ctx.fast_readback", &ctx->opt_fast_readback, 0, 1},
+        {"traverse.image_uniform", &ctx->opt_image_uniform, 0, 2},  {"traverse.image_slim", &ctx->opt_image_slim, 1, 2}, {"traverse.image_general", &ctx->opt_image_general, 0, 2}, {"traverse.image_vtop", &ctx->opt_image_vtop, 0, 1}, {"traverse.quad_head", &ctx->opt_quad_head, 0, 1000}, {"ctx.fast_readback", &ctx->opt_fast_readback, 0, 2},
         {"traverse.tail", &ctx->opt_tail, 0, 1},                    {"traverse.quad_tail", &ctx->opt_quad_tail, -1, 100},
         {"traverse.tail_dual", &ctx->opt_tail_dual, -1, 1},        
         {"traverse.super_tile", &ctx->opt_super_log2, 0, 8},        {"traverse.xcd_chunk", &ctx->opt_xcd_chunk_log2, -2, 16},
@@ -354,6 +354,12 @@
     return HAGRID_OK;
 }
 
+extern "C" int hagrid_kat_set_async_error(hagrid_ctx* ctx, int hip_error) {
+    if (!ctx || hip_error < 0) return HAGRID_EINVAL;
+    ctx->async_err = hip_error;
+    return HAGRID_OK;
+}
+
 extern "C" int hagrid_kat_forget_hints(hagrid_ctx* ctx) {
     if (!ctx) return HAGRID_EINVAL;
     for (auto& h : ctx->hints) { h.key_rays = nullptr; h.key_n = 0; h.used = 0; h.lpt_rays = nullptr; h.lpt_valid = false; h.rowlen_rays = nullptr; h.rowlen_seen = 0; h.share_ncand = 0; h.share_shape_nc = 0; h.share_choice = -1; }
diff --git a/hagrid_amd/csrc/merge.hip b/hagrid_amd/csrc/merge.hip
--- a/hagrid_amd/csrc/merge.hip
+++ b/hagrid_amd/csrc/merge.hip
@@ -432,7 +432,7 @@
 __global__ void __launch_bounds__(kBlock) ip_mark(MergeK k, const Entry* __restrict__ entries, const void* __restrict__ cells, const unsigned char* __restrict__ absorbs,
                                                   int pass_tag, int slots, unsigned char* __restrict__ dirty, const Int2* __restrict__ pass_total,
                                                   const int* __restrict__ removed, int num_tiles, int* __restrict__ books ,
-                                                  int* __restrict__ snap, size_t dstride) {
+                                                  int* __restrict__ snap, size_t dstride, Publish pub, int axis) {
     __shared__ int lds[kWaves];
     const int id4 = (blockIdx.x * kBlock + threadIdx.x) * kIpPer;
     const int overflow = books[3];
@@ -444,6 +444,11 @@
             if (overflow == 0) { books[0] += pass_total->a; books[1] -= pass_total->b; books[2] -= gone; }
             else if (overflow < 0) books[3] = -overflow;
             snap[0] = books[1]; snap[1] = books[2];
+            if (pub.n > 0) {
+                for (int i = 0; i < pub.n; i++) pub.dst[i] = i < 4 ? books[i] : snap[i - 4 - 2 * axis];
+                __threadfence_system();
+                __hip_atomic_store(pub.flag, pub.epoch, __ATOMIC_RELEASE, __HIP_MEMORY_SCOPE_SYSTEM);
+            }
         }
     }
     __shared__ int list[kIpTile];
@@ -627,14 +632,15 @@
     auto ip_leave = [&]() -> int {
         const int tiles = grid_blocks(ip_slots, kMergeTile);
         ip_live_sums<<<grid_blocks(tiles, kWaves), kBlock, 0, st>>>(cells, list_end, ip_slots, tile_sums, tiles); HG_DBG(ctx);
-        if (!ctx_scan<Int2>(ctx, SumsIn{tile_sums}, SumsOut{tile_sums}, tiles, partials, (const Int2*)nullptr, ip_total)) return HAGRID_ENOMEM;
+        const Publish pub = read_back_begin(ctx, ip_total, 2 * sizeof(int));
+        if (!ctx_scan<Int2>(ctx, SumsIn{tile_sums}, SumsOut{tile_sums}, tiles, partials, (const Int2*)nullptr, ip_total, pub)) return HAGRID_ENOMEM;
         ip_compact<<<tiles, kBlock, 0, st>>>(cells, list_end, refs, ip_slots, tile_sums, static_cast<Cell*>(cells_other), refs_b, nexts); HG_DBG(ctx);
         ip_resolve_tombs<<<grid_blocks(ip_slots, kBlock), kBlock, 0, st>>>(nexts, ip_slots); HG_DBG(ctx);
         remap_entries_kernel<<<grid_blocks((num_entries + 3) / 4, kBlock), kBlock, 0, st>>>(entries, nexts, num_entries); HG_DBG(ctx);
         std::swap(cells, cells_other);
         std::swap(refs, refs_b);
         int h[2];
-        HG_TRY(read_back(ctx, ip_total, h, sizeof(h)));
+        HG_TRY(read_back_wait(ctx, pub, ip_total, h, sizeof(h)));
         if (h[0] != num_cells) return fail(ctx, HAGRID_EHIP, __FILE__, __LINE__, "merge_grid: the books of the in-place iterations do not add up");
         num_refs = h[1];
         in_place = false; in_narrow = false; ip_iters = 0;
@@ -643,6 +649,7 @@
     };
     int last_pass_in = 0, last_pass_out = 0;
     auto compacting_passes = [&](int first_axis, int mask) -> int {
+        const Publish pub = read_back_begin(ctx, total, sizeof(int) * 6);
         for (int axis = first_axis; axis < 3; axis++) {
             const int blocks = grid_blocks(num_cells, kBlock);
             Int2* tot = total + axis;
@@ -655,7 +662,7 @@
             cell_flags_kernel<<<grid_blocks((num_cells + 3) / 4, kBlock), kBlock, 0, st>>>(nexts, prevs, pass_tag, cell_flags, num_cells, n_dev); HG_DBG(ctx);
             const int tiles = grid_blocks(num_cells, kMergeTile);
             merge_tile_sums<<<grid_blocks(tiles, kWaves), kBlock, 0, st>>>(cell_flags, merge_counts, num_cells, n_dev, tile_sums, tiles); HG_DBG(ctx);
-            if (!ctx_scan<Int2>(ctx, SumsIn{tile_sums}, SumsOut{tile_sums}, tiles, partials, (const Int2*)nullptr, tot)) return HAGRID_ENOMEM;
+            if (!ctx_scan<Int2>(ctx, SumsIn{tile_sums}, SumsOut{tile_sums}, tiles, partials, (const Int2*)nullptr, tot, axis == 2 ? pub : Publish())) return HAGRID_ENOMEM;
             global_pass++;
             const bool stamping = global_pass < 250 && (have_stamps || global_pass == 1);
             const unsigned char* st_in = stamping && have_stamps ? stamps : nullptr;
@@ -672,7 +679,7 @@
             std::swap(refs, refs_b);
         }
         int h[6];
-        HG_TRY(read_back(ctx, total, h, sizeof(int) * 6));
+        HG_TRY(read_back_wait(ctx, pub, total, h, sizeof(int) * 6));
         for (int axis = first_axis; axis < 3; axis++) {
             record(num_cells, num_refs);
             if (axis == 2) { last_pass_in = num_cells; last_pass_out = h[4]; }
@@ -693,6 +700,8 @@
             if (prev_mask & ~mask) (void)hipMemsetAsync(dirty, 1, 3 * ip_dstride, st);
             const int blocks = grid_blocks(ip_slots, kIpTile), tiles = blocks;
             const Entry* ent = reinterpret_cast<const Entry*>(entries);
+            int h[10];
+            const Publish pub = read_back_begin(ctx, books, sizeof(h));
             for (int axis = 0; axis < 3 && rc == HAGRID_OK; axis++) {
                 global_pass++;
                 if (++pass_tag == 256) {
@@ -705,11 +714,10 @@
                 if (!ctx_scan<Int2>(ctx, SumsIn{tile_sums}, SumsOut{tile_sums}, tiles, partials, (const Int2*)nullptr, ip_total)) { rc = HAGRID_ENOMEM; break; }
                 ip_apply<<<tiles, kBlock, 0, st>>>(cells, list_end, refs, cell_flags, pass_tag, minfo, nexts, tile_sums, ip_slots, books, ip_total,
                                                     ctx->opt_merge_inplace_room > 0 ? std::min(ip_capacity, ctx->opt_merge_inplace_room) : ip_capacity, axis); HG_DBG(ctx);
-                ip_mark<<<blocks, kBlock, 0, st>>>(k, ent, cells, cell_flags, pass_tag, ip_slots, dirty, ip_total, tile_removed, tiles, books, snap + 2 * axis, ip_dstride); HG_DBG(ctx);
+                ip_mark<<<blocks, kBlock, 0, st>>>(k, ent, cells, cell_flags, pass_tag, ip_slots, dirty, ip_total, tile_removed, tiles, books, snap + 2 * axis, ip_dstride, axis == 2 ? pub : Publish(), axis); HG_DBG(ctx);
             }
             if (rc != HAGRID_OK) break;
-            int h[10];
-            rc = read_back(ctx, books, h, sizeof(h));
+            rc = read_back_wait(ctx, pub, books, h, sizeof(h));
             if (rc != HAGRID_OK) break;
             const int applied = h[3] > 0 ? h[3] - 1 : 3;
             for (int axis = 0; axis < applied; axis++) { record(num_cells, num_refs); num_cells = h[4 + 2 * axis]; num_refs = h[5 + 2 * axis]; }
@@ -743,7 +751,7 @@
     hagrid_mem_free(ctx, cells_other);
     hagrid_mem_free(ctx, refs_b);
     if (rc != HAGRID_OK) {
-        (void)hipStreamSynchronize(st);
+        stream_sync_quiet(ctx);
         hagrid_mem_free(ctx, cells); hagrid_mem_free(ctx, refs);
         grid->cells = nullptr; grid->ref_ids = nullptr; grid->num_cells = 0; grid->num_refs = 0;
         return rc;
diff --git a/hagrid_amd/csrc/wave_prims.h b/hagrid_amd/csrc/wave_prims.h
--- a/hagrid_amd/csrc/wave_prims.h
+++ b/hagrid_amd/csrc/wave_prims.h
@@ -232,6 +232,8 @@
     return (unsigned)(a >> 34) == epoch && (unsigned)(b >> 34) == epoch && flag != 0u && flag == (unsigned(b >> 32) & 3u);
 }
 template <typename V> constexpr int lb_words() { return int(sizeof(V) / sizeof(int)); }
+__device__ __forceinline__ void lb_publish_total(const Publish& pub, const int* at, int t) { publish_from_wave(pub, at, t, 0, 1); }
+__device__ __forceinline__ void lb_publish_total(const Publish& pub, const Int2* at, Int2 t) { publish_from_wave(pub, reinterpret_cast<const int*>(at), t.a, t.b, 2); }
 
 __device__ __forceinline__ bool lb_aligned16(const void* p) { return (reinterpret_cast<uintptr_t>(p) & 15u) == 0; }
 template <typename V, typename In> __device__ __forceinline__ auto lb_load_row(const In& in, int i, int n, V* v, int) -> decltype(in.load4(i, n, v), void()) { in.load4(i, n, v); }
@@ -246,7 +248,7 @@
 }
 
 template <typename V, typename In, typename Out>
-__global__ void __launch_bounds__(kBlock) scan_lookback(In in, Out out, int n, int tiles, unsigned long long* state, unsigned epoch, unsigned help_after, const V* carry_in, V* total_out) {
+__global__ void __launch_bounds__(kBlock) scan_lookback(In in, Out out, int n, int tiles, unsigned long long* state, unsigned epoch, unsigned help_after, const V* carry_in, V* total_out, Publish pub) {
     __shared__ V lds[kWaves];
     __shared__ V tile_prefix;
     constexpr int kWaveItems = kLbItems * 64, kRows = kLbItems / kLbVec;
@@ -337,6 +339,7 @@
                 tile_prefix = excl;
                 if (total_out && tile == tiles - 1) *total_out = excl + agg;
             }
+            if (pub.n > 0 && tile == tiles - 1) lb_publish_total(pub, total_out, excl + agg);
         }
         __syncthreads();
         V offset = tile_prefix;
@@ -348,13 +351,17 @@
             lb_store_row<V>(out, base + r * 64 * kLbVec, n, v + r * kLbVec, 0);
         }
     }
-    if (tiles == 0 && blockIdx.x == 0 && threadIdx.x == 0 && total_out) *total_out = carry_in ? *carry_in : zero_of(V());
+    if (tiles == 0 && blockIdx.x == 0 && wave_id() == 0) {
+        const V t = carry_in ? *carry_in : zero_of(V());
+        if (lane_id() == 0 && total_out) *total_out = t;
+        if (pub.n > 0) lb_publish_total(pub, total_out, t);
+    }
 }
 
 inline int scan_num_tiles(int n) { return (n + kScanTile - 1) / kScanTile; }
 
 template <typename V, typename In, typename Out>
-inline void device_scan_lookback(hipStream_t stream, int num_cus, In in, Out out, int n, unsigned long long* state, unsigned epoch, unsigned help_after, const V* carry_in, V* total_out) {
+inline void device_scan_lookback(hipStream_t stream, int num_cus, In in, Out out, int n, unsigned long long* state, unsigned epoch, unsigned help_after, const V* carry_in, V* total_out, const Publish& pub = Publish()) {
     static const int per_cu = [] {
         int n = 0;
         if (hipOccupancyMaxActiveBlocksPerMultiprocessor(&n, scan_lookback<V, In, Out>, kBlock, 0) != hipSuccess) { (void)hipGetLastError(); n = 2; }
@@ -362,7 +369,7 @@
     }();
     const int tiles = (n + kLbTile - 1) / kLbTile;
     const int blocks = std::max(1, std::min(tiles, std::max(num_cus, 1) * per_cu));
-    scan_lookback<V, In, Out><<<blocks, kBlock, 0, stream>>>(in, out, n, tiles, state, epoch, help_after, carry_in, total_out);
+    scan_lookback<V, In, Out><<<blocks, kBlock, 0, stream>>>(in, out, n, tiles, state, epoch, help_after, carry_in, total_out, pub);
 }
 
 template <typename V, typename In, typename Out>
@@ -374,14 +381,14 @@
 }
 
 template <typename V, typename In, typename Out>
-inline bool ctx_scan(hagrid_ctx* ctx, In in, Out out, int n, V* partials, const V* carry_in, V* total_out) {
+inline bool ctx_scan(hagrid_ctx* ctx, In in, Out out, int n, V* partials, const V* carry_in, V* total_out, const Publish& pub = Publish()) {
 #ifdef HG_SCAN_THREE_KERNELS
     if (!ctx->opt_lookback) { device_scan<V>(ctx->stream, in, out, n, partials, carry_in, total_out); HG_DBG(ctx); return true; }
 #endif
     unsigned epoch = 0;
     unsigned long long* state = lookback_state(ctx, scan_num_tiles(n), lb_words<V>(), &epoch);
     if (!state) return false;
-    device_scan_lookback<V>(ctx->stream, ctx->num_cus, in, out, n, state, epoch, ctx->opt_lookback == 2 ? 0u : 4096u, carry_in, total_out);
+    device_scan_lookback<V>(ctx->stream, ctx->num_cus, in, out, n, state, epoch, ctx->opt_lookback == 2 ? 0u : 4096u, carry_in, total_out, pub);
     HG_DBG(ctx);
     return true;
 }
diff --git a/hagrid_amd/lib.py b/hagrid_amd/lib.py
--- a/hagrid_amd/lib.py
+++ b/hagrid_amd/lib.py
@@ -158,6 +158,7 @@
     "hagrid_kat_set_option": (_i32, [_vp, C.c_char_p, _i32]),
     "hagrid_kat_order_state": (_i32, [_vp, _vp, _vp, _vp]),
     "hagrid_kat_forget_hints": (_i32, [_vp]),
+    "hagrid_kat_set_async_error": (_i32, [_vp, _i32]),
     "hagrid_kat_detect_ray_rows": (_i32, [_vp, _vp, _i32, C.c_float, _vp]),
     "hagrid_kat_image_records": (_i32, [_vp, _vp, _vp, _i32, _vp, _vp]),
     "hagrid_kat_tile_slots": (_i32, [_vp, _i32, _i32, _i32, _i32, _vp]),
```

Result: no change. 7682 (-0.0%).
